# LCSL/nys-koop-lqr

Hardware: AMD Instinct MI355X
Metric: Nyström-Koopman fits/sec (K_nm build + A,B,C solve), N=1e5 m=2000 d=384 (higher is better)
Workload: dtype f64

## Files before the change

nys_koop_lqr_amd/csrc/nk_api.hip:

```cpp
#include "nk_common.h"

#include <cmath>
#include <cstdarg>
#include <cstdio>
#include <cstring>
#include <chrono>
#include <cstdlib>
#include <algorithm>
#include <condition_variable>
#include <mutex>
#include <set>
#include <thread>

namespace nk {

static thread_local std::string g_err;

void set_error(const char* fmt, ...) {
  char buf[1024];
  va_list ap;
  va_start(ap, fmt);
  vsnprintf(buf, sizeof(buf), fmt, ap);
  va_end(ap);
  g_err = buf;
// ... 111 lines not shown
  double* d = nullptr;
  NK_TRY(arena_alloc_t(ctx, (size_t)rows * ldd, &d));
  NK_HIP(hipMemcpy2DAsync(d, (size_t)ldd * 8, p, (size_t)ld * 8, (size_t)cols * 8, (size_t)rows, hipMemcpyHostToDevice,
                          ctx->stream));
  out->ptr = d;
  out->ld = ldd;
  out->staged = true;
  return NK_OK;
}
struct MatOut {
  double* dev = nullptr;
  int64_t ld = 0;
  double* host = nullptr;
  int64_t host_ld = 0;
  int64_t rows = 0, cols = 0;
};
static int stage_out(nk_ctx* ctx, double* p, int64_t ld, int64_t rows, int64_t cols, MatOut* out) {
  out->rows = rows;
  out->cols = cols;
  if (is_device_ptr(p)) {
    out->dev = p;
    out->ld = ld;
    out->host = nullptr;
    return NK_OK;
  }
  const int64_t ldd = cols + (cols & 1);
  NK_TRY(arena_alloc_t(ctx, (size_t)(rows > 0 ? rows : 1) * ldd, &out->dev));
  out->ld = ldd;
  out->host = p;
  out->host_ld = ld;
  return NK_OK;
}
static int finish_out(nk_ctx* ctx, const MatOut& o) {
  if (o.host && o.rows > 0 && o.cols > 0)
    NK_HIP(hipMemcpy2DAsync(o.host, (size_t)o.host_ld * 8, o.dev, (size_t)o.ld * 8, (size_t)o.cols * 8, (size_t)o.rows,
                            hipMemcpyDeviceToHost, ctx->stream));
  return NK_OK;
}

static int check_ctx(nk_ctx* ctx) {
  if (!ctx) {
    set_error("null context");
    return NK_ERR_BAD_ARG;
  }
  tl_ctx = ctx;
  NK_HIP(hipSetDevice(ctx->device));
  return arena_reset(ctx);
}

static int make_winv(nk_ctx* ctx, const nk_kernel_desc* kd, int d, double* dst_dev) {
  NK_REQUIRE(kd != nullptr, "null kernel descriptor");
  NK_REQUIRE(kd->type >= NK_KERNEL_RBF && kd->type <= NK_KERNEL_LINEAR, "unknown kernel type %d", kd->type);
  NK_REQUIRE(kd->d == d, "kernel descriptor is for %d dimensions, data has %d", kd->d, d);
  std::vector<double> w((size_t)d, 1.0);
  if (kd->type != NK_KERNEL_LINEAR) {
    NK_REQUIRE(kd->lengthscale != nullptr, "kernel lengthscale pointer is null");
    NK_REQUIRE(kd->n_lengthscale == 1 || kd->n_lengthscale == d,
               "Anisotropic kernel must have the same number of dimensions as data (%d!=%d)", kd->n_lengthscale, d);
    for (int k = 0; k < d; ++k) {
      const double l = kd->lengthscale[kd->n_lengthscale == 1 ? 0 : k];
      NK_REQUIRE(l > 0.0 && std::isfinite(l), "lengthscale[%d] = %g is not positive", k, l);
      w[k] = 1.0 / l;
    }
  }
  NK_HIP(hipMemcpyAsync(dst_dev, w.data(), sizeof(double) * d, hipMemcpyHostToDevice, ctx->stream));
  NK_HIP(hipStreamSynchronize(ctx->stream));
  return NK_OK;
}

struct ModelBuf {
  int device;
  size_t bytes;
  double* ptr;
};
static std::mutex g_pool_mu;
static std::vector<ModelBuf> g_pool;
static std::mutex g_reg_mu;
static std::set<nk_ctx*> g_ctxs;
static std::set<nk_model*> g_models;
static std::set<void*> g_host_blocks;

static double* pool_take(int device, size_t bytes) {
  std::lock_guard<std::mutex> lk(g_pool_mu);
  for (size_t i = 0; i < g_pool.size(); ++i)
    if (g_pool[i].device == device && g_pool[i].bytes == bytes) {
      double* p = g_pool[i].ptr;
      g_pool.erase(g_pool.begin() + i);
      return p;
    }
  return nullptr;
}
static void pool_give(int device, size_t bytes, double* ptr) {
  {
    std::lock_guard<std::mutex> lk(g_pool_mu);
    if (g_pool.size() < 512) {
      g_pool.push_back(ModelBuf{device, bytes, ptr});
      return;
    }
  }
  (void)hipSetDevice(device);
  (void)hipFree(ptr);
}
static void pool_drain() {
  std::lock_guard<std::mutex> lk(g_pool_mu);
  for (auto& b : g_pool) {
    (void)hipSetDevice(b.device);
    (void)hipFree(b.ptr);
  }
  g_pool.clear();
}

static int model_alloc(nk_ctx* ctx, int m, int d, int p, nk_model** out) {
  nk_model* mdl = new nk_model();
  mdl->device = ctx->device;
  mdl->m = m; mdl->d = d; mdl->p = p;
  const size_t mp = (size_t)m + p;
  const size_t total = (size_t)m * mp  + (size_t)d * m  + (size_t)d * mp  + 2 * (size_t)m * m +
                       (size_t)m * d  + (size_t)d  + 64;
  mdl->bytes = total * sizeof(double);
  mdl->buf = pool_take(ctx->device, mdl->bytes);
  if (!mdl->buf) {
    hipError_t e = hipMalloc(reinterpret_cast<void**>(&mdl->buf), mdl->bytes);
    if (e != hipSuccess) {
      (void)hipGetLastError();
      delete mdl;
      set_error("model allocation of %zu bytes failed: %s", total * sizeof(double), hipGetErrorString(e));
      return NK_ERR_OOM;
    }
  }
  double* q = mdl->buf;
  auto take = [&](size_t cnt) { double* r = q; q += (cnt + 1) & ~(size_t)1; return r; };
  mdl->A = take((size_t)m * mp);
  mdl->B = mdl->A + m;
  mdl->C = take((size_t)d * m);
  mdl->W = take((size_t)d * mp);
  mdl->S = take((size_t)m * m);
  mdl->Sinv = take((size_t)m * m);
  mdl->Z = take((size_t)m * d);
  mdl->winv = take((size_t)d);
  {
    std::lock_guard<std::mutex> lk(g_reg_mu);
    g_models.insert(mdl);
  }
  *out = mdl;
  return NK_OK;
}

static int lift_device(nk_ctx* ctx, const nk_model* mdl, const double* Xq, int64_t ldx, int64_t nq, double* out,
                       int64_t ldo) {
  const int m = mdl->m;
  const int64_t chunk = 32768;
  const ArenaMark mk = arena_mark(ctx);
  double* Kq = nullptr;
  NK_TRY(arena_alloc_t(ctx, (size_t)(nq < chunk ? nq : chunk) * m, &Kq));
  for (int64_t r0 = 0; r0 < nq; r0 += chunk) {
    const int64_t len = nq - r0 < chunk ? nq - r0 : chunk;
    NK_TRY(launch_kmat(ctx, mdl->ktype, Xq + r0 * ldx, ldx, len, mdl->Z, mdl->d, m, mdl->d, mdl->winv, mdl->sigma0, Kq,
                       m));
    NK_TRY(launch_gemm(ctx, false, false, len, m, m, 1.0, Kq, m, mdl->Sinv, m, 0.0, out + r0 * ldo, ldo));
  }
  arena_release(ctx, mk);
  return NK_OK;
}

static int predict_device(nk_ctx* ctx, const nk_model* mdl, const double* Xaug, int64_t ldx, int64_t nq, double* out,
                          int64_t ldo) {
  const int m = mdl->m, d = mdl->d, p = mdl->p;
  const int64_t chunk = 32768;
  const ArenaMark mk = arena_mark(ctx);
  double* phi = nullptr;
  NK_TRY(arena_alloc_t(ctx, (size_t)(nq < chunk ? nq : chunk) * m, &phi));
  for (int64_t r0 = 0; r0 < nq; r0 += chunk) {
    const int64_t len = nq - r0 < chunk ? nq - r0 : chunk;
    NK_TRY(lift_device(ctx, mdl, Xaug + r0 * ldx, ldx, len, phi, m));
    NK_TRY(launch_gemm(ctx, false, true, len, d, m, 1.0, phi, m, mdl->W, m + p, 0.0, out + r0 * ldo, ldo));
    if (p > 0)
      NK_TRY(launch_gemm(ctx, false, true, len, d, p, 1.0, Xaug + r0 * ldx + d, ldx, mdl->W + m, m + p, 1.0,
                         out + r0 * ldo, ldo));
  }
  arena_release(ctx, mk);
  return NK_OK;
}

struct HostTrace {
  bool on;
  std::chrono::steady_clock::time_point t0, last;
  HostTrace() : on(getenv("NYSKOOP_TRACE") != nullptr) { t0 = last = std::chrono::steady_clock::now(); }
  void mark(const char* what) {
    if (!on) return;
    auto now = std::chrono::steady_clock::now();
    fprintf(stderr, "[nk trace] %-28s +%8.3f ms (total %8.3f)\n", what,
            std::chrono::duration<double, std::milli>(now - last).count(),
            std::chrono::duration<double, std::milli>(now - t0).count());
    last = now;
  }
};

static float ev_ms(nk_ctx* ctx, int a, int b) {
  float ms = 0.f;
  (void)hipEventElapsedTime(&ms, ctx->ev[a], ctx->ev[b]);
  return ms;
}

}

using namespace nk;

extern "C" {

int nk_version(void) { return NK_ABI_VERSION; }

const char* nk_last_error(void) { return g_err.c_str(); }

int nk_device_count(void) {
  int n = 0;
  if (hipGetDeviceCount(&n) != hipSuccess) {
    (void)hipGetLastError();
    return 0;
  }
  return n;
}

int nk_create(int device, nk_ctx** out) {
  NK_REQUIRE(out != nullptr, "nk_create: null output pointer");
  *out = nullptr;
  int n = nk_device_count();
  if (n <= 0) {
    set_error("no HIP device visible: libnyskoop has no CPU fallback");
    return NK_ERR_NO_DEVICE;
  }
  NK_REQUIRE(device >= 0 && device < n, "nk_create: device %d out of range (0..%d)", device, n - 1);
  NK_HIP(hipSetDevice(device));
  hipDeviceProp_t prop;
  NK_HIP(hipGetDeviceProperties(&prop, device));
  if (strncmp(prop.gcnArchName, "gfx950", 6) != 0) {
    set_error("device %d is %s; libnyskoop is built for gfx950 (MI355X) only", device, prop.gcnArchName);
    return NK_ERR_NO_DEVICE;
  }
  nk_ctx* ctx = new nk_ctx();
  ctx->device = device;
  ctx->num_cu = prop.multiProcessorCount;
  int prio_lo = 0, prio_hi = 0;
  NK_HIP(hipDeviceGetStreamPriorityRange(&prio_lo, &prio_hi));
  const int prio_mid = (prio_lo - prio_hi >= 2) ? (prio_lo + prio_hi) / 2 : prio_hi;
  NK_HIP(hipStreamCreateWithPriority(&ctx->stream_main, hipStreamNonBlocking, prio_mid));
  NK_HIP(hipStreamCreateWithPriority(&ctx->stream_side, hipStreamNonBlocking, prio_lo));
  NK_HIP(hipStreamCreateWithPriority(&ctx->stream_prep, hipStreamNonBlocking, prio_hi));
  NK_HIP(hipStreamCreateWithFlags(&ctx->stream_copy, hipStreamNonBlocking));
  NK_HIP(hipStreamCreateWithPriority(&ctx->stream_la[0], hipStreamNonBlocking, prio_hi));
  NK_HIP(hipStreamCreateWithPriority(&ctx->stream_la[1], hipStreamNonBlocking, prio_mid));
  for (int q = 0; q < 2; ++q)
    for (int i = 0; i < 4; ++i) NK_HIP(hipEventCreateWithFlags(&ctx->ev_la[q][i], hipEventDisableTiming));
  ctx->stream = ctx->stream_main;
  ctx->cur_arena = &ctx->arena;
  NK_HIP(hipEventCreateWithFlags(&ctx->ev_fork, hipEventDisableTiming));
  NK_HIP(hipEventCreateWithFlags(&ctx->ev_join, hipEventDisableTiming));
  NK_HIP(hipEventCreateWithFlags(&ctx->ev_chain, hipEventDisableTiming));
  NK_HIP(hipMalloc(reinterpret_cast<void**>(&ctx->d_info), 256));
  ctx->d_piv = reinterpret_cast<unsigned long long*>(ctx->d_info + 16);
  NK_HIP(hipMalloc(reinterpret_cast<void**>(&ctx->d_scalars), 64 * sizeof(double)));
  NK_HIP(hipHostMalloc(reinterpret_cast<void**>(&ctx->h_scalars), 64 * sizeof(double), hipHostMallocMapped | hipHostMallocCoherent));
  NK_HIP(hipHostMalloc(reinterpret_cast<void**>(&ctx->h_info), 256, hipHostMallocMapped | hipHostMallocCoherent));
  ctx->h_piv = reinterpret_cast<unsigned long long*>(ctx->h_info + 16);
  for (int i = 0; i < 16; ++i) NK_HIP(hipEventCreate(&ctx->ev[i]));
  NK_HIP(hipEventCreateWithFlags(&ctx->ev_ext, hipEventDisableTiming));
  for (int i = 0; i < 8; ++i) NK_HIP(hipEventCreateWithFlags(&ctx->ev_up[i], hipEventDisableTiming));
  const char* km = getenv("NYSKOOP_KMAT");
  ctx->kmat_mode = (km && strcmp(km, "direct") == 0) ? 1 : 0;
  const char* st = getenv("NYSKOOP_STRICT_SPD");
  ctx->strict_spd = (st && atoi(st) != 0) ? 1 : 0;
  if (const char* rp = getenv("NYSKOOP_REFINE_PIVOT")) ctx->refine_pivot = atof(rp);
  if (const char* rs = getenv("NYSKOOP_REFINE_STEPS")) ctx->refine_steps = std::max(0, atoi(rs));
  {
    std::lock_guard<std::mutex> lk(g_reg_mu);
    g_ctxs.insert(ctx);
  }
  *out = ctx;
  return NK_OK;
}

static void destroy_ctx_unregistered(nk_ctx* ctx) {
  (void)hipSetDevice(ctx->device);
  if (tl_ctx == ctx) tl_ctx = nullptr;
  group_detach(ctx);
  (void)hipStreamSynchronize(ctx->stream_main);
  (void)hipStreamSynchronize(ctx->stream_side);
  (void)hipStreamSynchronize(ctx->stream_prep);
  (void)hipStreamSynchronize(ctx->stream_copy);
  for (int q = 0; q < 2; ++q) {
    if (ctx->stream_la[q]) { (void)hipStreamSynchronize(ctx->stream_la[q]); (void)hipStreamDestroy(ctx->stream_la[q]); }
    for (int i = 0; i < 4; ++i) if (ctx->ev_la[q][i]) (void)hipEventDestroy(ctx->ev_la[q][i]);
  }
  for (auto& c : ctx->arena.chunks) (void)hipFree(c.base);
  for (auto& c : ctx->arena_side.chunks) (void)hipFree(c.base);
  (void)hipEventDestroy(ctx->ev_fork);
  (void)hipEventDestroy(ctx->ev_join);
  if (ctx->ev_chain) (void)hipEventDestroy(ctx->ev_chain);
  if (ctx->ev_ext) (void)hipEventDestroy(ctx->ev_ext);
  for (int i = 0; i < 8; ++i) if (ctx->ev_up[i]) (void)hipEventDestroy(ctx->ev_up[i]);
  (void)hipStreamDestroy(ctx->stream_side);
  (void)hipStreamDestroy(ctx->stream_prep);
  (void)hipStreamDestroy(ctx->stream_copy);
  (void)hipFree(ctx->d_info);
  (void)hipFree(ctx->d_scalars);
  if (ctx->d_zeros) (void)hipFree(ctx->d_zeros);
  if (ctx->h_stage) (void)hipHostFree(ctx->h_stage);
  (void)hipHostFree(ctx->h_scalars);
  (void)hipHostFree(ctx->h_info);
  for (int i = 0; i < 16; ++i) (void)hipEventDestroy(ctx->ev[i]);
  (void)hipStreamDestroy(ctx->stream_main);
  delete ctx;
}

int nk_destroy(nk_ctx* ctx) {
  if (!ctx) return NK_OK;
  {
    std::lock_guard<std::mutex> lk(g_reg_mu);
    if (g_ctxs.erase(ctx) == 0) return NK_OK;
  }
  destroy_ctx_unregistered(ctx);
  return NK_OK;
}

static int model_wait_unchecked(nk_model* mdl);
static void destroy_model_unregistered(nk_model* model, bool to_pool) {
  (void)model_wait_unchecked(model);
  if (to_pool) {
    pool_give(model->device, model->bytes, model->buf);
  } else {
    (void)hipSetDevice(model->device);
    (void)hipFree(model->buf);
  }
  delete model;
}

int nk_shutdown(void) {
  tl_ctx = nullptr;
  std::set<nk_ctx*> ctxs;
  std::set<nk_model*> models;
  std::set<void*> blocks;
  {
    std::lock_guard<std::mutex> lk(g_reg_mu);
    ctxs.swap(g_ctxs);
    models.swap(g_models);
    blocks.swap(g_host_blocks);
  }
  for (nk_ctx* c : ctxs) {
    (void)hipSetDevice(c->device);
    (void)hipStreamSynchronize(c->stream_main);
    (void)hipStreamSynchronize(c->stream_side);
    (void)hipStreamSynchronize(c->stream_prep);
    (void)hipStreamSynchronize(c->stream_copy);
  }
  for (nk_model* m : models) destroy_model_unregistered(m, false);
  for (nk_ctx* c : ctxs) destroy_ctx_unregistered(c);
  pool_drain();
  for (void* b : blocks) (void)hipHostFree(b);
  return NK_OK;
}

int nk_set_compute_dtype(nk_ctx* ctx, int dtype) {
  NK_REQUIRE(ctx != nullptr && (dtype == NK_DTYPE_F64 || dtype == NK_DTYPE_F32), "nk_set_compute_dtype: bad argument");
  ctx->compute_f32 = dtype == NK_DTYPE_F32 ? 1 : 0;
  return NK_OK;
}

int nk_set_strict_spd(nk_ctx* ctx, int strict) {
  NK_REQUIRE(ctx != nullptr && strict >= 0 && strict <= 2, "nk_set_strict_spd: bad argument");
  ctx->strict_spd = strict;
  return NK_OK;
}

int nk_set_refine(nk_ctx* ctx, double pivot_ratio, int32_t steps) {
  NK_REQUIRE(ctx != nullptr && pivot_ratio >= 0.0 && pivot_ratio <= 1.0 && steps >= 0 && steps <= 8, "nk_set_refine: bad argument");
  ctx->refine_pivot = pivot_ratio;
  ctx->refine_steps = steps;
  return NK_OK;
}

int nk_wait_stream(nk_ctx* ctx, void* producer_stream) {
  NK_REQUIRE(ctx != nullptr, "nk_wait_stream: null context");
  NK_HIP(hipSetDevice(ctx->device));
  if (ctx->group) {
    hipError_t e = real_stream_sync(reinterpret_cast<hipStream_t>(producer_stream));
    if (e != hipSuccess) { set_error("synchronising the producer stream failed: %s", hipGetErrorString(e)); return NK_ERR_HIP; }
    return NK_OK;
  }
  NK_HIP(hipEventRecord(ctx->ev_ext, reinterpret_cast<hipStream_t>(producer_stream)));
  NK_HIP(hipStreamWaitEvent(ctx->stream_main, ctx->ev_ext, 0));
  NK_HIP(hipStreamWaitEvent(ctx->stream_side, ctx->ev_ext, 0));
  NK_HIP(hipStreamWaitEvent(ctx->stream_prep, ctx->ev_ext, 0));
  NK_HIP(hipStreamWaitEvent(ctx->stream_copy, ctx->ev_ext, 0));
  return NK_OK;
}

int nk_group_create(int device, int size, nk_ctx** out) {
  NK_REQUIRE(out != nullptr && size >= 1 && size <= 256, "nk_group_create: bad argument");
  for (int i = 0; i < size; ++i) out[i] = nullptr;
  for (int i = 0; i < size; ++i) {
    int rc = nk_create(device, &out[i]);
    if (rc != NK_OK) {
      for (int j = 0; j < i; ++j) { nk_destroy(out[j]); out[j] = nullptr; }
      return rc;
    }
  }
  nk_group* g = group_new(device, size);
  if (!g) {
    for (int i = 0; i < size; ++i) { nk_destroy(out[i]); out[i] = nullptr; }
    set_error("nk_group_create: could not create the shared stream / argument table");
    return NK_ERR_HIP;
  }
  for (int i = 0; i < size; ++i) group_attach(g, i, out[i]);
  return NK_OK;
}

int nk_group_enter(nk_ctx* ctx) {
  NK_REQUIRE(ctx != nullptr, "nk_group_enter: null context");
  return group_enter(ctx);
}

int nk_group_leave(nk_ctx* ctx) {
  NK_REQUIRE(ctx != nullptr, "nk_group_leave: null context");
  tl_ctx = ctx;
  const int rc = group_leave(ctx);
  tl_ctx = nullptr;
  return rc;
}

int nk_runtime_counters(uint64_t* out, int32_t n) {
  NK_REQUIRE(out != nullptr && n >= 0, "nk_runtime_counters: bad argument");
  for (int i = 0; i < n && i < CNT_N; ++i) out[i] = nk::read_counter(i);
  return NK_OK;
}

int nk_group_stats(nk_ctx* ctx, uint64_t* out4) {
  NK_REQUIRE(ctx != nullptr && out4 != nullptr, "nk_group_stats: null argument");
  group_stats(ctx, out4);
  return NK_OK;
}

int nk_cv_grid(nk_ctx* const* members, int32_t n_members, const double* X, int64_t ldx, const double* Y, int64_t ldy,
               int64_t n, int32_t d, int32_t p, const nk_cv_unit* units, int32_t n_units, double* scores, int32_t* status) {
  NK_REQUIRE(members && n_members >= 1 && X && Y && units && scores, "nk_cv_grid: null argument");
  NK_REQUIRE(n > 0 && d > 0 && p >= 0 && n_units >= 0 && ldx >= d + p && ldy >= d, "nk_cv_grid: bad sizes");
  for (int k = 0; k < n_members; ++k) NK_REQUIRE(members[k] != nullptr, "nk_cv_grid: null member context");
  for (int u = 0; u < n_units; ++u) {
    const nk_cv_unit& cu = units[u];
    NK_REQUIRE(cu.kernel && cu.landmark_rows && cu.m > 0, "nk_cv_grid: unit %d: null kernel / landmarks", u);
    NK_REQUIRE(0 <= cu.test_begin && cu.test_begin < cu.test_end && cu.test_end <= n, "nk_cv_grid: unit %d: bad test fold", u);
    for (int j = 0; j < cu.m; ++j)
      NK_REQUIRE(cu.landmark_rows[j] >= 0 && cu.landmark_rows[j] < n, "nk_cv_grid: unit %d: landmark row out of range", u);
  }
  if (n_units == 0) return NK_OK;
  nk_ctx* lead = members[0];
  NK_HIP(hipSetDevice(lead->device));
  const double *Xd = X, *Yd = Y;
  int64_t ldxd = ldx, ldyd = ldy;
  double *Xown = nullptr, *Yown = nullptr;
  struct Free { double*& a; double*& b; ~Free() { if (a) (void)hipFree(a); if (b) (void)hipFree(b); } } freer{Xown, Yown};
  if (!is_device_ptr(X)) {
    ldxd = d + p + ((d + p) & 1);
    NK_HIP(hipMalloc(reinterpret_cast<void**>(&Xown), (size_t)n * ldxd * 8));
    NK_HIP(hipMemcpy2D(Xown, (size_t)ldxd * 8, X, (size_t)ldx * 8, (size_t)(d + p) * 8, (size_t)n, hipMemcpyHostToDevice));
    Xd = Xown;
  }
  if (!is_device_ptr(Y)) {
    ldyd = d + (d & 1);
    NK_HIP(hipMalloc(reinterpret_cast<void**>(&Yown), (size_t)n * ldyd * 8));
    NK_HIP(hipMemcpy2D(Yown, (size_t)ldyd * 8, Y, (size_t)ldy * 8, (size_t)d * 8, (size_t)n, hipMemcpyHostToDevice));
    Yd = Yown;
  }
  std::vector<double> Yhost;
  const double* Yh = Y;
  int64_t ldyh = ldy;
  if (is_device_ptr(Y)) {
    Yhost.resize((size_t)n * d);
    NK_HIP(hipMemcpy2D(Yhost.data(), (size_t)d * 8, Y, (size_t)ldy * 8, (size_t)d * 8, (size_t)n, hipMemcpyDeviceToHost));
    Yh = Yhost.data();
    ldyh = d;
  }
  const int B = n_members;
  struct Round {
    std::mutex mu;
    std::condition_variable cv;
    int arrived = 0;
    uint64_t gen = 0;
    void wait(int parties) {
      std::unique_lock<std::mutex> lk(mu);
      const uint64_t g = gen;
      if (++arrived == parties) { arrived = 0; ++gen; lk.unlock(); cv.notify_all(); return; }
      cv.wait(lk, [&] { return gen != g; });
    }
  };
  std::vector<int> saved_strict((size_t)B);
  for (int k = 0; k < B; ++k) saved_strict[(size_t)k] = members[k]->strict_spd;
  std::mutex deferred_mu;
  std::vector<int> deferred;
  auto run_units = [&](const std::vector<int>& list, bool defer_rank_deficient) {
    Round round;
    const int count = (int)list.size();
    const int n_rounds = (count + B - 1) / B;
    auto worker = [&](int k) {
      nk_ctx* ctx = members[k];
      std::vector<double> Z;
      for (int r = 0; r < n_rounds; ++r) {
        const int slot = r * B + k;
        const bool mine = slot < count;
        if (mine) (void)group_enter(ctx);
        round.wait(B);
        if (mine) {
          const int u = list[(size_t)slot];
          const nk_cv_unit& cu = units[u];
          Z.resize((size_t)cu.m * d);
          for (int j = 0; j < cu.m; ++j) memcpy(&Z[(size_t)j * d], Yh + cu.landmark_rows[j] * ldyh, (size_t)d * 8);
          const int64_t rr[4] = {0, cu.test_begin, cu.test_end, n};
          nk_model* mdl = nullptr;
          int rc = nk_nystrom_fit(ctx, cu.kernel, Xd, ldxd, Yd, ldyd, n, d, p, rr, 2, nullptr, 0, Z.data(), d, cu.m, cu.gamma,
                                  cu.jitter, &mdl, nullptr);
          double sc = std::nan("");
          if (rc == NK_OK)
            rc = nk_score_neg_rmse(ctx, mdl, Xd + cu.test_begin * ldxd, ldxd, Yd + cu.test_begin * ldyd, ldyd,
                                   cu.test_end - cu.test_begin, &sc);
          if (mdl) nk_model_destroy(mdl);
          tl_ctx = ctx;
          const int rc_leave = group_leave(ctx);
          if (rc == NK_OK) rc = rc_leave;
          if (rc == NK_ERR_NOT_SPD && defer_rank_deficient) {
            std::lock_guard<std::mutex> lk(deferred_mu);
            deferred.push_back(u);
          } else {
            scores[u] = rc == NK_OK ? sc : std::nan("");
            if (status) status[u] = rc;
          }
        }
        round.wait(B);
      }
      tl_ctx = nullptr;
    };
    std::vector<std::thread> threads;
    threads.reserve((size_t)B);
    for (int k = 0; k < B; ++k) threads.emplace_back(worker, k);
    for (auto& t : threads) t.join();
  };
  std::vector<int> all((size_t)n_units);
  for (int u = 0; u < n_units; ++u) all[(size_t)u] = u;
  bool all_lenient = true;
  for (int k = 0; k < B; ++k) all_lenient = all_lenient && saved_strict[(size_t)k] == 0;
  if (!all_lenient) {
    run_units(all, false);
    return NK_OK;
  }
  const bool cv_trace = getenv("NYSKOOP_CV_TRACE") != nullptr;
  const auto t_start = std::chrono::steady_clock::now();
  for (int k = 0; k < B; ++k) members[k]->strict_spd = 1;
  run_units(all, true);
  for (int k = 0; k < B; ++k) members[k]->strict_spd = saved_strict[(size_t)k];
  const auto t_mid = std::chrono::steady_clock::now();
  if (!deferred.empty()) {
    std::sort(deferred.begin(), deferred.end());
    for (int k = 0; k < B; ++k) members[k]->strict_spd = 0;
    run_units(deferred, false);
    for (int k = 0; k < B; ++k) members[k]->strict_spd = saved_strict[(size_t)k];
  }
  if (cv_trace)
    fprintf(stderr, "[nyskoop] cv_grid: %d units in %.3f s, %zu rank-deficient units again in %.3f s (%d members)\n", n_units,
            std::chrono::duration<double>(t_mid - t_start).count(), deferred.size(),
            std::chrono::duration<double>(std::chrono::steady_clock::now() - t_mid).count(), B);
  return NK_OK;
}

int nk_synchronize(nk_ctx* ctx) {
  NK_REQUIRE(ctx != nullptr, "null context");
  tl_ctx = ctx;
  NK_HIP(hipStreamSynchronize(ctx->stream));
  return NK_OK;
}

void* nk_stream(nk_ctx* ctx) { return ctx ? reinterpret_cast<void*>(ctx->stream) : nullptr; }

void* nk_host_alloc(uint64_t bytes) {
  void* p = nullptr;
  if (hipHostMalloc(&p, bytes ? bytes : 1, hipHostMallocDefault) != hipSuccess) {
    (void)hipGetLastError();
    set_error("hipHostMalloc of %llu bytes failed", (unsigned long long)bytes);
    return nullptr;
  }
  std::lock_guard<std::mutex> lk(g_reg_mu);
  g_host_blocks.insert(p);
  return p;
}

void nk_host_free(void* ptr) {
  if (!ptr) return;
  {
    std::lock_guard<std::mutex> lk(g_reg_mu);
    if (g_host_blocks.erase(ptr) == 0) return;
  }
  (void)hipHostFree(ptr);
}

int nk_set_kmat_mode(nk_ctx* ctx, int mode) {
  NK_REQUIRE(ctx != nullptr && (mode == 0 || mode == 1), "nk_set_kmat_mode: bad argument");
  ctx->kmat_mode = mode;
  return NK_OK;
}

// ... 208 lines not shown
  };
  auto queue_side = [&]() -> int {
    NK_TRY(alloc_sqrt_bufs());
    SideScope side(ctx);
    NK_HIP(hipStreamWaitEvent(ctx->stream, ctx->ev_fork, 0));
    NK_HIP(hipStreamWaitEvent(ctx->stream, ev[9], 0));
    NK_HIP(hipEventRecord(ev[6], ctx->stream));
    NK_TRY(sqrtm_finish(ctx, &splan, mdl->S, mdl->Sinv));
    NK_HIP(hipEventRecord(ev[7], ctx->stream));
    NK_TRY(sqrt_products());
    NK_HIP(hipEventRecord(ctx->ev_join, ctx->stream));
    return NK_OK;
  };
  if (mode == FIT_SOLVE) {
    NK_HIP(hipMemcpyAsync(G1, gram_io, gram_doubles(m, d, p) * sizeof(double),
                          is_device_ptr(gram_io) ? hipMemcpyDeviceToDevice : hipMemcpyHostToDevice, ctx->stream));
    NK_HIP(hipEventRecord(ev[2], ctx->stream));
  } else {
  const bool f32 = ctx->compute_f32 != 0 && ctx->kmat_mode == 0 && d >= 32 && !ctx_recording(ctx) && m >= 4 && d >= 4;
  const int64_t off_out = f32 ? ((mp + 3) & ~3) : ((mp + 1) & ~1);
  const int64_t ldf = f32 ? ((off_out + m + 3) & ~(int64_t)3) : ((off_out + m + 1) & ~(int64_t)1);
  const double felem = f32 ? 4.0 : 8.0;
  int64_t pass_rows;
  {
    const char* b = getenv("NYSKOOP_F_BUDGET_GB");
    const double budget = (b ? atof(b) : 48.0) * 1073741824.0;
    pass_rows = (int64_t)(budget / ((double)ldf * felem));
    if (pass_rows < 1024) pass_rows = 1024;
    pass_rows &= ~(int64_t)1023;
    if (host_passes > 1) {
      const int64_t per = ((n_eff + host_passes - 1) / host_passes + 1023) & ~(int64_t)1023;
      if (per < pass_rows) pass_rows = per;
    }
  }
  struct Piece { int64_t b, len; };
  std::vector<std::vector<Piece>> passes(1);
  {
    int64_t used = 0;
    for (size_t i = 0; i < rng.size(); i += 2) {
      int64_t b = rng[i];
      const int64_t e = rng[i + 1];
      while (b < e) {
        if (used == pass_rows) { passes.emplace_back(); used = 0; }
        const int64_t len = std::min(e - b, pass_rows - used);
        passes.back().push_back(Piece{b, len});
        used += len;
        b += len;
      }
    }
  }
  const int64_t f_rows = passes.size() > 1 ? pass_rows : n_eff;
  double* F = nullptr;
  NK_TRY(arena_alloc_t(ctx, f32 ? ((size_t)f_rows * ldf + 1) / 2 + 64 : (size_t)f_rows * ldf + 64, &F));
  const bool gram_form = ctx->kmat_mode == 0 && d >= 32;
  int64_t maxlen = 0;
  for (auto& ps : passes) for (auto& pc : ps) maxlen = std::max(maxlen, pc.len);
  const int64_t ldt = (maxlen + 1) & ~(int64_t)1, ldzt = (m + 1) & ~1;
  double *center = nullptr, *Rt = nullptr, *sqr = nullptr, *Zto = nullptr, *sqzo = nullptr, *Zti = nullptr, *sqzi = nullptr;
  double *Rt2 = nullptr, *sqr2 = nullptr;
  const bool overlap_prep = gram_form && passes.size() == 1 && passes[0].size() == 1;
  if (gram_form) {
    NK_TRY(arena_alloc_t(ctx, (size_t)d, &center));
    if (!f32) {
      NK_TRY(arena_alloc_t(ctx, (size_t)d * ldt, &Rt));
      NK_TRY(arena_alloc_t(ctx, (size_t)maxlen, &sqr));
    }
    if (overlap_prep && !f32) {
      NK_TRY(arena_alloc_t(ctx, (size_t)d * ldt, &Rt2));
      NK_TRY(arena_alloc_t(ctx, (size_t)maxlen, &sqr2));
    }
    NK_TRY(arena_alloc_t(ctx, (size_t)d * ldzt, &Zto));
    NK_TRY(arena_alloc_t(ctx, (size_t)m, &sqzo));
    if (kd->type == NK_KERNEL_LINEAR) NK_TRY(launch_fill(ctx, center, d, 1, d, 0.0));
    else NK_TRY(launch_colmean(ctx, zo.ptr, zo.ld, m, d, center));
    NK_TRY(prep_rows(ctx, zo.ptr, zo.ld, m, d, mdl->winv, center, Zto, ldzt, sqzo));
    if (same_centers) {
      Zti = Zto; sqzi = sqzo;
    } else {
      NK_TRY(arena_alloc_t(ctx, (size_t)d * ldzt, &Zti));
      NK_TRY(arena_alloc_t(ctx, (size_t)m, &sqzi));
      NK_TRY(prep_rows(ctx, zi.ptr, zi.ld, m, d, mdl->winv, center, Zti, ldzt, sqzi));
    }
  }
  float *F32 = reinterpret_cast<float*>(F), *Rt32 = nullptr, *sq32 = nullptr, *Zt32 = nullptr, *sqz32 = nullptr, *Y32 = nullptr;
  const int64_t ldt32 = (maxlen + 3) & ~(int64_t)3, ldzt32 = (m + 3) & ~3, ldy32 = (d + 3) & ~3;
  if (f32) {
    NK_REQUIRE(same_centers, "fp32 engine: separate input landmarks are not supported");
    double* tmp = nullptr;
    NK_TRY(arena_alloc_t(ctx, ((size_t)d * ldt32 + 1) / 2 + 2, &tmp)); Rt32 = reinterpret_cast<float*>(tmp);
    NK_TRY(arena_alloc_t(ctx, ((size_t)maxlen + 1) / 2 + 2, &tmp)); sq32 = reinterpret_cast<float*>(tmp);
    NK_TRY(arena_alloc_t(ctx, ((size_t)d * ldzt32 + 1) / 2 + 2, &tmp)); Zt32 = reinterpret_cast<float*>(tmp);
    NK_TRY(arena_alloc_t(ctx, ((size_t)m + 1) / 2 + 2, &tmp)); sqz32 = reinterpret_cast<float*>(tmp);
    NK_TRY(arena_alloc_t(ctx, ((size_t)f_rows * ldy32 + 1) / 2 + 2, &tmp)); Y32 = reinterpret_cast<float*>(tmp);
    NK_TRY(prep_rows_f32(ctx, zo.ptr, zo.ld, m, d, mdl->winv, center, Zt32, ldzt32, sqz32));
  }
  const bool multi_pass = passes.size() > 1;
  const bool pipelined = host_passes > 1;
  auto upload_pass = [&](size_t ip) -> int {
    for (const Piece& pc : passes[ip]) {
      NK_HIP(hipMemcpy2DAsync(const_cast<double*>(x.ptr) + pc.b * x.ld, (size_t)x.ld * 8, X + pc.b * ldx, (size_t)ldx * 8,
                              (size_t)(d + p) * 8, (size_t)pc.len, hipMemcpyHostToDevice, ctx->stream_side));
      NK_HIP(hipMemcpy2DAsync(const_cast<double*>(y.ptr) + pc.b * y.ld, (size_t)y.ld * 8, Y + pc.b * ldy, (size_t)ldy * 8,
                              (size_t)d * 8, (size_t)pc.len, hipMemcpyHostToDevice, ctx->stream_side));
    }
    NK_HIP(hipEventRecord(ctx->ev_up[ip & 7], ctx->stream_side));
    return NK_OK;
  };
  if (pipelined) {
    NK_HIP(hipEventRecord(ev[12], ctx->stream));
    NK_HIP(hipStreamWaitEvent(ctx->stream_side, ev[12], 0));
    NK_TRY(upload_pass(0));
  }
  for (size_t ip = 0; ip < passes.size(); ++ip) {
    const std::vector<Piece>& ps = passes[ip];
    const double beta = ip == 0 ? 0.0 : 1.0;
    if (pipelined) NK_HIP(hipStreamWaitEvent(ctx->stream, ctx->ev_up[ip & 7], 0));
    if (f32) {
      int64_t o32 = 0;
      for (const Piece& pc : ps) {
        const double* xs = x.ptr + pc.b * x.ld;
        const double* ys = y.ptr + pc.b * y.ld;
        NK_TRY(prep_rows_f32(ctx, xs, x.ld, pc.len, d, mdl->winv, center, Rt32, ldt32, sq32));
        NK_TRY(launch_kmat_gram_f32(ctx, kd->type, Rt32, ldt32, sq32, pc.len, Zt32, ldzt32, sqz32, m, d, kd->sigma0,
                                    F32 + o32 * ldf, ldf));
        NK_TRY(prep_rows_f32(ctx, ys, y.ld, pc.len, d, mdl->winv, center, Rt32, ldt32, sq32));
        NK_TRY(launch_kmat_gram_f32(ctx, kd->type, Rt32, ldt32, sq32, pc.len, Zt32, ldzt32, sqz32, m, d, kd->sigma0,
                                    F32 + o32 * ldf + off_out, ldf));
        if (p > 0) NK_TRY(launch_cvt_f64_f32(ctx, xs + d, x.ld, F32 + o32 * ldf + m, ldf, pc.len, p));
        NK_TRY(launch_cvt_f64_f32(ctx, ys, y.ld, Y32 + o32 * ldy32, ldy32, pc.len, d));
        o32 += pc.len;
      }
      if (ip == 0) {
        NK_HIP(hipEventRecord(ev[2], ctx->stream));
        tr.mark("kmat issued");
      }
      TnProblemF pf[4];
      pf[0].A = F32; pf[0].B = F32; pf[0].lda = pf[0].ldb = ldf; pf[0].M = pf[0].N = mp; pf[0].C = G1; pf[0].ldc = mp;
      pf[0].tri = TRI_UPPER_MIRROR;
      pf[1].A = F32 + off_out; pf[1].B = F32; pf[1].lda = pf[1].ldb = ldf; pf[1].M = m; pf[1].N = mp; pf[1].C = G2; pf[1].ldc = mp;
      pf[2].A = F32 + off_out; pf[2].B = F32 + off_out; pf[2].lda = pf[2].ldb = ldf; pf[2].M = pf[2].N = m; pf[2].C = G3;
      pf[2].ldc = m; pf[2].tri = TRI_UPPER_MIRROR;
      pf[3].A = Y32; pf[3].lda = ldy32; pf[3].M = d; pf[3].N = m; pf[3].C = G4; pf[3].ldc = m; pf[3].B = F32 + off_out;
      pf[3].ldb = ldf;
      for (int q = 0; q < 4; ++q) pf[q].beta = beta;
      float ms1 = 0.f;
      NK_TRY(launch_gemm_tn_f32_multi(ctx, pf, 4, o32, 0, timed ? &ms1 : nullptr, multi_pass));
      if (multi_pass) ms_gram_kernel += ms1; else gram_deferred = timed;
      gram_launches += 1;
      if (pipelined && ip + 1 < passes.size()) NK_TRY(upload_pass(ip + 1));
      continue;
    }
    int64_t o = 0;
    for (const Piece& pc : ps) {
      const double* xs = x.ptr + pc.b * x.ld;
      const double* ys = y.ptr + pc.b * y.ld;
      if (gram_form && overlap_prep) {
        NK_HIP(hipEventRecord(ev[12], ctx->stream));
        {
          SideScope side(ctx);
          NK_HIP(hipStreamWaitEvent(ctx->stream, ev[12], 0));
          NK_TRY(prep_rows(ctx, ys, y.ld, pc.len, d, mdl->winv, center, Rt2, ldt, sqr2));
          NK_HIP(hipEventRecord(ev[13], ctx->stream));
        }
        NK_TRY(prep_rows(ctx, xs, x.ld, pc.len, d, mdl->winv, center, Rt, ldt, sqr));
        NK_TRY(launch_kmat_gram(ctx, kd->type, Rt, ldt, sqr, pc.len, Zti, ldzt, sqzi, m, d, kd->sigma0, F + o * ldf, ldf));
        NK_HIP(hipStreamWaitEvent(ctx->stream, ev[13], 0));
        NK_TRY(launch_kmat_gram(ctx, kd->type, Rt2, ldt, sqr2, pc.len, Zto, ldzt, sqzo, m, d, kd->sigma0,
                                F + o * ldf + off_out, ldf));
      } else if (gram_form) {
        NK_TRY(prep_rows(ctx, xs, x.ld, pc.len, d, mdl->winv, center, Rt, ldt, sqr));
        NK_TRY(launch_kmat_gram(ctx, kd->type, Rt, ldt, sqr, pc.len, Zti, ldzt, sqzi, m, d, kd->sigma0, F + o * ldf, ldf));
        NK_TRY(prep_rows(ctx, ys, y.ld, pc.len, d, mdl->winv, center, Rt, ldt, sqr));
        NK_TRY(launch_kmat_gram(ctx, kd->type, Rt, ldt, sqr, pc.len, Zto, ldzt, sqzo, m, d, kd->sigma0,
                                F + o * ldf + off_out, ldf));
      } else {
        NK_TRY(launch_kmat(ctx, kd->type, xs, x.ld, pc.len, zi.ptr, zi.ld, m, d, mdl->winv, kd->sigma0, F + o * ldf, ldf));
        NK_TRY(launch_kmat(ctx, kd->type, ys, y.ld, pc.len, zo.ptr, zo.ld, m, d, mdl->winv, kd->sigma0,
                           F + o * ldf + off_out, ldf));
      }
      if (p > 0) NK_TRY(launch_copy2d(ctx, xs + d, x.ld, F + o * ldf + m, ldf, pc.len, p));
      o += pc.len;
    }
    const int64_t rows = o;
    if (ip == 0) {
      NK_HIP(hipEventRecord(ev[2], ctx->stream));
      tr.mark("kmat issued");
    }
    TnProblem pr[4];
    pr[0].A = F; pr[0].B = F; pr[0].lda = pr[0].ldb = ldf; pr[0].M = pr[0].N = mp; pr[0].C = G1; pr[0].ldc = mp;
    pr[0].tri = TRI_UPPER_MIRROR;
    pr[1].A = F + off_out; pr[1].B = F; pr[1].lda = pr[1].ldb = ldf; pr[1].M = m; pr[1].N = mp; pr[1].C = G2;
    pr[1].ldc = mp;
    pr[2].A = F + off_out; pr[2].B = F + off_out; pr[2].lda = pr[2].ldb = ldf; pr[2].M = pr[2].N = m; pr[2].C = G3;
    pr[2].ldc = m; pr[2].tri = TRI_UPPER_MIRROR;
    pr[3].A = y.ptr + ps[0].b * y.ld; pr[3].lda = y.ld; pr[3].M = d; pr[3].N = m; pr[3].C = G4; pr[3].ldc = m;
    pr[3].B = F + off_out; pr[3].ldb = ldf;
    for (int q = 0; q < 4; ++q) pr[q].beta = beta;
    const bool single = ps.size() == 1;
    const bool fast = tn_fast_ok(pr[0]) && tn_fast_ok(pr[1]) && tn_fast_ok(pr[2]);
    const bool fast_y = fast && tn_fast_ok(pr[3]);
    bool y_done = false;
    if (fast) {
      const int np = (single && fast_y) ? 4 : 3;
      float ms1 = 0.f;
      NK_TRY(launch_gemm_tn_multi(ctx, pr, np, rows, 0, (timed && !pipelined) ? &ms1 : nullptr, multi_pass));
      if (multi_pass) ms_gram_kernel += ms1; else gram_deferred = timed;
      gram_launches += 1;
      y_done = np == 4;
    } else {
      GemmOpts sym;
      sym.tri = TRI_UPPER_MIRROR;
      float t3[3] = {0.f, 0.f, 0.f};
      NK_TRY(launch_gemm(ctx, true, false, mp, mp, rows, 1.0, F, ldf, F, ldf, beta, G1, mp, sym, timed ? &t3[0] : nullptr));
      NK_TRY(launch_gemm(ctx, true, false, m, mp, rows, 1.0, F + off_out, ldf, F, ldf, beta, G2, mp, GemmOpts(),
                         timed ? &t3[1] : nullptr));
      NK_TRY(launch_gemm(ctx, true, false, m, m, rows, 1.0, F + off_out, ldf, F + off_out, ldf, beta, G3, m, sym,
                         timed ? &t3[2] : nullptr));
      ms_gram_kernel += t3[0] + t3[1] + t3[2];
      gram_launches += 3;
    }
    if (!y_done) {
      int64_t oo = 0;
      bool first = true;
      for (const Piece& pc : ps) {
        NK_TRY(launch_gemm(ctx, true, false, d, m, pc.len, 1.0, y.ptr + pc.b * y.ld, y.ld, F + oo * ldf + off_out, ldf,
                           (first && ip == 0) ? 0.0 : 1.0, G4, m));
        oo += pc.len;
        first = false;
      }
    }
    if (pipelined && ip + 1 < passes.size()) NK_TRY(upload_pass(ip + 1));
  }
  }
  NK_HIP(hipEventRecord(ev[3], ctx->stream));
  if (mode == FIT_GRAM) {
    NK_HIP(hipMemcpyAsync(gram_io, G1, gram_doubles(m, d, p) * sizeof(double),
                          is_device_ptr(gram_io) ? hipMemcpyDeviceToDevice : hipMemcpyDeviceToHost, ctx->stream));
    NK_HIP(hipStreamSynchronize(ctx->stream));
    if (stats) {
      memset(stats, 0, sizeof(*stats));
      stats->ms_total = ev_ms(ctx, 0, 3);
      stats->ms_upload = (x.staged || y.staged) ? ev_ms(ctx, 0, 1) : 0.0;
      stats->ms_kmat = ev_ms(ctx, 1, 2);
      stats->ms_gram = ev_ms(ctx, 2, 3);
      if (gram_deferred) ms_gram_kernel = ev_ms(ctx, 14, 15);
      stats->ms_gram_kernel_avg = gram_launches ? ms_gram_kernel / gram_launches : 0.0;
      stats->gram_kernel_launches = gram_launches;
    }
    if (ctx->arena.chunks.size() > 1 || ctx->arena_side.chunks.size() > 1) NK_TRY(arena_reset(ctx));
    return NK_OK;
  }
  NK_HIP(hipEventRecord(ctx->ev_fork, ctx->stream));
  tr.mark("gram issued");

  NK_TRY(queue_prep());

  if (landmarks_aside) NK_HIP(hipStreamWaitEvent(ctx->stream, ev[8], 0));
  NK_TRY(launch_axpby2d(ctx, gamma_n, Kj_in, m, 1.0, G1, mp, m, m));
  if (p > 0) NK_TRY(launch_add_diag(ctx, G1 + (int64_t)m * mp + m, mp, p, gamma_n));
  NK_TRY(launch_axpby2d(ctx, gamma_n, Kj, m, 1.0, G3, m, m, m));
  double* Gsave = nullptr;
  NK_TRY(arena_alloc_t(ctx, gram_doubles(m, d, p), &Gsave));
  NK_HIP(hipMemcpyAsync(Gsave, G1, gram_doubles(m, d, p) * sizeof(double), hipMemcpyDeviceToDevice, ctx->stream));
  double *Linv = nullptr, *Linv2 = nullptr, *V1 = nullptr, *Wc = nullptr, *Ct = nullptr;
  const int nblk = (mp + CHOL_NB - 1) / CHOL_NB;
  NK_TRY(arena_alloc_t(ctx, (size_t)nblk * CHOL_WS, &Linv));
  NK_TRY(arena_alloc_t(ctx, (size_t)nblk * CHOL_WS, &Linv2));
  NK_TRY(arena_alloc_t(ctx, (size_t)m * m, &V1));
  NK_TRY(alloc_sqrt_bufs());
  NK_TRY(arena_alloc_t(ctx, (size_t)m * ldd, &Wc));
  NK_TRY(arena_alloc_t(ctx, (size_t)m * ldd, &Ct));
  CholSys sys[2];
  double* pivlog = nullptr;
  NK_TRY(arena_alloc_t(ctx, (size_t)mp + m + 4, &pivlog));
  sys[0].P = G1; sys[0].ldp = mp; sys[0].m = mp; sys[0].Linv = Linv; sys[0].extra = m;
  sys[1].P = G3; sys[1].ldp = m; sys[1].m = m; sys[1].Linv = Linv2; sys[1].extra = d;
  sys[0].pivlog = pivlog; sys[1].pivlog = pivlog + mp + (mp & 1);
  NK_TRY(cholesky_aug_pair_async(ctx, sys, 2));
  tr.mark("cholesky + solves issued");

  NK_TRY(queue_side());
  NK_HIP(hipStreamWaitEvent(ctx->stream, ctx->ev_join, 0));
  NK_HIP(hipEventRecord(ev[4], ctx->stream));
  tr.mark("side stream joined (queued)");

  auto operator_products = [&]() -> int {
    NK_TRY(launch_transpose(ctx, G2, mp, V1, m, m, m));
    NK_TRY(launch_gemm(ctx, true, false, m, m, m, 1.0, V1, m, T1t, m, 0.0, X1, m));
    NK_TRY(launch_gemm(ctx, true, false, m, m, m, 1.0, Sinvt, m, X1, m, 0.0, mdl->A, mp));
    if (p > 0) NK_TRY(launch_gemm(ctx, true, false, m, p, m, 1.0, Sinvt, m, G2 + m, mp, 0.0, mdl->B, mp));
    NK_TRY(launch_transpose(ctx, G4, m, Wc, ldd, d, m));
    NK_TRY(launch_gemm(ctx, true, false, m, d, m, 1.0, mdl->S, m, Wc, ldd, 0.0, Ct, ldd));
    NK_TRY(launch_transpose(ctx, Ct, ldd, mdl->C, m, m, d));
    NK_TRY(launch_gemm(ctx, true, false, d, mp, m, 1.0, Ct, ldd, mdl->A, mp, 0.0, mdl->W, mp));
    return NK_OK;
  };
  NK_TRY(operator_products());
  NK_HIP(hipEventRecord(ev[5], ctx->stream));
  tr.mark("solve issued");
  int chol_failed[2] = {0, 0};
  double piv_ratio[2] = {1.0, 1.0};
  NK_TRY(cholesky_fail_flags(ctx, sys, 2, chol_failed, piv_ratio));
  tr.mark("final sync");
  int rank_sys[2] = {mp, m};
  bool redo_products = false;
  if (ctx->strict_spd == 2) chol_failed[0] = chol_failed[1] = -1;
  if (chol_failed[0] || chol_failed[1]) {
    if (ctx->strict_spd == 1) {
      set_error("Cholesky: system %d is numerically rank deficient (non-positive or rounding-level pivot; the reference's "
                "lstsq truncates here) and strict mode is on", chol_failed[0] ? 0 : 1);
      return NK_ERR_NOT_SPD;
    }
    const double rcond = 2.220446049250313e-16;
    for (int q = 0; q < 2; ++q) {
      if (!chol_failed[q]) continue;
      PinvInfo pi;
      if (q == 0)
        NK_TRY(pinv_right_divide(ctx, Gsave, mp, mp, Gsave + (size_t)mp * mp, mp, m, G2, mp, rcond, &pi));
      else
        NK_TRY(pinv_right_divide(ctx, Gsave + gram_block1(m, p), m, m, Gsave + gram_block1(m, p) + (size_t)m * m, m, d, G4,
                                 m, rcond, &pi));
      if (!pi.converged) {
        set_error("rank-revealing fallback: Jacobi SVD of system %d did not converge in %d sweeps", q, pi.sweeps);
        return NK_ERR_NO_CONVERGENCE;
      }
      rank_sys[q] = pi.rank;
    }
    count_event(CNT_RANK_TRUNCATED);
    redo_products = true;
  }
  int refined[2] = {0, 0};
  {
    const double refine_below = ctx->refine_pivot;
    const int refine_steps = ctx->refine_steps;
    double* refine_state = nullptr;
    NK_TRY(arena_alloc_t(ctx, (size_t)8, &refine_state));
    for (int q = 0; q < 2 && refine_steps > 0; ++q) {
      if (chol_failed[q] || !(piv_ratio[q] > 0.0) || piv_ratio[q] >= refine_below) continue;
      const int mq = sys[q].m, nr = sys[q].extra;
      const size_t off = q == 0 ? 0 : gram_block1(m, p);
      const double* Pq = Gsave + off;
      const double* Rq = Gsave + off + (size_t)mq * mq;
      double* Xq = G1 + off + (size_t)mq * mq;
      const ArenaMark mk = arena_mark(ctx);
      double *Res = nullptr, *ResT = nullptr, *partial = nullptr;
      const int64_t ldt_ = nr + (nr & 1);
      NK_TRY(arena_alloc_t(ctx, (size_t)nr * mq, &Res));
      NK_TRY(arena_alloc_t(ctx, (size_t)mq * ldt_, &ResT));
      NK_TRY(arena_alloc_t(ctx, (size_t)2 * refine_partial_blocks(), &partial));
      CholSys y = sys[q];
      y.R = ResT; y.ldr = ldt_; y.nrhs = nr;
      for (int step = 0; step < refine_steps; ++step) {
        NK_TRY(launch_resid_dd(ctx, Xq, mq, Pq, mq, Rq, mq, Res, mq, nr, mq));
        NK_TRY(launch_transpose(ctx, Res, mq, ResT, ldt_, nr, mq));
        NK_TRY(cholesky_solve_pair(ctx, &y, 1));
        NK_TRY(launch_transpose(ctx, ResT, ldt_, Res, mq, mq, nr));
        NK_TRY(launch_refine_apply(ctx, Res, mq, Xq, mq, nr, mq, step, refine_state + 4 * q, partial));
      }
      NK_HIP(hipMemcpyAsync(ctx->h_scalars + 16 + 4 * q, refine_state + 4 * q, 4 * sizeof(double), hipMemcpyDeviceToHost,
                            ctx->stream));
      arena_release(ctx, mk);
      refined[q] = -1;
      redo_products = true;
    }
  }
  {
    const int vr = sqrtm_verdict(ctx, &splan, &it, &resid);
    if (vr == NK_SQRT_RETRY) {
      count_event(CNT_SQRT_RETRY);
      NK_TRY(sqrtm_spd_coupled(ctx, Kj, m, m, mdl->S, mdl->Sinv, &it, &resid));
      NK_TRY(sqrt_products());
      redo_products = true;
    } else {
      NK_TRY(vr);
    }
  }
  if (redo_products) {
    NK_TRY(operator_products());
    NK_HIP(hipStreamSynchronize(ctx->stream));
  }
  double refine_ratio[2] = {0.0, 0.0};
  for (int q = 0; q < 2; ++q)
    if (refined[q] < 0) {
      refined[q] = (int)ctx->h_scalars[16 + 4 * q + 2];
      refine_ratio[q] = ctx->h_scalars[16 + 4 * q + 3];
    }
  if (refined[0] > 0 || refined[1] > 0) count_event(CNT_REFINED);
  mdl->has_ops = true;

  if (stats) {
    memset(stats, 0, sizeof(*stats));
    stats->ms_total = ev_ms(ctx, 0, 5);
    stats->ms_upload = (x.staged || y.staged) ? ev_ms(ctx, 0, 1) : 0.0;
    stats->ms_kmat = ev_ms(ctx, 1, 2);
    stats->ms_gram = ev_ms(ctx, 2, 3);
    stats->ms_sqrt = ev_ms(ctx, 6, 7);
    stats->ms_solve = ev_ms(ctx, 4, 5);
    if (gram_deferred) ms_gram_kernel = ev_ms(ctx, 14, 15);
    stats->ms_gram_kernel_avg = gram_launches ? ms_gram_kernel / gram_launches : 0.0;
    stats->gram_kernel_launches = gram_launches;
    stats->sqrt_iters = it;
    stats->sqrt_residual = resid;
    const double ne = (double)n_eff;
    const double t128 = 128.0;
    auto tiles = [&](double v) { return std::ceil(v / t128); };
    const double tmp_ = tiles(mp), tm_ = tiles(m);
    stats->gram_flops = 2.0 * ne * t128 * t128 * (tmp_ * (tmp_ + 1) / 2 + tm_ * tmp_ + tm_ * (tm_ + 1) / 2) +
                        2.0 * ne * (double)d * m;
    stats->kmat_pairs = 2.0 * ne * m * d + (same_centers ? 1.0 : 3.0) * (double)m * m * d;
    stats->rank_inner = rank_sys[0];
    stats->rank_inner_rec = rank_sys[1];
    stats->pivot_ratio_inner = piv_ratio[0];
    stats->pivot_ratio_inner_rec = piv_ratio[1];
    stats->refined = refined[0] + 16 * refined[1];
    stats->refine_ratio_inner = refine_ratio[0];
    stats->refine_ratio_inner_rec = refine_ratio[1];
  }
  tr.mark("stats");
  if (ctx->arena.chunks.size() > 1 || ctx->arena_side.chunks.size() > 1) NK_TRY(arena_reset(ctx));
  guard.m = nullptr;
  *model = mdl;
  return NK_OK;
}

int nk_nystrom_fit(nk_ctx* ctx, const nk_kernel_desc* kd, const double* X, int64_t ldx, const double* Y, int64_t ldy,
                   int64_t n, int32_t d, int32_t p, const int64_t* row_ranges, int32_t n_ranges, const double* Zin,
                   int64_t ldzi, const double* Zout, int64_t ldzo, int32_t m, double gamma, double jitter,
                   nk_model** model, nk_fit_stats* stats) {
  NK_REQUIRE(model != nullptr, "nk_nystrom_fit: null argument");
  return fit_impl(ctx, kd, X, ldx, Y, ldy, n, d, p, row_ranges, n_ranges, Zin, ldzi, Zout, ldzo, m, gamma, jitter, model,
                  stats, FIT_FULL, nullptr);
}

int nk_gram_doubles(int32_t m, int32_t d, int32_t p, int64_t* count) {
  NK_REQUIRE(count && m > 0 && d > 0 && p >= 0, "nk_gram_doubles: bad argument");
  *count = (int64_t)gram_doubles(m, d, p);
  return NK_OK;
}

int nk_nystrom_gram(nk_ctx* ctx, const nk_kernel_desc* kd, const double* X, int64_t ldx, const double* Y, int64_t ldy,
                    int64_t n, int32_t d, int32_t p, const int64_t* row_ranges, int32_t n_ranges, const double* Zin,
                    int64_t ldzi, const double* Zout, int64_t ldzo, int32_t m, double* gram, nk_fit_stats* stats) {
  return fit_impl(ctx, kd, X, ldx, Y, ldy, n, d, p, row_ranges, n_ranges, Zin, ldzi, Zout, ldzo, m, 0.0, 0.0, nullptr,
                  stats, FIT_GRAM, gram);
}

int nk_nystrom_solve(nk_ctx* ctx, const nk_kernel_desc* kd, const double* Zin, int64_t ldzi, const double* Zout,
                     int64_t ldzo, int32_t m, int32_t d, int32_t p, const double* gram, int64_t n_total, double gamma,
                     double jitter, nk_model** model, nk_fit_stats* stats) {
  NK_REQUIRE(model != nullptr, "nk_nystrom_solve: null argument");
  return fit_impl(ctx, kd, nullptr, 0, nullptr, 0, n_total, d, p, nullptr, 0, Zin, ldzi, Zout, ldzo, m, gamma, jitter,
                  model, stats, FIT_SOLVE, const_cast<double*>(gram));
}

int nk_model_create(nk_ctx* ctx, const nk_kernel_desc* kd, const double* Zout, int64_t ldz, int32_t m, int32_t d,
                    int32_t p, double jitter, const double* A, const double* B, const double* C, const double* W,
                    nk_model** model) {
  NK_TRY(check_ctx(ctx));
  NK_REQUIRE(kd && Zout && model, "nk_model_create: null argument");
  NK_REQUIRE(m > 0 && d > 0 && p >= 0 && ldz >= d, "nk_model_create: bad sizes");
  *model = nullptr;
  nk_model* mdl = nullptr;
  NK_TRY(model_alloc(ctx, m, d, p, &mdl));
  struct Guard { nk_model* m; ~Guard() { if (m) nk_model_destroy(m); } } guard{mdl};
  mdl->ktype = kd->type; mdl->sigma0 = kd->sigma0; mdl->jitter = jitter;
  NK_TRY(make_winv(ctx, kd, d, mdl->winv));
  MatIn z;
  NK_TRY(stage_in(ctx, Zout, ldz, m, d, &z));
  NK_TRY(launch_copy2d(ctx, z.ptr, z.ld, mdl->Z, d, m, d));
  double* Kj = nullptr;
  NK_TRY(arena_alloc_t(ctx, (size_t)m * m, &Kj));
  NK_TRY(launch_kmat(ctx, kd->type, mdl->Z, d, m, mdl->Z, d, m, d, mdl->winv, kd->sigma0, Kj, m));
  NK_TRY(launch_add_diag(ctx, Kj, m, m, jitter));
  NK_TRY(sqrtm_spd(ctx, Kj, m, m, mdl->S, mdl->Sinv, nullptr, nullptr));
  const int mp = m + p;
  if (A && C) {
    NK_REQUIRE(p == 0 || B != nullptr, "nk_model_create: B missing");
    MatIn a, b, c, w;
    NK_TRY(stage_in(ctx, A, m, m, m, &a));
    NK_TRY(launch_copy2d(ctx, a.ptr, a.ld, mdl->A, mp, m, m));
    if (p > 0) {
      NK_TRY(stage_in(ctx, B, p, m, p, &b));
      NK_TRY(launch_copy2d(ctx, b.ptr, b.ld, mdl->B, mp, m, p));
    }
    NK_TRY(stage_in(ctx, C, m, d, m, &c));
    NK_TRY(launch_copy2d(ctx, c.ptr, c.ld, mdl->C, m, d, m));
    if (W) {
      NK_TRY(stage_in(ctx, W, mp, d, mp, &w));
      NK_TRY(launch_copy2d(ctx, w.ptr, w.ld, mdl->W, mp, d, mp));
    } else {
      NK_TRY(launch_gemm(ctx, false, false, d, mp, m, 1.0, mdl->C, m, mdl->A, mp, 0.0, mdl->W, mp));
    }
    mdl->has_ops = true;
  }
  NK_HIP(hipStreamSynchronize(ctx->stream));
  guard.m = nullptr;
  *model = mdl;
  return NK_OK;
}

int nk_model_destroy(nk_model* model) {
  if (!model) return NK_OK;
  {
    std::lock_guard<std::mutex> lk(g_reg_mu);
    if (g_models.erase(model) == 0) return NK_OK;
  }
  destroy_model_unregistered(model, true);
  return NK_OK;
}

int nk_model_dims(const nk_model* model, int32_t* m, int32_t* d, int32_t* p) {
  NK_REQUIRE(model != nullptr, "null model");
  if (m) *m = model->m;
  if (d) *d = model->d;
  if (p) *p = model->p;
  return NK_OK;
}

int nk_model_get(nk_ctx* ctx, const nk_model* mdl, char which, double* out, int64_t ldo) {
  NK_TRY(check_ctx(ctx));
  NK_REQUIRE(mdl && out, "nk_model_get: null argument");
  const int m = mdl->m, d = mdl->d, p = mdl->p, mp = m + p;
  const double* src = nullptr;
  int64_t lds = 0, rows = 0, cols = 0;
  switch (which) {
    case 'A': src = mdl->A; lds = mp; rows = m; cols = m; break;
    case 'B': src = mdl->B; lds = mp; rows = m; cols = p; break;
    case 'C': src = mdl->C; lds = m; rows = d; cols = m; break;
    case 'W': src = mdl->W; lds = mp; rows = d; cols = mp; break;
    case 'S': src = mdl->S; lds = m; rows = m; cols = m; break;
    case 'I': src = mdl->Sinv; lds = m; rows = m; cols = m; break;
    case 'Z': src = mdl->Z; lds = d; rows = m; cols = d; break;
    default: set_error("nk_model_get: unknown selector '%c'", which); return NK_ERR_BAD_ARG;
  }
  if ((which == 'A' || which == 'B' || which == 'C' || which == 'W') && !mdl->has_ops) {
    set_error("nk_model_get: model holds no fitted operators");
    return NK_ERR_BAD_ARG;
  }
  if (rows == 0 || cols == 0) return NK_OK;
  NK_REQUIRE(ldo >= cols, "nk_model_get: leading dimension too small");
  NK_HIP(hipMemcpy2DAsync(out, (size_t)ldo * 8, src, (size_t)lds * 8, (size_t)cols * 8, (size_t)rows,
                          is_device_ptr(out) ? hipMemcpyDeviceToDevice : hipMemcpyDeviceToHost, ctx->stream));
  NK_HIP(hipStreamSynchronize(ctx->stream));
  return NK_OK;
}

int nk_model_get_ops(nk_ctx* ctx, const nk_model* mdl, double* G, int64_t ldg, double* Cm, int64_t ldc, double* W,
                     int64_t ldw) {
  NK_TRY(check_ctx(ctx));
  NK_REQUIRE(mdl != nullptr, "nk_model_get_ops: null model");
  if (!mdl->has_ops) {
    set_error("nk_model_get_ops: model holds no fitted operators");
    return NK_ERR_BAD_ARG;
  }
  const int m = mdl->m, d = mdl->d, mp = m + mdl->p;
  NK_REQUIRE((!G || ldg >= mp) && (!Cm || ldc >= m) && (!W || ldw >= mp), "nk_model_get_ops: leading dimension too small");
  auto copy = [&](double* dst, int64_t ldd, const double* src, int64_t lds, int64_t rows, int64_t cols,
                  hipStream_t st) -> hipError_t {
    const hipMemcpyKind kind = is_device_ptr(dst) ? hipMemcpyDeviceToDevice : hipMemcpyDeviceToHost;
    if (ldd == cols && lds == cols) return hipMemcpyAsync(dst, src, (size_t)rows * cols * 8, kind, st);
    return hipMemcpy2DAsync(dst, (size_t)ldd * 8, src, (size_t)lds * 8, (size_t)cols * 8, (size_t)rows, kind, st);
  };
  if (G) NK_HIP(copy(G, ldg, mdl->A, mp, m, mp, ctx->stream_main));
  if (Cm) NK_HIP(copy(Cm, ldc, mdl->C, m, d, m, ctx->stream_side));
  if (W) NK_HIP(copy(W, ldw, mdl->W, mp, d, mp, ctx->stream_side));
  NK_HIP(hipStreamSynchronize(ctx->stream_side));
  NK_HIP(hipStreamSynchronize(ctx->stream_main));
  return NK_OK;
}

int nk_model_get_ops_async(nk_ctx* ctx, nk_model* mdl, double* G, int64_t ldg, double* Cm, int64_t ldc, double* W,
                           int64_t ldw) {
  NK_TRY(check_ctx(ctx));
  NK_REQUIRE(mdl != nullptr, "nk_model_get_ops_async: null model");
  if (!mdl->has_ops) {
    set_error("nk_model_get_ops_async: model holds no fitted operators");
    return NK_ERR_BAD_ARG;
  }
  const int m = mdl->m, d = mdl->d, mp = m + mdl->p;
  NK_REQUIRE((!G || ldg >= mp) && (!Cm || ldc >= m) && (!W || ldw >= mp),
             "nk_model_get_ops_async: leading dimension too small");
  NK_TRY(nk_model_wait(mdl));
  auto copy = [&](double* dst, int64_t ldd, const double* src, int64_t lds, int64_t rows, int64_t cols) -> hipError_t {
    const hipMemcpyKind kind = is_device_ptr(dst) ? hipMemcpyDeviceToDevice : hipMemcpyDeviceToHost;
    if (ldd == cols && lds == cols) return hipMemcpyAsync(dst, src, (size_t)rows * cols * 8, kind, ctx->stream_copy);
    return hipMemcpy2DAsync(dst, (size_t)ldd * 8, src, (size_t)lds * 8, (size_t)cols * 8, (size_t)rows, kind,
                            ctx->stream_copy);
  };
  if (G) NK_HIP(copy(G, ldg, mdl->A, mp, m, mp));
  if (Cm) NK_HIP(copy(Cm, ldc, mdl->C, m, d, m));
  if (W) NK_HIP(copy(W, ldw, mdl->W, mp, d, mp));
  if (ctx_recording(ctx)) {
    NK_HIP(hipStreamSynchronize(ctx->stream));
    return NK_OK;
  }
  hipEvent_t ev = nullptr;
  NK_HIP(hipEventCreateWithFlags(&ev, hipEventDisableTiming));
  hipError_t e = hipEventRecord(ev, ctx->stream_copy);
  if (e != hipSuccess) {
    (void)hipEventDestroy(ev);
    (void)hipStreamSynchronize(ctx->stream_copy);
    set_error("hipEventRecord failed: %s", hipGetErrorString(e));
    return NK_ERR_HIP;
  }
  mdl->ev_fetch = ev;
  return NK_OK;
}

static int model_wait_unchecked(nk_model* mdl);

int nk_model_wait(nk_model* mdl) {
  NK_REQUIRE(mdl != nullptr, "nk_model_wait: null model");
  {
    std::lock_guard<std::mutex> lk(g_reg_mu);
    if (g_models.count(mdl) == 0) return NK_OK;
  }
  return model_wait_unchecked(mdl);
}

static int model_wait_unchecked(nk_model* mdl) {
  if (mdl->ev_fetch) {
    hipError_t e = real_event_sync(mdl->ev_fetch);
    (void)hipEventDestroy(mdl->ev_fetch);
    mdl->ev_fetch = nullptr;
    if (e != hipSuccess) {
      set_error("hipEventSynchronize failed: %s", hipGetErrorString(e));
      return NK_ERR_HIP;
    }
  }
  return NK_OK;
}

struct SmallStage {
  nk_ctx* ctx = nullptr;
  size_t off = 0;
  struct Out { double* stage; double* user; int64_t user_ld; int64_t rows, cols; };
  std::vector<Out> outs;
};
constexpr size_t SMALL_STAGE_LIMIT = (size_t)4 << 20;
static int small_reserve(nk_ctx* ctx, size_t bytes) {
  if (ctx->h_stage_bytes >= bytes) return NK_OK;
  if (ctx->h_stage) (void)hipHostFree(ctx->h_stage);
  ctx->h_stage = nullptr;
  ctx->h_stage_bytes = 0;
  NK_HIP(hipHostMalloc(reinterpret_cast<void**>(&ctx->h_stage), bytes, hipHostMallocDefault));
  ctx->h_stage_bytes = bytes;
  return NK_OK;
}
static const double* small_in(SmallStage& st, const double* host, int64_t ld, int64_t rows, int64_t cols) {
  double* dst = reinterpret_cast<double*>(reinterpret_cast<char*>(st.ctx->h_stage) + st.off);
  for (int64_t r = 0; r < rows; ++r) memcpy(dst + r * cols, host + r * ld, (size_t)cols * 8);
  st.off += (((size_t)rows * cols * 8) + 255) & ~(size_t)255;
  return dst;
}
static double* small_out(SmallStage& st, double* user, int64_t user_ld, int64_t rows, int64_t cols) {
  double* dst = reinterpret_cast<double*>(reinterpret_cast<char*>(st.ctx->h_stage) + st.off);
  st.off += (((size_t)rows * cols * 8) + 255) & ~(size_t)255;
  st.outs.push_back(SmallStage::Out{dst, user, user_ld, rows, cols});
  return dst;
}
static void small_finish(SmallStage& st) {
  for (auto& o : st.outs)
    for (int64_t r = 0; r < o.rows; ++r) memcpy(o.user + r * o.user_ld, o.stage + r * o.cols, (size_t)o.cols * 8);
}
static inline size_t pad256(size_t doubles) { return ((doubles * 8) + 255) & ~(size_t)255; }

int nk_lift(nk_ctx* ctx, const nk_model* mdl, const double* Xq, int64_t ldx, int64_t nq, double* out, int64_t ldo) {
  NK_TRY(check_ctx(ctx));
  NK_REQUIRE(mdl && Xq && out, "nk_lift: null argument");
  NK_REQUIRE(nq >= 0 && ldx >= mdl->d && ldo >= mdl->m, "nk_lift: bad sizes");
  if (nq == 0) return NK_OK;
// ... 518 lines not shown
```

nys_koop_lqr_amd/csrc/nk_common.h:

```cpp
#pragma once
#include <hip/hip_runtime.h>
#include <stdint.h>
#include <stddef.h>
#include <string>
#include <vector>

#include "nyskoop.h"
#include "nk_lockstep.h"

namespace nk {

void set_error(const char* fmt, ...);

#define NK_HIP(call)                                                                         \
  do {                                                                                       \
    hipError_t e_ = (call);                                                                  \
    if (e_ != hipSuccess) {                                                                  \
      nk::set_error("%s failed: %s (%s:%d)", #call, hipGetErrorString(e_), __FILE__, __LINE__); \
      return e_ == hipErrorOutOfMemory ? NK_ERR_OOM : NK_ERR_HIP;                            \
    }                                                                                        \
  } while (0)

#define NK_TRY(call)            \
  do {                          \
    int rc_ = (call);           \
    if (rc_ != NK_OK) return rc_; \
  } while (0)

#define NK_REQUIRE(cond, ...)     \
  do {                            \
    if (!(cond)) {                \
      nk::set_error(__VA_ARGS__); \
      return NK_ERR_BAD_ARG;      \
    }                             \
  } while (0)

struct ArenaChunk {
  char* base = nullptr;
  size_t cap = 0;
  size_t off = 0;
};
struct Arena {
  std::vector<ArenaChunk> chunks;
  int cur = 0;
};
struct ArenaMark {
  int chunk;
  size_t off;
};

}

struct nk_member_state;
struct nk_ctx {
  int device = 0;
  hipStream_t stream = nullptr;
  hipStream_t stream_main = nullptr;
  hipStream_t stream_side = nullptr;
  hipStream_t stream_copy = nullptr;
  hipStream_t stream_prep = nullptr;
  nk::Arena arena;
  nk::Arena arena_side;
  nk::Arena* cur_arena = nullptr;
  hipStream_t stream_la[2] = {nullptr, nullptr};
  hipEvent_t ev_la[2][4] = {};
  int compute_f32 = 0;
  hipEvent_t ev_fork = nullptr, ev_join = nullptr, ev_chain = nullptr;
  int* d_info = nullptr;
  unsigned long long* d_piv = nullptr;
  unsigned long long* h_piv = nullptr;
  double* d_scalars = nullptr;
  double* h_scalars = nullptr;
  int* h_info = nullptr;
  double* d_zeros = nullptr;
  hipEvent_t ev[16];
  int num_cu = 256;
  int kmat_mode = 0;
  double refine_pivot = 0.0;
  int refine_steps = 2;
  int strict_spd = 0;
  hipEvent_t ev_ext = nullptr;
  hipEvent_t ev_up[8] = {};
  nk_group* group = nullptr;
  nk_member_state* gstate = nullptr;
  double* h_stage = nullptr;
  size_t h_stage_bytes = 0;
};

struct nk_model {
  int device = 0;
  int32_t m = 0, d = 0, p = 0;
  int32_t ktype = 0;
  double sigma0 = 0.0;
  double jitter = 0.0;
  double* buf = nullptr;
  size_t bytes = 0;
  double *A = nullptr, *B = nullptr, *C = nullptr, *W = nullptr, *S = nullptr, *Sinv = nullptr, *Z = nullptr,
         *winv = nullptr;
  bool has_ops = false;
  hipEvent_t ev_fetch = nullptr;
};

namespace nk {

struct SideScope {
  nk_ctx* c;
  hipStream_t s0;
  Arena* a0;
  explicit SideScope(nk_ctx* ctx, hipStream_t s = nullptr) : c(ctx), s0(ctx->stream), a0(ctx->cur_arena) {
    c->stream = s ? s : c->stream_side;
    c->cur_arena = &c->arena_side;
  }
  ~SideScope() {
    c->stream = s0;
    c->cur_arena = a0;
  }
};

inline int info_base(const nk_ctx* c) { return c->stream != c->stream_main ? 2 : 0; }

__device__ __forceinline__ double exp_nonpos_ca() {
  double ca = __longlong_as_double(0x3e5ade156a5dcb37LL);
  asm volatile("" : "+v"(ca));
  return ca;
}
__device__ __forceinline__ double exp_nonpos(double x, double ca_v) {
  const double k = __builtin_rint(x * __longlong_as_double(0x3ff71547652b82feLL));
  double r = __builtin_fma(__longlong_as_double((long long)0xbfe62e42fefa39efULL), k, x);
  r = __builtin_fma(__longlong_as_double((long long)0xbc7abc9e3b39803fULL), k, r);
  double p;
#define NK_EXP_STEP(c) asm("v_fma_f64 %0, %1, %2, %3" : "=v"(p) : "v"(r), "v"(p), "s"(c))
  asm("v_fma_f64 %0, %1, %2, %3" : "=v"(p) : "v"(r), "v"(ca_v), "s"(__longlong_as_double(0x3e928af3fca7ab0cLL)));
  NK_EXP_STEP(__longlong_as_double(0x3ec71dee623fde64LL));
  NK_EXP_STEP(__longlong_as_double(0x3efa01997c89e6b0LL));
  NK_EXP_STEP(__longlong_as_double(0x3f2a01a014761f6eLL));
  NK_EXP_STEP(__longlong_as_double(0x3f56c16c1852b7b0LL));
  NK_EXP_STEP(__longlong_as_double(0x3f81111111122322LL));
  NK_EXP_STEP(__longlong_as_double(0x3fa55555555502a1LL));
  NK_EXP_STEP(__longlong_as_double(0x3fc5555555555511LL));
  NK_EXP_STEP(__longlong_as_double(0x3fe000000000000bLL));
#undef NK_EXP_STEP
  p = __builtin_fma(r, p, 1.0);
  p = __builtin_fma(r, p, 1.0);
  return x < -1075.0 ? 0.0 : ldexp(p, (int)k);
}
__device__ __forceinline__ double exp_nonpos(double x) { return exp_nonpos(x, exp_nonpos_ca()); }

nk_group* group_new(int device, int size);
void group_attach(nk_group* g, int slot, nk_ctx* c);
void group_detach(nk_ctx* c);
int group_enter(nk_ctx* c);
int group_leave(nk_ctx* c);
void group_stats(nk_ctx* c, uint64_t out[4]);
enum { CNT_CHAIN_GIVEUP = 0, CNT_JACOBI_GIVEUP = 1, CNT_RANK_TRUNCATED = 2, CNT_SQRT_RETRY = 3, CNT_REFINED = 4, CNT_N = 5 };
void count_event(int which);
uint64_t read_counter(int which);
hipError_t real_stream_sync(hipStream_t s);
hipError_t real_event_sync(hipEvent_t e);

int arena_reset(nk_ctx* ctx);
ArenaMark arena_mark(nk_ctx* ctx);
void arena_release(nk_ctx* ctx, ArenaMark mk);
int arena_alloc(nk_ctx* ctx, size_t bytes, void** out);
template <typename T>
inline int arena_alloc_t(nk_ctx* ctx, size_t count, T** out) {
  return arena_alloc(ctx, count * sizeof(T), reinterpret_cast<void**>(out));
}
bool is_device_ptr(const void* p);

int launch_kmat(nk_ctx* ctx, int ktype, const double* A, int64_t lda, int64_t nA, const double* B, int64_t ldb,
                int64_t nB, int d, const double* winv, double sigma0, double* out, int64_t ldo);

enum { TRI_FULL = 0, TRI_UPPER_MIRROR = 1, TRI_LOWER = 2 };
struct GemmOpts {
  int tri = TRI_FULL;
  int splitk = 0;
};
int launch_gemm(nk_ctx* ctx, bool transA, bool transB, int64_t M, int64_t N, int64_t K, double alpha, const double* A,
                int64_t lda, const double* B, int64_t ldb, double beta, double* C, int64_t ldc,
                const GemmOpts& opts = GemmOpts(), float* ms_kernel = nullptr);

struct GemmCall {
  int64_t M = 0, N = 0, K = 0;
  double alpha = 1.0, beta = 0.0;
  const double* A = nullptr;
  const double* B = nullptr;
  double* C = nullptr;
  int64_t lda = 0, ldb = 0, ldc = 0;
  GemmOpts opts;
};
int launch_gemm_pair(nk_ctx* ctx, bool transA, bool transB, const GemmCall* calls, int ncalls);

struct TnSkip;
int launch_add_diag(nk_ctx* ctx, double* A, int64_t lda, int n, double v);
int launch_copy2d(nk_ctx* ctx, const double* src, int64_t lds, double* dst, int64_t ldd, int64_t rows, int64_t cols);
int launch_axpby2d(nk_ctx* ctx, double a, const double* X, int64_t ldx, double b, double* Y, int64_t ldy,
                   int64_t rows, int64_t cols);
int launch_scale_add_identity(nk_ctx* ctx, double a, const double* X, int64_t ldx, double c, double* Y, int64_t ldy,
                              int n, const TnSkip* skip = nullptr);
int launch_fill(nk_ctx* ctx, double* A, int64_t lda, int64_t rows, int64_t cols, double v);
int launch_frob_minus_identity(nk_ctx* ctx, const double* M, int64_t ldm, int n, double* d_out,
                               const TnSkip* skip = nullptr);
int launch_max_abs_rowsum(nk_ctx* ctx, const double* M, int64_t ldm, int n, double* d_out);
int launch_colsum_sqdiff(nk_ctx* ctx, const double* P, int64_t ldp, const double* Y, int64_t ldy, int64_t rows,
                         int cols, double* d_colsum);

int sqrtm_spd(nk_ctx* ctx, const double* P, int64_t ldp, int m, double* S, double* Sinv, int* iters, double* resid);
struct SqrtPlan {
  const double* P = nullptr;
  int64_t ldp = 0;
  int m = 0;
  double* W = nullptr;
  double* Linv = nullptr;
  double* X0 = nullptr;
  double* X0t = nullptr;
  double* d_sc = nullptr;
  ArenaMark mark{0, 0};
  bool deferred = false;
  int rc = 0, iters = 0, kmax = 0;
  double resid = 0.0;
  double lambda_min_hint = 0.0;
  bool early = false;
  hipEvent_t pause_event = nullptr;
  int pause_step = -1;
};
constexpr int NK_SQRT_RETRY = 1;
int sqrtm_spd_coupled(nk_ctx* ctx, const double* P, int64_t ldp, int m, double* S, double* Sinv, int* iters, double* resid);
int sqrtm_prepare(nk_ctx* ctx, const double* P, int64_t ldp, int m, SqrtPlan* plan);
int sqrtm_finish(nk_ctx* ctx, SqrtPlan* plan, double* S, double* Sinv);
int sqrtm_verdict(nk_ctx* ctx, SqrtPlan* plan, int* iters, double* resid);
int cholesky_lower(nk_ctx* ctx, double* P, int64_t ldp, int m, double* Linv );
int cholesky_solve(nk_ctx* ctx, const double* L, int64_t ldl, int m, const double* Linv, double* R, int64_t ldr,
                   int nrhs);
struct CholSys {
  double* P = nullptr;
  int64_t ldp = 0;
  int m = 0;
  int extra = 0;
  bool backward = true;
  double* Linv = nullptr;
  double* pivlog = nullptr;
  double* R = nullptr;
  int64_t ldr = 0;
  int nrhs = 0;
};
int cholesky_lower_pair(nk_ctx* ctx, const CholSys* sys, int nsys);
int cholesky_lower_pair_async(nk_ctx* ctx, const CholSys* sys, int nsys);
int cholesky_check_pair(nk_ctx* ctx, const CholSys* sys, int nsys);
int cholesky_solve_pair(nk_ctx* ctx, const CholSys* sys, int nsys);
int cholesky_aug_pair_async(nk_ctx* ctx, const CholSys* sys, int nsys, hipEvent_t pause = nullptr, int pause_step = -1);
constexpr int CHOL_NB = 64;
constexpr int CHOL_WS = 2 * CHOL_NB * CHOL_NB + 8;
constexpr double CHOL_FIX_KAPPA = 8.0 * CHOL_NB;
inline int chol_fix_enabled() {
  const char* e = getenv("NYSKOOP_CHOL_FIX");
  return (e && e[0] == '0') ? 0 : ((e && e[0] == '2') ? 2 : 1);
}
bool launch_chol_trail_pair(nk_ctx* ctx, const GemmCall* calls, int ncalls, int* rc);
bool launch_chol_trail_potrf_pair(nk_ctx* ctx, const GemmCall* calls, int ncalls, const int* nb, double* const* Linv, int blk,
                                  double* const* plog, int* rc);
inline bool chol_fuse_enabled() {
  const char* e = getenv("NYSKOOP_CHOL_FUSE");
  return !(e && e[0] == '0');
}
bool launch_chol_panel_pair(nk_ctx* ctx, const GemmCall* calls, int ncalls, int* rc);
int launch_trsm_right_lower_pair(nk_ctx* ctx, const CholSys* sys, int nsys);

struct PinvInfo {
  int rank = 0, sweeps = 0;
  bool converged = false;
  double sigma_max = 0.0, sigma_min_kept = 0.0, sigma_min = 0.0;
};
int pinv_right_divide(nk_ctx* ctx, const double* P, int64_t ldp, int m, const double* E, int64_t lde, int rows,
                      double* E_out, int64_t ldeo, double rcond, PinvInfo* info);
int cholesky_fail_flags(nk_ctx* ctx, const CholSys* sys, int nsys, int* failed , double* piv_ratio = nullptr);

int launch_lifted_step(nk_ctx* ctx, const double* G, int64_t ldg, int m, int mz, int pu, const double* z, int64_t zstride,
                       const double* u, int64_t ustride, const double* bias, double* out, int64_t ostride, int batch);

struct ChainArgs {
  const double* G = nullptr; int64_t ldg = 0; int m = 0, pu = 0;
  const double* z0 = nullptr; int64_t z0_stride = 0;
  bool lift = false;
  const double* x0 = nullptr; int64_t x0_stride = 0;
  const double* Zl = nullptr; int d = 0; const double* winv = nullptr; const double* Sinv = nullptr; int ktype = 0;
  double sigma0 = 0.0;
  const double* U = nullptr; int64_t u_stride = 0;
  const double* bias = nullptr; int64_t bias_stride = 0;
  double* Zall = nullptr; int64_t z_stride = 0;
  int T = 0, batch = 0;
};
int launch_ref_minus_traj(nk_ctx* ctx, const double* ref, int64_t ref_stride, const double* Phi, int64_t phi_stride,
                          double* D, int64_t d_stride, int steps, int m, int batch);
bool lifted_chain_ok(int m, int pu, int d_lift);
int launch_lifted_chain(nk_ctx* ctx, const ChainArgs& a);
bool lifted_chain_mw_ok(const nk_ctx* ctx, int m, int pu);
int chain_mw_workgroups(int m);
int chain_mw_group(int m, int batch);
int launch_lifted_chain_mw(nk_ctx* ctx, const ChainArgs& a);
int lifted_chain_mw_reset(nk_ctx* ctx);
int lifted_chain_mw_fetch_status(nk_ctx* ctx);
bool lifted_chain_mw_timed_out(nk_ctx* ctx, int* row, int* step, int* traj);

}

namespace nk {
enum { KTRIM_NONE = 0, KTRIM_B_UPPER = 1 , KTRIM_A_LOWER = 2  };
struct TnProblem {
  const double* A = nullptr;
  const double* B = nullptr;
  double* C = nullptr;
  int64_t lda = 0, ldb = 0, ldc = 0;
  int M = 0, N = 0;
  int tri = TRI_FULL;
  int ktrim = 0;
  double alpha = 1.0, beta = 0.0;
  double* Ct = nullptr;
  int64_t ldct = 0;
  const double* A_even = nullptr;
  const double* B_even = nullptr;
  double* Caff = nullptr;
  double aff_a = 0.0, aff_c = 0.0;
};
struct TnSkip {
  const double* state = nullptr;
  int step = 0;
  const double* select = nullptr;
  double* resid_partials = nullptr;
  int* resid_count = nullptr;
};
bool tn_fast_ok(const TnProblem& p);
struct TnProblemF {
  const float* A = nullptr;
  const float* B = nullptr;
  double* C = nullptr;
  int64_t lda = 0, ldb = 0, ldc = 0;
  int M = 0, N = 0;
  int tri = TRI_FULL;
  double beta = 0.0;
};
bool tnf_fast_ok(const TnProblemF& p);
int launch_gemm_tn_f32_multi(nk_ctx* ctx, const TnProblemF* probs, int nprob, int64_t K, int splitk ,
                             float* ms_kernel = nullptr, bool sync_timing = true);
int prep_rows_f32(nk_ctx* ctx, const double* X, int64_t ldx, int64_t rows, int d, const double* winv, const double* center,
                  float* Xt, int64_t ldt, float* sq);
int launch_cvt_f64_f32(nk_ctx* ctx, const double* src, int64_t lds_, float* dst, int64_t ldd, int64_t rows, int cols);
int launch_kmat_gram_f32(nk_ctx* ctx, int ktype, const float* At, int64_t ldat, const float* sqa, int64_t nA, const float* Bt,
                         int64_t ldbt, const float* sqb, int64_t nB, int d, double sigma0, float* out, int64_t ldo);
int launch_gemm_tn_multi(nk_ctx* ctx, const TnProblem* probs, int nprob, int64_t K, int splitk ,
                         float* ms_kernel = nullptr, bool sync_timing = true, const TnSkip* skip = nullptr);
int launch_transpose(nk_ctx* ctx, const double* src, int64_t lds, double* dst, int64_t ldd, int rows, int cols);
constexpr int refine_partial_blocks() { return 512; }
int launch_refine_apply(nk_ctx* ctx, const double* dX, int64_t ldd, double* X, int64_t ldx, int64_t rows, int64_t cols, int step,
                        double* state, double* partial);
int launch_resid_dd(nk_ctx* ctx, const double* X, int64_t ldx, const double* P, int64_t ldp, const double* R, int64_t ldr,
                    double* Res, int64_t ldres, int nr, int mq);
int launch_colmean(nk_ctx* ctx, const double* Z, int64_t ldz, int rows, int d, double* mean);
int prep_rows(nk_ctx* ctx, const double* X, int64_t ldx, int64_t rows, int d, const double* winv, const double* center,
              double* Xt, int64_t ldt, double* sq);
int launch_kmat_gram(nk_ctx* ctx, int ktype, const double* At, int64_t ldat, const double* sqa, int64_t nA,
                     const double* Bt, int64_t ldbt, const double* sqb, int64_t nB, int d, double sigma0, double* out,
                     int64_t ldo);
}

#if defined(__HIPCC__)
namespace nk {
typedef unsigned chain_u2 __attribute__((ext_vector_type(2)));
template <int CTRL> __device__ __forceinline__ double dpp_f64(double v) {
  int lo = __double2loint(v), hi = __double2hiint(v);
  lo = __builtin_amdgcn_update_dpp(0, lo, CTRL, 0xf, 0xf, true);
  hi = __builtin_amdgcn_update_dpp(0, hi, CTRL, 0xf, 0xf, true);
  return __hiloint2double(hi, lo);
}
__device__ __forceinline__ void swap16_f64(double& a, double& b) {
  const chain_u2 lo = __builtin_amdgcn_permlane16_swap((unsigned)__double2loint(a), (unsigned)__double2loint(b), false, false);
  const chain_u2 hi = __builtin_amdgcn_permlane16_swap((unsigned)__double2hiint(a), (unsigned)__double2hiint(b), false, false);
  a = __hiloint2double((int)hi.x, (int)lo.x);
  b = __hiloint2double((int)hi.y, (int)lo.y);
}
__device__ __forceinline__ void swap32_f64(double& a, double& b) {
  const chain_u2 lo = __builtin_amdgcn_permlane32_swap((unsigned)__double2loint(a), (unsigned)__double2loint(b), false, false);
  const chain_u2 hi = __builtin_amdgcn_permlane32_swap((unsigned)__double2hiint(a), (unsigned)__double2hiint(b), false, false);
  a = __hiloint2double((int)hi.x, (int)lo.x);
  b = __hiloint2double((int)hi.y, (int)lo.y);
}
__device__ __forceinline__ double wave_sum64_dpp(double c) {
  c += dpp_f64<0xB1>(c);
  c += dpp_f64<0x4E>(c);
  c += dpp_f64<0x141>(c);
  c += dpp_f64<0x140>(c);
  double a = c, b = c;
  swap16_f64(a, b);
  c = a + b;
  a = c; b = c;
  swap32_f64(a, b);
  return a + b;
}

}
#endif
```

nys_koop_lqr_amd/csrc/nk_linalg.hip:

```cpp
#include "nk_common.h"

#include <algorithm>
#include <cmath>
#include <cstring>
#include <vector>

namespace nk {

__device__ __forceinline__ void add_diag_kernel_body(double* A, int64_t lda, int n, double v) {
  int i = blockIdx.x * blockDim.x + threadIdx.x;
  if (i < n) A[(int64_t)i * lda + i] += v;
}
__global__ void __launch_bounds__(256) add_diag_kernel(double* A, int64_t lda, int n, double v) { add_diag_kernel_body(A, lda, n, v); }
NK_BATCHED_TWIN(add_diag_kernel, (256), double*, int64_t, int, double)
__device__ __forceinline__ void copy2d_kernel_body(const double* __restrict__ src, int64_t lds, double* __restrict__ dst, int64_t ldd, int64_t rows, int64_t cols) {
  const int64_t total = rows * cols;
  for (int64_t e = blockIdx.x * (int64_t)blockDim.x + threadIdx.x; e < total; e += (int64_t)gridDim.x * blockDim.x) {
    const int64_t r = e / cols, c = e - r * cols;
    dst[r * ldd + c] = src[r * lds + c];
  }
}
__global__ void __launch_bounds__(256) copy2d_kernel(const double* __restrict__ src, int64_t lds, double* __restrict__ dst, int64_t ldd, int64_t rows, int64_t cols) { copy2d_kernel_body(src, lds, dst, ldd, rows, cols); }
NK_BATCHED_TWIN(copy2d_kernel, (256), const double*, int64_t, double*, int64_t, int64_t, int64_t)
__device__ __forceinline__ void axpby2d_kernel_body(double a, const double* __restrict__ X, int64_t ldx, double b, double* __restrict__ Y, int64_t ldy, int64_t rows, int64_t cols) {
// ... 316 lines not shown
  if (rows <= 0 || cols <= 0) return NK_OK;
  hipLaunchKernelGGL(fill_kernel, dim3(grid_for(rows * cols, ctx->num_cu)), dim3(256), 0, ctx->stream, A, lda, rows,
                     cols, v);
  NK_HIP(hipGetLastError());
  return NK_OK;
}
int launch_frob_minus_identity(nk_ctx* ctx, const double* M, int64_t ldm, int n, double* d_out, const TnSkip* skip) {
  const ArenaMark mk = arena_mark(ctx);
  const int blocks = grid_for((int64_t)n * n, ctx->num_cu);
  double* partial = nullptr;
  NK_TRY(arena_alloc_t(ctx, (size_t)blocks, &partial));
  hipLaunchKernelGGL(frob_mi_partial_kernel, dim3(blocks), dim3(256), 0, ctx->stream, M, ldm, n, partial,
                     skip ? skip->state : nullptr, skip ? skip->step : 0);
  hipLaunchKernelGGL(sum_partials_kernel, dim3(1), dim3(256), 0, ctx->stream, partial, blocks, d_out);
  NK_HIP(hipGetLastError());
  arena_release(ctx, mk);
  return NK_OK;
}
int launch_max_abs_rowsum(nk_ctx* ctx, const double* M, int64_t ldm, int n, double* d_out) {
  const ArenaMark mk = arena_mark(ctx);
  double* rs = nullptr;
  NK_TRY(arena_alloc_t(ctx, (size_t)n, &rs));
  hipLaunchKernelGGL(abs_rowsum_kernel, dim3((n + 3) / 4), dim3(256), 0, ctx->stream, M, ldm, n, rs);
  hipLaunchKernelGGL(max_kernel, dim3(1), dim3(256), 0, ctx->stream, rs, n, d_out);
  NK_HIP(hipGetLastError());
  arena_release(ctx, mk);
  return NK_OK;
}
int launch_colsum_sqdiff(nk_ctx* ctx, const double* P, int64_t ldp, const double* Y, int64_t ldy, int64_t rows,
                         int cols, double* d_colsum) {
  const ArenaMark mk = arena_mark(ctx);
  const int rpb = 256;
  const int nslabs = (int)((rows + rpb - 1) / rpb);
  double* partial = nullptr;
  NK_TRY(arena_alloc_t(ctx, (size_t)nslabs * cols, &partial));
  hipLaunchKernelGGL(colsum_sqdiff_partial_kernel, dim3((cols + 63) / 64, nslabs), dim3(256), 0, ctx->stream, P, ldp, Y,
                     ldy, rows, cols, rpb, partial);
  hipLaunchKernelGGL(colsum_finish_kernel, dim3((cols + 255) / 256), dim3(256), 0, ctx->stream, partial, nslabs, cols,
                     d_colsum);
  NK_HIP(hipGetLastError());
  arena_release(ctx, mk);
  return NK_OK;
}

static int read_scalar(nk_ctx* ctx, const double* d_ptr, double* out) {
  NK_HIP(hipMemcpyAsync(ctx->h_scalars, d_ptr, sizeof(double), hipMemcpyDeviceToHost, ctx->stream));
  NK_HIP(hipStreamSynchronize(ctx->stream));
  *out = ctx->h_scalars[0];
  return NK_OK;
}

int sqrtm_spd_coupled(nk_ctx* ctx, const double* P, int64_t ldp, int m, double* S, double* Sinv, int* iters,
                      double* resid) {
  const ArenaMark mk = arena_mark(ctx);
  const size_t mm = (size_t)m * m;
  double *Y = nullptr, *Z = nullptr, *Yn = nullptr, *Zn = nullptr, *M = nullptr, *T = nullptr;
  double *Yt = nullptr, *Zt = nullptr, *Ytn = nullptr, *Ztn = nullptr;
  NK_TRY(arena_alloc_t(ctx, mm, &Y));
  NK_TRY(arena_alloc_t(ctx, mm, &Z));
  NK_TRY(arena_alloc_t(ctx, mm, &Yn));
  NK_TRY(arena_alloc_t(ctx, mm, &Zn));
  NK_TRY(arena_alloc_t(ctx, mm, &M));
  NK_TRY(arena_alloc_t(ctx, mm, &T));
  NK_TRY(arena_alloc_t(ctx, mm, &Yt));
  NK_TRY(arena_alloc_t(ctx, mm, &Zt));
  NK_TRY(arena_alloc_t(ctx, mm, &Ytn));
  NK_TRY(arena_alloc_t(ctx, mm, &Ztn));
  double c = 0.0;
  NK_TRY(launch_max_abs_rowsum(ctx, P, ldp, m, ctx->d_scalars));
  NK_TRY(read_scalar(ctx, ctx->d_scalars, &c));
  if (!(c > 0.0) || !std::isfinite(c)) {
    set_error("sqrtm: matrix norm is %g", c);
    arena_release(ctx, mk);
    return NK_ERR_NOT_SPD;
  }
  NK_TRY(launch_axpby2d(ctx, 1.0 / c, P, ldp, 0.0, Y, m, m, m));
  NK_TRY(launch_fill(ctx, Z, m, m, m, 0.0));
  NK_TRY(launch_add_diag(ctx, Z, m, m, 1.0));
  NK_TRY(launch_transpose(ctx, Y, m, Yt, m, m, m));
  NK_TRY(launch_copy2d(ctx, Z, m, Zt, m, m, m));
  double a_lo = 1.0, b_hi = 1.0;
  {
    const int blocks = grid_for((int64_t)m * m, ctx->num_cu);
    double* partial = nullptr;
    NK_TRY(arena_alloc_t(ctx, (size_t)2 * blocks, &partial));
    hipLaunchKernelGGL(sumsq_trace_partial_kernel, dim3(blocks), dim3(256), 0, ctx->stream, Y, (int64_t)m, m, partial,
                       blocks);
    hipLaunchKernelGGL(sum_partials_kernel, dim3(1), dim3(256), 0, ctx->stream, partial, blocks, ctx->d_scalars + 1);
    hipLaunchKernelGGL(sum_partials_kernel, dim3(1), dim3(256), 0, ctx->stream, partial + blocks, blocks,
                       ctx->d_scalars + 2);
    NK_HIP(hipGetLastError());
    NK_HIP(hipMemcpyAsync(ctx->h_scalars, ctx->d_scalars, 4 * sizeof(double), hipMemcpyDeviceToHost, ctx->stream));
    NK_HIP(hipStreamSynchronize(ctx->stream));
    const double fro = std::sqrt(ctx->h_scalars[1]), tr = ctx->h_scalars[2];
    const double lam1 = fro < 1.0 ? fro : 1.0;
    if (m > 1 && tr > lam1) a_lo = (tr - lam1) / (m - 1);
    else a_lo = tr / m * 1e-2;
    if (!(a_lo > 0.0) || !std::isfinite(a_lo)) a_lo = 1e-12;
    if (a_lo > 1.0) a_lo = 1.0;
  }
  auto p3 = [](double x) { return x * (3.0 - x) * (3.0 - x) * 0.25; };
  GemmOpts sym;
  sym.tri = TRI_UPPER_MIRROR;
  const int maxit = 100;
  double r = 1e300, r_prev = 1e300;
  int it = 0;
  bool ok = false;
  for (; it < maxit; ++it) {
    if (it == 0) {
      NK_TRY(launch_copy2d(ctx, Y, m, M, m, m, m));
      NK_TRY(launch_axpby2d(ctx, 0.5, Yt, m, 0.5, M, m, m, m));
    } else {
      NK_TRY(launch_gemm(ctx, true, false, m, m, m, 1.0, Zt, m, Y, m, 0.0, M, m, sym));
    }
    if (a_lo >= 0.5 || it + 1 == maxit) {
      NK_TRY(launch_frob_minus_identity(ctx, M, m, m, ctx->d_scalars));
      double r2 = 0.0;
      NK_TRY(read_scalar(ctx, ctx->d_scalars, &r2));
      r_prev = r;
      r = std::sqrt(r2 / m);
      if (!std::isfinite(r)) break;
      if (r < 5e-14 || r_prev < 1e-7) {
        ok = true;
        break;
      }
    }
    const double s2 = 3.0 / (a_lo + std::sqrt(a_lo * b_hi) + b_hi);
    const double sc = std::sqrt(s2);
    {
      const double xa = s2 * a_lo, xb = s2 * b_hi;
      const double lo = p3(xa) < p3(xb) ? p3(xa) : p3(xb);
      b_hi = (xa <= 1.0 && xb >= 1.0) ? 1.0 : (p3(xa) > p3(xb) ? p3(xa) : p3(xb));
      a_lo = lo < b_hi ? lo : b_hi;
    }
    NK_TRY(launch_scale_add_identity(ctx, -0.5 * s2 * sc, M, m, 1.5 * sc, T, m, m));
    {
      TnProblem pr[2];
      pr[0].A = Yt; pr[0].B = T; pr[0].C = Yn; pr[0].lda = pr[0].ldb = pr[0].ldc = m; pr[0].M = pr[0].N = m;
      pr[0].Ct = Ytn; pr[0].ldct = m;
      pr[1].A = T; pr[1].B = Z; pr[1].C = Zn; pr[1].lda = pr[1].ldb = pr[1].ldc = m; pr[1].M = pr[1].N = m;
      pr[1].Ct = Ztn; pr[1].ldct = m;
      if (it == 0) {
        if (tn_fast_ok(pr[0]) && m >= 128) {
          NK_TRY(launch_gemm_tn_multi(ctx, pr, 1, m, 0));
        } else {
          NK_TRY(launch_gemm(ctx, true, false, m, m, m, 1.0, Yt, m, T, m, 0.0, Yn, m));
          NK_TRY(launch_transpose(ctx, Yn, m, Ytn, m, m, m));
        }
        NK_TRY(launch_copy2d(ctx, T, m, Zn, m, m, m));
        NK_TRY(launch_copy2d(ctx, T, m, Ztn, m, m, m));
      } else if (tn_fast_ok(pr[0]) && tn_fast_ok(pr[1]) && m >= 128) {
        NK_TRY(launch_gemm_tn_multi(ctx, pr, 2, m, 0));
      } else {
        NK_TRY(launch_gemm(ctx, true, false, m, m, m, 1.0, Yt, m, T, m, 0.0, Yn, m));
        NK_TRY(launch_gemm(ctx, true, false, m, m, m, 1.0, T, m, Z, m, 0.0, Zn, m));
        NK_TRY(launch_transpose(ctx, Yn, m, Ytn, m, m, m));
        NK_TRY(launch_transpose(ctx, Zn, m, Ztn, m, m, m));
      }
    }
    double* t = Y; Y = Yn; Yn = t;
    t = Z; Z = Zn; Zn = t;
    t = Yt; Yt = Ytn; Ytn = t;
    t = Zt; Zt = Ztn; Ztn = t;
  }
  if (iters) *iters = it;
  if (resid) *resid = r;
  NK_TRY(x_align());
  if (!ok) {
    set_error("sqrtm: Newton-Schulz did not converge (residual %g after %d iterations)", r, it);
    arena_release(ctx, mk);
    return NK_ERR_NO_CONVERGENCE;
  }
  const double sc = std::sqrt(c);
  NK_TRY(launch_axpby2d(ctx, sc, Y, m, 0.0, S, m, m, m));
  NK_TRY(launch_axpby2d(ctx, 1.0 / sc, Z, m, 0.0, Sinv, m, m, m));
  arena_release(ctx, mk);
  return NK_OK;
}

int launch_potrf_diag_pair(nk_ctx* ctx, double* const* Ajj, const int64_t* lda, const int* nb, double* const* Linv,
                           int nsys, int blk, double* const* plog);

__device__ __forceinline__ void reset_pivots_kernel_body(int* info, unsigned long long* piv) {
  if (threadIdx.x < 4) piv[threadIdx.x] = (threadIdx.x & 1) ? 0ull : 0x7FF0000000000000ull;
  if (threadIdx.x < 2) info[threadIdx.x] = 0;
}
__global__ void __launch_bounds__(256) reset_pivots_kernel(int* info, unsigned long long* piv) { reset_pivots_kernel_body(info, piv); }
NK_BATCHED_TWIN(reset_pivots_kernel, (256), int*, unsigned long long*)
static int reset_pivots(nk_ctx* ctx) {
  hipLaunchKernelGGL(reset_pivots_kernel, dim3(1), dim3(64), 0, ctx->stream, ctx->d_info + info_base(ctx),
                     ctx->d_piv + 2 * info_base(ctx));
  NK_HIP(hipGetLastError());
  return NK_OK;
}

static void next_block(const CholSys* sys, int nsys, int jb, int* nbn, double** Lin, double** Pln) {
  constexpr int NB = CHOL_NB;
  const int j1 = (jb + 1) * NB;
  for (int q = 0; q < nsys; ++q) {
    const CholSys& y = sys[q];
    if (j1 >= y.m) continue;
    nbn[q] = y.m - j1 < NB ? y.m - j1 : NB;
    Lin[q] = y.Linv + (size_t)(jb + 1) * CHOL_WS;
    Pln[q] = y.pivlog ? y.pivlog + j1 : nullptr;
  }
}

int cholesky_lower_pair_async(nk_ctx* ctx, const CholSys* sys, int nsys) {
  constexpr int NB = CHOL_NB;
  NK_REQUIRE(nsys >= 1 && nsys <= 2, "cholesky_lower_pair: 1..2 systems");
  NK_TRY(reset_pivots(ctx));
  int nblk = 0;
  for (int q = 0; q < nsys; ++q) nblk = std::max(nblk, (sys[q].m + NB - 1) / NB);
  const bool fuse = chol_fuse_enabled();
  bool diag_done = false;
  for (int jb = 0; jb < nblk; ++jb) {
    const int j0 = jb * NB;
    double* Ajj[2] = {nullptr, nullptr};
    double* Li[2] = {nullptr, nullptr};
    double* Pl[2] = {nullptr, nullptr};
    int64_t lda[2] = {0, 0};
    int nbj[2] = {0, 0};
    GemmCall panel[2], trail[2];
    for (int q = 0; q < nsys; ++q) {
      const CholSys& y = sys[q];
      if (j0 >= y.m) continue;
      nbj[q] = y.m - j0 < NB ? y.m - j0 : NB;
      Ajj[q] = y.P + (int64_t)j0 * y.ldp + j0;
      lda[q] = y.ldp;
      Li[q] = y.Linv + (size_t)jb * CHOL_WS;
      Pl[q] = y.pivlog ? y.pivlog + j0 : nullptr;
      const int rem = y.m - j0 - nbj[q];
      if (rem > 0) {
        double* pnl = y.P + (int64_t)(j0 + nbj[q]) * y.ldp + j0;
        panel[q].M = rem; panel[q].N = nbj[q]; panel[q].K = nbj[q];
        panel[q].A = pnl; panel[q].lda = y.ldp; panel[q].B = Li[q]; panel[q].ldb = NB;
        panel[q].C = pnl; panel[q].ldc = y.ldp;
        trail[q].M = rem; trail[q].N = rem; trail[q].K = nbj[q]; trail[q].alpha = -1.0; trail[q].beta = 1.0;
        trail[q].A = pnl; trail[q].lda = y.ldp; trail[q].B = pnl; trail[q].ldb = y.ldp;
        trail[q].C = y.P + (int64_t)(j0 + nbj[q]) * y.ldp + (j0 + nbj[q]); trail[q].ldc = y.ldp;
        trail[q].opts.tri = TRI_LOWER;
      }
    }
    if (!diag_done) NK_TRY(launch_potrf_diag_pair(ctx, Ajj, lda, nbj, Li, nsys, jb, Pl));
    diag_done = false;
    {
      int rc_panel = NK_OK;
      if (!launch_chol_panel_pair(ctx, panel, nsys, &rc_panel)) NK_TRY(launch_gemm_pair(ctx, false, true, panel, nsys));
      NK_TRY(rc_panel);
    }
    if (fuse && jb + 1 < nblk) {
      int rc_f = NK_OK;
      int nbn[2] = {0, 0};
      double* Lin[2] = {nullptr, nullptr};
      double* Pln[2] = {nullptr, nullptr};
      next_block(sys, nsys, jb, nbn, Lin, Pln);
      if (launch_chol_trail_potrf_pair(ctx, trail, nsys, nbn, Lin, jb + 1, Pln, &rc_f)) {
        NK_TRY(rc_f);
        diag_done = true;
        continue;
      }
    }
    {
      int rc_trail = NK_OK;
      if (!launch_chol_trail_pair(ctx, trail, nsys, &rc_trail)) NK_TRY(launch_gemm_pair(ctx, false, true, trail, nsys));
      NK_TRY(rc_trail);
    }
  }
  return NK_OK;
}

int cholesky_check_pair(nk_ctx* ctx, const CholSys* sys, int nsys) {
  int failed[2] = {0, 0};
  NK_TRY(cholesky_fail_flags(ctx, sys, nsys, failed));
  for (int q = 0; q < nsys; ++q)
    if (failed[q] != 0) {
      if (failed[q] > 0)
        set_error("Cholesky: non-positive pivot at index %d of %d (system %d is numerically rank deficient; the "
                  "reference's lstsq would truncate here)", failed[q] - 1, sys[q].m, q);
      else
        set_error("Cholesky: system %d (order %d) has an isolated cluster of rounding-level pivots: an exact null space (the "
                  "reference's lstsq truncates it)", q, sys[q].m);
      return NK_ERR_NOT_SPD;
    }
  return NK_OK;
}

int cholesky_fail_flags(nk_ctx* ctx, const CholSys* sys, int nsys, int* failed, double* piv_ratio) {
  const int ib = info_base(ctx);
  std::vector<double> plog[2];
  NK_HIP(hipMemcpyAsync(ctx->h_info + ib, ctx->d_info + ib, 2 * sizeof(int), hipMemcpyDeviceToHost, ctx->stream));
  NK_HIP(hipMemcpyAsync(ctx->h_piv + 2 * ib, ctx->d_piv + 2 * ib, 4 * sizeof(unsigned long long), hipMemcpyDeviceToHost,
                        ctx->stream));
  for (int q = 0; q < nsys; ++q)
    if (sys[q].pivlog) {
      plog[q].resize((size_t)sys[q].m);
      NK_HIP(hipMemcpyAsync(plog[q].data(), sys[q].pivlog, sizeof(double) * sys[q].m, hipMemcpyDeviceToHost, ctx->stream));
    }
  NK_HIP(hipStreamSynchronize(ctx->stream));
  const double eps = 2.220446049250313e-16;
  for (int q = 0; q < nsys; ++q) {
    failed[q] = ctx->h_info[ib + q];
    if (piv_ratio) piv_ratio[q] = 0.0;
    if (failed[q] != 0) continue;
    double dmin, dmax;
    memcpy(&dmin, &ctx->h_piv[2 * (ib + q)], 8);
    memcpy(&dmax, &ctx->h_piv[2 * (ib + q) + 1], 8);
    if (!(dmax > 0.0)) continue;
    if (piv_ratio) piv_ratio[q] = dmin / dmax;
    if (dmin <= eps * dmax) { failed[q] = -1; continue; }
    if (plog[q].empty()) continue;
    std::sort(plog[q].begin(), plog[q].end());
    const double window = 8.0 * (double)sys[q].m * eps * dmax;
    size_t k = 0;
    while (k < plog[q].size() && plog[q][k] <= window) ++k;
    if (k > 0 && k < plog[q].size() && plog[q][k] >= 1000.0 * plog[q][k - 1]) failed[q] = -1;
  }
  return NK_OK;
}

int cholesky_lower_pair(nk_ctx* ctx, const CholSys* sys, int nsys) {
  NK_TRY(cholesky_lower_pair_async(ctx, sys, nsys));
  return cholesky_check_pair(ctx, sys, nsys);
}

int cholesky_aug_pair_async(nk_ctx* ctx, const CholSys* sys, int nsys, hipEvent_t pause, int pause_step) {
  constexpr int NB = CHOL_NB;
  NK_REQUIRE(nsys >= 1 && nsys <= 2, "cholesky_aug_pair: 1..2 systems");
  NK_TRY(reset_pivots(ctx));
  int nblk = 0;
  for (int q = 0; q < nsys; ++q) nblk = std::max(nblk, (sys[q].m + NB - 1) / NB);
  static const bool la_env = getenv("NYSKOOP_CHOL_LOOKAHEAD") && getenv("NYSKOOP_CHOL_LOOKAHEAD")[0] == '1';
  const int la = ctx->stream == ctx->stream_main ? 1 : -1;
  const bool lookahead = la_env && la >= 0 && nblk >= 4 && !ctx_recording(ctx);
  hipStream_t s_chain = ctx->stream;
  hipStream_t s_rest = lookahead ? ctx->stream_la[la] : ctx->stream;
  hipEvent_t* ev = lookahead ? ctx->ev_la[la] : nullptr;
  bool rest_pending = false;
  hipEvent_t last_rest = nullptr;
  if (lookahead) {
    NK_HIP(hipEventRecord(ev[1], s_chain));
    NK_HIP(hipStreamWaitEvent(s_rest, ev[1], 0));
  }
  const bool fuse = chol_fuse_enabled();
  bool diag_done = false;
  for (int jb = 0; jb < nblk; ++jb) {
    if (pause != nullptr && jb == pause_step) NK_HIP(hipStreamWaitEvent(ctx->stream, pause, 0));
    const int j0 = jb * NB;
    double* Ajj[2] = {nullptr, nullptr};
    double* Li[2] = {nullptr, nullptr};
    double* Pl[2] = {nullptr, nullptr};
    int64_t lda[2] = {0, 0};
    int nbj[2] = {0, 0};
    GemmCall panel[2], trail[2], next[2], rest[2];
    bool any_rest = false;
    for (int q = 0; q < nsys; ++q) {
      const CholSys& y = sys[q];
      if (j0 >= y.m) continue;
      nbj[q] = y.m - j0 < NB ? y.m - j0 : NB;
      Ajj[q] = y.P + (int64_t)j0 * y.ldp + j0;
      lda[q] = y.ldp;
      Li[q] = y.Linv + (size_t)jb * CHOL_WS;
      Pl[q] = y.pivlog ? y.pivlog + j0 : nullptr;
      const int rem = y.m - j0 - nbj[q];
      const int rows = rem + y.extra;
      if (rows > 0) {
        double* pnl = y.P + (int64_t)(j0 + nbj[q]) * y.ldp + j0;
        panel[q].M = rows; panel[q].N = nbj[q]; panel[q].K = nbj[q];
        panel[q].A = pnl; panel[q].lda = y.ldp; panel[q].B = Li[q]; panel[q].ldb = NB;
        panel[q].C = pnl; panel[q].ldc = y.ldp;
        if (rem > 0) {
          trail[q].M = rows; trail[q].N = rem; trail[q].K = nbj[q]; trail[q].alpha = -1.0; trail[q].beta = 1.0;
          trail[q].A = pnl; trail[q].lda = y.ldp; trail[q].B = pnl; trail[q].ldb = y.ldp;
          trail[q].C = y.P + (int64_t)(j0 + nbj[q]) * y.ldp + (j0 + nbj[q]); trail[q].ldc = y.ldp;
          trail[q].opts.tri = TRI_LOWER;
          const int nbn = rem < NB ? rem : NB;
          next[q] = trail[q];
          next[q].N = nbn;
          if (rem > nbn) {
            rest[q] = trail[q];
            rest[q].M = rows - nbn; rest[q].N = rem - nbn;
            rest[q].A = rest[q].B = pnl + (int64_t)nbn * y.ldp;
            rest[q].C = trail[q].C + (int64_t)nbn * y.ldp + nbn;
            any_rest = true;
          }
        }
      }
    }
    if (!diag_done) NK_TRY(launch_potrf_diag_pair(ctx, Ajj, lda, nbj, Li, nsys, jb, Pl));
    diag_done = false;
    {
      int rc_panel = NK_OK;
      if (!launch_chol_panel_pair(ctx, panel, nsys, &rc_panel)) NK_TRY(launch_gemm_pair(ctx, false, true, panel, nsys));
      NK_TRY(rc_panel);
    }
    if (fuse && !lookahead && jb + 1 < nblk) {
      int rc_f = NK_OK;
      int nbn[2] = {0, 0};
      double* Lin[2] = {nullptr, nullptr};
      double* Pln[2] = {nullptr, nullptr};
      next_block(sys, nsys, jb, nbn, Lin, Pln);
      if (launch_chol_trail_potrf_pair(ctx, trail, nsys, nbn, Lin, jb + 1, Pln, &rc_f)) {
        NK_TRY(rc_f);
        diag_done = true;
        continue;
      }
    }
    auto update = [&](const GemmCall* calls) -> int {
      int rc_trail = NK_OK;
      if (!launch_chol_trail_pair(ctx, calls, nsys, &rc_trail)) NK_TRY(launch_gemm_pair(ctx, false, true, calls, nsys));
      return rc_trail;
    };
    if (!lookahead) {
      NK_TRY(update(trail));
    } else {
      hipEvent_t evP = ev[jb & 1], evR = ev[2 + (jb & 1)], evR_prev = ev[2 + ((jb + 1) & 1)];
      NK_HIP(hipEventRecord(evP, s_chain));
      if (rest_pending) NK_HIP(hipStreamWaitEvent(s_chain, evR_prev, 0));
      NK_TRY(update(next));
      rest_pending = false;
      if (any_rest) {
        ctx->stream = s_rest;
        NK_HIP(hipStreamWaitEvent(s_rest, evP, 0));
        const int rc = update(rest);
        if (rc == NK_OK) NK_HIP(hipEventRecord(evR, s_rest));
        last_rest = evR;
        ctx->stream = s_chain;
        NK_TRY(rc);
        rest_pending = true;
      }
    }
  }
  if (lookahead && last_rest) NK_HIP(hipStreamWaitEvent(s_chain, last_rest, 0));
  NK_TRY(launch_trsm_right_lower_pair(ctx, sys, nsys));
  return NK_OK;
}

int cholesky_solve_pair(nk_ctx* ctx, const CholSys* sys, int nsys) {
  constexpr int NB = CHOL_NB;
  NK_REQUIRE(nsys >= 1 && nsys <= 2, "cholesky_solve_pair: 1..2 systems");
  int nblk = 0;
  for (int q = 0; q < nsys; ++q) nblk = std::max(nblk, (sys[q].m + NB - 1) / NB);
  const ArenaMark mk = arena_mark(ctx);
  double* tmp[2] = {nullptr, nullptr};
  for (int q = 0; q < nsys; ++q) NK_TRY(arena_alloc_t(ctx, (size_t)NB * sys[q].ldr, &tmp[q]));
  auto diag_solve = [&](int jb, bool trans) -> int {
    const int j0 = jb * NB;
    GemmCall g1[2], g2[2], g3[2];
    for (int q = 0; q < nsys; ++q) {
      const CholSys& y = sys[q];
      if (j0 >= y.m) continue;
      const int nbj = y.m - j0 < NB ? y.m - j0 : NB;
      const double* Li = y.Linv + (size_t)jb * CHOL_WS;
      const double* Ld = Li + NB * NB;
      double* Rj = y.R + (int64_t)j0 * y.ldr;
      NK_TRY(launch_copy2d(ctx, Rj, y.ldr, tmp[q], y.ldr, nbj, y.nrhs));
      g1[q].M = nbj; g1[q].N = y.nrhs; g1[q].K = nbj; g1[q].A = Li; g1[q].lda = NB; g1[q].B = tmp[q]; g1[q].ldb = y.ldr;
      g1[q].C = Rj; g1[q].ldc = y.ldr;
      g2[q] = g1[q]; g2[q].A = Ld; g2[q].B = Rj; g2[q].C = tmp[q]; g2[q].alpha = -1.0; g2[q].beta = 1.0;
      g3[q] = g1[q]; g3[q].beta = 1.0;
    }
    NK_TRY(launch_gemm_pair(ctx, trans, false, g1, nsys));
    NK_TRY(launch_gemm_pair(ctx, trans, false, g2, nsys));
    NK_TRY(launch_gemm_pair(ctx, trans, false, g3, nsys));
    return NK_OK;
  };
  for (int jb = 0; jb < nblk; ++jb) {
    const int j0 = jb * NB;
    GemmCall upd[2];
    for (int q = 0; q < nsys; ++q) {
      const CholSys& y = sys[q];
      if (j0 >= y.m) continue;
      const int nbj = y.m - j0 < NB ? y.m - j0 : NB;
      double* Rj = y.R + (int64_t)j0 * y.ldr;
      const int rem = y.m - j0 - nbj;
      if (rem > 0) {
        upd[q].M = rem; upd[q].N = y.nrhs; upd[q].K = nbj; upd[q].alpha = -1.0; upd[q].beta = 1.0;
        upd[q].A = y.P + (int64_t)(j0 + nbj) * y.ldp + j0; upd[q].lda = y.ldp; upd[q].B = Rj; upd[q].ldb = y.ldr;
        upd[q].C = y.R + (int64_t)(j0 + nbj) * y.ldr; upd[q].ldc = y.ldr;
      }
    }
    NK_TRY(diag_solve(jb, false));
    NK_TRY(launch_gemm_pair(ctx, false, false, upd, nsys));
  }
  for (int jb = nblk - 1; jb >= 0; --jb) {
    const int j0 = jb * NB;
    GemmCall upd[2];
    for (int q = 0; q < nsys; ++q) {
      const CholSys& y = sys[q];
      if (j0 >= y.m) continue;
      const int nbj = y.m - j0 < NB ? y.m - j0 : NB;
      double* Rj = y.R + (int64_t)j0 * y.ldr;
      if (j0 > 0) {
        upd[q].M = j0; upd[q].N = y.nrhs; upd[q].K = nbj; upd[q].alpha = -1.0; upd[q].beta = 1.0;
        upd[q].A = y.P + (int64_t)j0 * y.ldp; upd[q].lda = y.ldp; upd[q].B = Rj; upd[q].ldb = y.ldr;
        upd[q].C = y.R; upd[q].ldc = y.ldr;
      }
    }
    NK_TRY(diag_solve(jb, true));
    NK_TRY(launch_gemm_pair(ctx, true, false, upd, nsys));
  }
  arena_release(ctx, mk);
  return NK_OK;
}

int cholesky_lower(nk_ctx* ctx, double* P, int64_t ldp, int m, double* Linv) {
  CholSys y;
  y.P = P; y.ldp = ldp; y.m = m; y.Linv = Linv;
  return cholesky_lower_pair(ctx, &y, 1);
}

int cholesky_solve(nk_ctx* ctx, const double* L, int64_t ldl, int m, const double* Linv, double* R, int64_t ldr,
                   int nrhs) {
  CholSys y;
  y.P = const_cast<double*>(L); y.ldp = ldl; y.m = m; y.Linv = const_cast<double*>(Linv); y.R = R; y.ldr = ldr;
  y.nrhs = nrhs;
  return cholesky_solve_pair(ctx, &y, 1);
}

__device__ __forceinline__ void tri_scale_both_kernel_body(const double* __restrict__ L, int64_t ldl, int m, const double* __restrict__ d_c, double* __restrict__ Xt, double* __restrict__ X) {
  __shared__ double tile[32][33];
  const double s = 1.0 / sqrt(d_c[0]);
  const int bx = blockIdx.x * 32, by = blockIdx.y * 32;
  const int tx = threadIdx.x & 31, ty = threadIdx.x >> 5;
  for (int r = ty; r < 32; r += 8) {
    const int i = by + r, j = bx + tx;
    double v = 0.0;
    if (i < m && j <= i) v = L[(int64_t)i * ldl + j] * s;
    if (i < m && j < m) Xt[(int64_t)i * m + j] = v;
    tile[r][tx] = v;
  }
  __syncthreads();
  for (int r = ty; r < 32; r += 8) {
    const int i = bx + r, j = by + tx;
    if (i < m && j < m) X[(int64_t)i * m + j] = tile[tx][r];
  }
}
__global__ void __launch_bounds__(256) tri_scale_both_kernel(const double* __restrict__ L, int64_t ldl, int m, const double* __restrict__ d_c, double* __restrict__ Xt, double* __restrict__ X) { tri_scale_both_kernel_body(L, ldl, m, d_c, Xt, X); }
NK_BATCHED_TWIN(tri_scale_both_kernel, (256), const double*, int64_t, int, const double*, double*, double*)

int sqrtm_prepare(nk_ctx* ctx, const double* P, int64_t ldp, int m, SqrtPlan* plan) {
  plan->P = P; plan->ldp = ldp; plan->m = m;
  plan->mark = arena_mark(ctx);
  const size_t mm = (size_t)m * m;
  const int nblk = (m + CHOL_NB - 1) / CHOL_NB;
  NK_TRY(arena_alloc_t(ctx, 2 * mm, &plan->W));
  NK_TRY(arena_alloc_t(ctx, (size_t)nblk * CHOL_WS, &plan->Linv));
  NK_TRY(arena_alloc_t(ctx, mm, &plan->X0));
  NK_TRY(arena_alloc_t(ctx, mm, &plan->X0t));
  NK_TRY(arena_alloc_t(ctx, (size_t)8, &plan->d_sc));
  NK_TRY(launch_max_abs_rowsum(ctx, P, ldp, m, plan->d_sc));
  {
    const ArenaMark mk = arena_mark(ctx);
    const int blocks = grid_for((int64_t)m * m, ctx->num_cu);
    double* partial = nullptr;
    NK_TRY(arena_alloc_t(ctx, (size_t)2 * blocks, &partial));
    hipLaunchKernelGGL(sumsq_trace_partial_kernel, dim3(blocks), dim3(256), 0, ctx->stream, P, ldp, m, partial, blocks);
    hipLaunchKernelGGL(sum_partials_kernel, dim3(1), dim3(256), 0, ctx->stream, partial, blocks, plan->d_sc + 1);
    hipLaunchKernelGGL(sum_partials_kernel, dim3(1), dim3(256), 0, ctx->stream, partial + blocks, blocks, plan->d_sc + 2);
    NK_HIP(hipGetLastError());
    arena_release(ctx, mk);
  }
  NK_HIP(hipMemcpyAsync(ctx->h_scalars + 12, plan->d_sc, 3 * sizeof(double), hipMemcpyDeviceToHost, ctx->stream));
  NK_HIP(hipEventRecord(ctx->ev[11], ctx->stream));
  double* E = plan->W + mm;
  NK_TRY(launch_copy2d(ctx, P, ldp, plan->W, m, m, m));
  NK_TRY(launch_fill(ctx, E, m, m, m, 0.0));
  NK_TRY(launch_add_diag(ctx, E, m, m, 1.0));
  CholSys y;
  y.P = plan->W; y.ldp = m; y.m = m; y.extra = m; y.backward = false; y.Linv = plan->Linv;
  NK_TRY(cholesky_aug_pair_async(ctx, &y, 1, plan->pause_event, plan->pause_step));
  {
    const ArenaMark mk = arena_mark(ctx);
    const int blocks = grid_for((int64_t)m * m, ctx->num_cu);
    double* partial = nullptr;
    NK_TRY(arena_alloc_t(ctx, (size_t)2 * blocks, &partial));
    hipLaunchKernelGGL(sumsq_trace_partial_kernel, dim3(blocks), dim3(256), 0, ctx->stream, E, (int64_t)m, m, partial, blocks);
    hipLaunchKernelGGL(sum_partials_kernel, dim3(1), dim3(256), 0, ctx->stream, partial, blocks, plan->d_sc + 3);
    NK_HIP(hipGetLastError());
    arena_release(ctx, mk);
  }
  const int tb = (m + 31) / 32;
  hipLaunchKernelGGL(tri_scale_both_kernel, dim3(tb, tb), dim3(256), 0, ctx->stream, plan->W, (int64_t)m, m, plan->d_sc,
                     plan->X0t, plan->X0);
  NK_HIP(hipGetLastError());
  return NK_OK;
}

__device__ __forceinline__ void ns_flag_kernel_body(const double* __restrict__ partial, int count, int m, int step, double* __restrict__ state) {
  __shared__ double sh[4];
  double s = 0.0;
  for (int i = threadIdx.x; i < count; i += blockDim.x) s += partial[i];
  s = wave_sum(s);
  if ((threadIdx.x & 63) == 0) sh[threadIdx.x >> 6] = s;
  __syncthreads();
  if (threadIdx.x == 0) {
    const double r = sqrt((sh[0] + sh[1] + sh[2] + sh[3]) / m);
    state[2] = r;
    if (state[0] == 0.0 && r < 1e-7) {
      state[0] = (double)(step + 1);
      state[1] = r;
    }
  }
}
__global__ void __launch_bounds__(256) ns_flag_kernel(const double* __restrict__ partial, int count, int m, int step, double* __restrict__ state) { ns_flag_kernel_body(partial, count, m, step, state); }
NK_BATCHED_TWIN(ns_flag_kernel, (256), const double*, int, int, int, double*)

static int sqrtm_polar_products(nk_ctx* ctx, SqrtPlan* plan, const double* Q, double* scratch, double c, double* S,
                                double* Sinv, const double* Q_even = nullptr, const double* select = nullptr) {
  const int m = plan->m;
  const size_t mm = (size_t)m * m;
  double* Linv_full = scratch;
  NK_TRY(launch_transpose(ctx, plan->W + mm, m, Linv_full, m, m, m));
  TnProblem pr[2];
  pr[0].A = Q; pr[0].B = plan->X0; pr[0].C = S; pr[0].lda = pr[0].ldb = pr[0].ldc = m; pr[0].M = pr[0].N = m;
  pr[0].alpha = std::sqrt(c);
  pr[0].ktrim = KTRIM_B_UPPER;
  pr[1].ktrim = KTRIM_A_LOWER;
  pr[1].A = Linv_full; pr[1].B = Q; pr[1].C = Sinv; pr[1].lda = pr[1].ldb = pr[1].ldc = m; pr[1].M = pr[1].N = m;
  pr[0].A_even = Q_even;
  pr[1].B_even = Q_even;
  TnSkip sel;
  sel.select = select;
  if (tn_fast_ok(pr[0]) && tn_fast_ok(pr[1]) && m >= 128) {
    NK_TRY(launch_gemm_tn_multi(ctx, pr, 2, m, 0, nullptr, true, select ? &sel : nullptr));
  } else {
    NK_TRY(launch_gemm(ctx, true, false, m, m, m, pr[0].alpha, Q, m, plan->X0, m, 0.0, S, m));
    NK_TRY(launch_gemm(ctx, true, false, m, m, m, 1.0, Linv_full, m, Q, m, 0.0, Sinv, m));
  }
  return NK_OK;
}

int sqrtm_finish(nk_ctx* ctx, SqrtPlan* plan, double* S, double* Sinv) {
  const int m = plan->m;
  const size_t mm = (size_t)m * m;
  const int ib = info_base(ctx);
  plan->deferred = false;
  plan->rc = NK_OK; plan->iters = 0; plan->resid = 0.0;
  plan->early = plan->lambda_min_hint > 0.0 && m >= 1024 && m % 2 == 0;
  double c, sumsq, trace, linv2 = 0.0;
  if (plan->early) {
    NK_HIP(hipEventSynchronize(ctx->ev[11]));
    c = ctx->h_scalars[12]; sumsq = ctx->h_scalars[13]; trace = ctx->h_scalars[14];
    if (!(c > 0.0) || !std::isfinite(c)) plan->early = false;
  }
  if (!plan->early) {
    NK_HIP(hipMemcpyAsync(ctx->h_scalars, plan->d_sc, 4 * sizeof(double), hipMemcpyDeviceToHost, ctx->stream));
    NK_HIP(hipMemcpyAsync(ctx->h_info + ib, ctx->d_info + ib, sizeof(int), hipMemcpyDeviceToHost, ctx->stream));
    NK_HIP(hipStreamSynchronize(ctx->stream));
    c = ctx->h_scalars[0]; sumsq = ctx->h_scalars[1]; trace = ctx->h_scalars[2]; linv2 = ctx->h_scalars[3];
  }
  if (!plan->early &&
      (ctx->h_info[ib] != 0 || !(c > 0.0) || !std::isfinite(c) || !(linv2 > 0.0) || !std::isfinite(linv2))) {
    arena_release(ctx, plan->mark);
    plan->rc = sqrtm_spd_coupled(ctx, plan->P, plan->ldp, m, S, Sinv, &plan->iters, &plan->resid);
    return plan->rc;
  }
  double *Xa = nullptr, *Xta = nullptr, *Xb = nullptr, *Xtb = nullptr, *M = nullptr, *T = nullptr;
  NK_TRY(arena_alloc_t(ctx, mm, &Xa));
  NK_TRY(arena_alloc_t(ctx, mm, &Xta));
  NK_TRY(arena_alloc_t(ctx, mm, &Xb));
  NK_TRY(arena_alloc_t(ctx, mm, &Xtb));
  NK_TRY(arena_alloc_t(ctx, mm, &M));
  NK_TRY(arena_alloc_t(ctx, mm, &T));
  double a_lo = 1.0, b_hi = 1.0;
  {
    const double fro = std::sqrt(sumsq) / c, tr = trace / c;
    const double lam1 = fro < 1.0 ? fro : 1.0;
    if (m > 1 && tr > lam1) a_lo = (tr - lam1) / (m - 1);
    else a_lo = tr / m * 1e-2;
    if (!(a_lo > 0.0) || !std::isfinite(a_lo)) a_lo = 1e-12;
    if (a_lo > 1.0) a_lo = 1.0;
  }
  auto p3 = [](double x) { return x * (3.0 - x) * (3.0 - x) * 0.25; };
  auto advance = [&](double s2, double& a, double& b) {
    const double xa = s2 * a, xb = s2 * b;
    const double lo = p3(xa) < p3(xb) ? p3(xa) : p3(xb);
    b = (xa <= 1.0 && xb >= 1.0) ? 1.0 : (p3(xa) > p3(xb) ? p3(xa) : p3(xb));
    a = lo < b ? lo : b;
  };
  GemmOpts sym;
  sym.tri = TRI_UPPER_MIRROR;
  const double* X = plan->X0;
  const double* Xt = plan->X0t;
  double *Xn = Xa, *Xtn = Xta;
  TnProblem probe;
  probe.A = Xta; probe.B = T; probe.C = Xa; probe.lda = probe.ldb = probe.ldc = m; probe.M = probe.N = m;
  const bool fast = m >= 128 && tn_fast_ok(probe);
  const bool queued = fast && m >= 1024;
  if (plan->early && !queued) {
    set_error("sqrtm: internal: early queueing needs the LDS-DMA path");
    return NK_ERR_BAD_ARG;
  }

  if (queued) {
    double s2s[128];
    bool checks[128];
    int kmax = 0;
    {
      double ta = plan->early ? 0.9 * plan->lambda_min_hint / c : 0.5 / (c * linv2), tb = 1.0;
      if (ta > a_lo) ta = a_lo;
      const double a_sched = std::pow(a_lo, 0.8) * std::pow(ta, 0.2);
      double a = a_sched, b = b_hi;
      int kconv = -1;
      for (int k = 0; k < 100; ++k) {
        if (kconv < 0 && ta >= 1.0 - 1e-9 && tb <= 1.0 + 1e-9) kconv = k;
        checks[k] = a >= 0.5;
        const double s2 = 3.0 / (a + std::sqrt(a * b) + b);
        s2s[k] = s2;
        advance(s2, a, b);
        advance(s2, ta, tb);
        if (kconv >= 0 && k >= kconv + 1) { kmax = k + 1; break; }
      }
      if (kmax == 0) kmax = 100;
    }
    double* state = plan->d_sc + 5;
    NK_HIP(hipMemsetAsync(state, 0, 3 * sizeof(double), ctx->stream));
    double* rpart = nullptr;
    {
      const size_t mt = (size_t)(m + 127) / 128;
      const size_t need = std::max((size_t)grid_for((int64_t)m * m, ctx->num_cu), mt * (mt + 1) / 2 * 8);
      NK_TRY(arena_alloc_t(ctx, need, &rpart));
    }
    for (int k = 0; k < kmax; ++k) {
      TnSkip skip;
      skip.state = state; skip.step = k;
      int npart = 0;
      if (k == 0) {
        NK_TRY(launch_transpose(ctx, plan->P, plan->ldp, M, m, m, m));
        NK_TRY(launch_axpby2d(ctx, 0.5 / c, plan->P, plan->ldp, 0.5 / c, M, m, m, m));
      } else {
        const double s2k = s2s[k], sck = std::sqrt(s2k);
        TnProblem pm;
        pm.A = X; pm.B = X; pm.C = M; pm.lda = pm.ldb = pm.ldc = m; pm.M = pm.N = m; pm.tri = TRI_UPPER_MIRROR;
        pm.Caff = T; pm.aff_a = -0.5 * s2k * sck; pm.aff_c = 1.5 * sck;
        TnSkip skip_m = skip;
        skip_m.resid_partials = rpart; skip_m.resid_count = &npart;
        NK_TRY(launch_gemm_tn_multi(ctx, &pm, 1, m, 0, nullptr, true, &skip_m));
      }
      if (checks[k]) {
        if (npart == 0) {
          npart = grid_for((int64_t)m * m, ctx->num_cu);
          hipLaunchKernelGGL(frob_mi_partial_kernel, dim3(npart), dim3(256), 0, ctx->stream, M, (int64_t)m, m, rpart,
                             skip.state, skip.step);
        }
        hipLaunchKernelGGL(ns_flag_kernel, dim3(1), dim3(256), 0, ctx->stream, rpart, npart, m, k, state);
        NK_HIP(hipGetLastError());
      }
      if (k == 0) {
        const double s2 = s2s[0], sc = std::sqrt(s2);
        NK_TRY(launch_scale_add_identity(ctx, -0.5 * s2 * sc, M, m, 1.5 * sc, T, m, m, &skip));
      }
      TnProblem pr;
      pr.A = Xt; pr.B = T; pr.C = Xn; pr.lda = pr.ldb = pr.ldc = m; pr.M = pr.N = m; pr.Ct = Xtn; pr.ldct = m;
      NK_TRY(launch_gemm_tn_multi(ctx, &pr, 1, m, 1, nullptr, true, &skip));
      X = Xn; Xt = Xtn;
      Xn = (Xn == Xa) ? Xb : Xa;
      Xtn = (Xtn == Xta) ? Xtb : Xta;
    }
    NK_TRY(sqrtm_polar_products(ctx, plan, Xa, T, c, S, Sinv, Xb, state));
    NK_HIP(hipMemcpyAsync(ctx->h_scalars + 8, state, 3 * sizeof(double), hipMemcpyDeviceToHost, ctx->stream));
    if (plan->early)
      NK_HIP(hipMemcpyAsync(ctx->h_info + ib, ctx->d_info + ib, sizeof(int), hipMemcpyDeviceToHost, ctx->stream));
    plan->deferred = true;
    plan->kmax = kmax;
    arena_release(ctx, plan->mark);
    return NK_OK;
  }

  const int maxit = 100;
  double r = 1e300;
  int it = 0;
  bool ok = false;
  for (; it < maxit; ++it) {
    if (it == 0) {
      NK_TRY(launch_transpose(ctx, plan->P, plan->ldp, M, m, m, m));
      NK_TRY(launch_axpby2d(ctx, 0.5 / c, plan->P, plan->ldp, 0.5 / c, M, m, m, m));
    } else {
      NK_TRY(launch_gemm(ctx, true, false, m, m, m, 1.0, X, m, X, m, 0.0, M, m, sym));
    }
    const bool check = a_lo >= 0.5 || it + 2 >= maxit;
    if (check) {
      NK_TRY(launch_frob_minus_identity(ctx, M, m, m, ctx->d_scalars));
      NK_HIP(hipMemcpyAsync(ctx->h_scalars, ctx->d_scalars, sizeof(double), hipMemcpyDeviceToHost, ctx->stream));
      NK_HIP(hipEventRecord(ctx->ev[10], ctx->stream));
    }
    const double s2 = 3.0 / (a_lo + std::sqrt(a_lo * b_hi) + b_hi);
    const double sc = std::sqrt(s2);
    advance(s2, a_lo, b_hi);
    NK_TRY(launch_scale_add_identity(ctx, -0.5 * s2 * sc, M, m, 1.5 * sc, T, m, m));
    if (fast) {
      TnProblem pr;
      pr.A = Xt; pr.B = T; pr.C = Xn; pr.lda = pr.ldb = pr.ldc = m; pr.M = pr.N = m; pr.Ct = Xtn; pr.ldct = m;
      NK_TRY(launch_gemm_tn_multi(ctx, &pr, 1, m, 0));
    } else {
      NK_TRY(launch_gemm(ctx, true, false, m, m, m, 1.0, Xt, m, T, m, 0.0, Xn, m));
      NK_TRY(launch_transpose(ctx, Xn, m, Xtn, m, m, m));
    }
    X = Xn; Xt = Xtn;
    Xn = (Xn == Xa) ? Xb : Xa;
    Xtn = (Xtn == Xta) ? Xtb : Xta;
    if (check) {
      NK_HIP(hipEventSynchronize(ctx->ev[10]));
      r = std::sqrt(ctx->h_scalars[0] / m);
      if (!std::isfinite(r)) break;
      if (r < 1e-7) {
        ok = true;
        ++it;
        break;
      }
    }
  }
  plan->iters = it;
  plan->resid = r;
  NK_TRY(x_align());
  if (!ok) {
    set_error("sqrtm: Newton-Schulz did not converge (residual %g after %d iterations)", r, it);
    arena_release(ctx, plan->mark);
    plan->rc = NK_ERR_NO_CONVERGENCE;
    return plan->rc;
  }
  NK_TRY(sqrtm_polar_products(ctx, plan, X, T, c, S, Sinv));
  arena_release(ctx, plan->mark);
  return NK_OK;
}

int sqrtm_verdict(nk_ctx* ctx, SqrtPlan* plan, int* iters, double* resid) {
  if (plan->deferred) {
    const double flag = ctx->h_scalars[8];
    plan->deferred = false;
    if (plan->early && (ctx->h_info[2] != 0 || flag == 0.0 || !std::isfinite(ctx->h_scalars[10]))) {
      plan->iters = plan->kmax;
      plan->resid = ctx->h_scalars[10];
      plan->rc = NK_SQRT_RETRY;
    } else if (flag == 0.0 || !std::isfinite(ctx->h_scalars[10])) {
      plan->iters = plan->kmax;
      plan->resid = ctx->h_scalars[10];
      plan->rc = NK_ERR_NO_CONVERGENCE;
      set_error("sqrtm: Newton-Schulz did not converge (residual %g after %d iterations)", plan->resid, plan->kmax);
    } else {
      plan->iters = (int)flag;
      plan->resid = ctx->h_scalars[9];
      plan->rc = NK_OK;
    }
  }
  if (iters) *iters = plan->iters;
  if (resid) *resid = plan->resid;
  return plan->rc;
}

int sqrtm_spd(nk_ctx* ctx, const double* P, int64_t ldp, int m, double* S, double* Sinv, int* iters, double* resid) {
  SqrtPlan plan;
  NK_TRY(sqrtm_prepare(ctx, P, ldp, m, &plan));
  NK_TRY(sqrtm_finish(ctx, &plan, S, Sinv));
  NK_HIP(hipStreamSynchronize(ctx->stream));
  return sqrtm_verdict(ctx, &plan, iters, resid);
}

}
```

nys_koop_lqr_amd/csrc/nk_potrf_body.h:

```cpp
#pragma once
#include "nk_common.h"

namespace nk {

typedef double d4 __attribute__((ext_vector_type(4)));

__device__ __forceinline__ double readlane_f64(double v, int lane) {
  const int lo = __builtin_amdgcn_readlane(__double2loint(v), lane);
  const int hi = __builtin_amdgcn_readlane(__double2hiint(v), lane);
  return __hiloint2double(hi, lo);
}

struct PotrfBatch {
  double* A[2];
  int64_t lda[2];
  int nb[2];
  double* Linv[2];
  int* info[2];
  unsigned long long* piv[2];
  double* plog[2];
};

constexpr int PLD = CHOL_NB + 1;
constexpr int SLD = 17;

template <bool NEG>
__device__ __forceinline__ d4 mm16(const double* P, int ldp, const double* Q, int ldq, d4 acc, int l15, int l4) {
#pragma unroll
  for (int ks = 0; ks < 4; ++ks) {
    double a = P[l15 * ldp + 4 * ks + l4];
    const double b = Q[(4 * ks + l4) * ldq + l15];
    if (NEG) a = -a;
    acc = __builtin_amdgcn_mfma_f64_16x16x4f64(a, b, acc, 0, 0, 0);
  }
  return acc;
}
__device__ __forceinline__ void store_tile(double* T, int ldt, d4 acc, int l15, int l4) {
#pragma unroll
  for (int reg = 0; reg < 4; ++reg) T[(l4 + 4 * reg) * ldt + l15] = acc[reg];
}

__device__ __forceinline__ void potrf_diag_kernel_body(const PotrfBatch& pb, int blk, int which, int lane) {
  constexpr int NB = CHOL_NB;
  static_assert(NB == 64, "one lane per row, four 16-column panels");
  const int nb = pb.nb[which];
  if (nb <= 0) return;
  __builtin_amdgcn_s_setprio(3);
  double* __restrict__ A = pb.A[which];
  const int64_t lda = pb.lda[which];
  double* __restrict__ Linv = pb.Linv[which];
  int* __restrict__ info = pb.info[which];
  double* __restrict__ plog = pb.plog[which];
  double piv_min = 1.0e308, piv_max = 0.0;
  __shared__ double As[NB * PLD];
  __shared__ double Iv[NB * PLD];
  __shared__ double Sc[3 * 16 * SLD];
  __shared__ double dinv[NB];
  const int l15 = lane & 15, l4 = lane >> 4;
#pragma unroll 8
  for (int r = 0; r < NB; ++r) {
    double v = (r == lane) ? 1.0 : 0.0;
    if (r < nb && lane < nb) v = A[(int64_t)r * lda + lane];
    As[r * PLD + lane] = v;
  }
  __syncthreads();

#pragma unroll
  for (int pbk = 0; pbk < 4; ++pbk) {
    const int c0 = 16 * pbk;
    double R[16];
#pragma unroll
    for (int jj = 0; jj < 16; ++jj) R[jj] = As[lane * PLD + c0 + jj];
#pragma unroll
    for (int k = 0; k < 16; ++k) {
      double dkk = readlane_f64(R[k], c0 + k);
      if (lane == 0 && plog != nullptr && c0 + k < nb) plog[c0 + k] = dkk;
      if (!(dkk > 0.0) || !isfinite(dkk)) {
        if (lane == 0 && c0 + k < nb) atomicCAS(info, 0, blk * NB + c0 + k + 1);
        dkk = 1.0;
      } else if (c0 + k < nb) {
        piv_min = fmin(piv_min, dkk);
        piv_max = fmax(piv_max, dkk);
      }
      double inv = __builtin_amdgcn_rsq(dkk);
      inv = inv * fma(-0.5 * dkk * inv, inv, 1.5);
      inv = inv * fma(-0.5 * dkk * inv, inv, 1.5);
      double s = dkk * inv;
      s = fma(0.5 * inv, fma(-s, s, dkk), s);
      inv = fma(inv, fma(-s, inv, 1.0), inv);
      if (lane == c0 + k) dinv[c0 + k] = inv;
      R[k] = (lane == c0 + k) ? s : R[k] * inv;
      {
        const int rk_lo = __double2loint(R[k]), rk_hi = __double2hiint(R[k]);
#pragma unroll
        for (int jj = k + 1; jj < 16; ++jj)
          asm volatile("v_readlane_b32 s96, %1, %3\n\tv_readlane_b32 s97, %2, %3\n\ts_nop 0\n\tv_fma_f64 %0, -%4, s[96:97], %0"
                       : "+v"(R[jj])
                       : "v"(rk_lo), "v"(rk_hi), "i"(c0 + jj), "v"(R[k])
                       : "s96", "s97");
      }
    }
#pragma unroll
    for (int jj = 0; jj < 16; ++jj) As[lane * PLD + c0 + jj] = R[jj];
    __syncthreads();
#pragma unroll
    for (int ti = pbk + 1; ti < 4; ++ti)
#pragma unroll
      for (int tj = pbk + 1; tj <= ti; ++tj) {
        d4 c;
#pragma unroll
        for (int reg = 0; reg < 4; ++reg) c[reg] = As[(16 * ti + l4 + 4 * reg) * PLD + 16 * tj + l15];
#pragma unroll
        for (int ks = 0; ks < 4; ++ks) {
          const double a = -As[(16 * ti + l15) * PLD + c0 + 4 * ks + l4];
          const double b = As[(16 * tj + l15) * PLD + c0 + 4 * ks + l4];
          c = __builtin_amdgcn_mfma_f64_16x16x4f64(a, b, c, 0, 0, 0);
        }
#pragma unroll
        for (int reg = 0; reg < 4; ++reg) As[(16 * ti + l4 + 4 * reg) * PLD + 16 * tj + l15] = c[reg];
      }
    __syncthreads();
  }
#pragma unroll 8
  for (int r = 0; r < NB; ++r)
    if (r < nb && lane < nb) A[(int64_t)r * lda + lane] = As[r * PLD + lane];

  {
    const double* Lb = As + (16 * l4) * PLD + 16 * l4;
    double x[16];
#pragma unroll
    for (int i = 0; i < 16; ++i) {
      double s0 = (i == l15) ? 1.0 : 0.0, s1 = 0.0;
#pragma unroll
      for (int j = 0; j < i; ++j) {
        const double l = Lb[i * PLD + j];
        if ((j & 1) == 0) s0 = fma(-l, x[j], s0);
        else s1 = fma(-l, x[j], s1);
      }
      x[i] = (s0 + s1) * dinv[16 * l4 + i];
    }
    double* Db = Iv + (16 * l4) * PLD + 16 * l4;
#pragma unroll
    for (int i = 0; i < 16; ++i) Db[i * PLD + l15] = x[i];
  }
  __syncthreads();
  auto Lblk = [&](int i, int j) { return As + (16 * i) * PLD + 16 * j; };
  auto Xblk = [&](int i, int j) { return Iv + (16 * i) * PLD + 16 * j; };
  const d4 zero = d4{0.0, 0.0, 0.0, 0.0};
#pragma unroll
  for (int i = 1; i < 4; ++i)
    store_tile(Sc + (i - 1) * 16 * SLD, SLD, mm16<false>(Lblk(i, i - 1), PLD, Xblk(i - 1, i - 1), PLD, zero, l15, l4), l15, l4);
  __syncthreads();
#pragma unroll
  for (int i = 1; i < 4; ++i)
    store_tile(Xblk(i, i - 1), PLD, mm16<true>(Xblk(i, i), PLD, Sc + (i - 1) * 16 * SLD, SLD, zero, l15, l4), l15, l4);
  __syncthreads();
#pragma unroll
  for (int i = 2; i < 4; ++i) {
    d4 t = mm16<false>(Lblk(i, i - 2), PLD, Xblk(i - 2, i - 2), PLD, zero, l15, l4);
    t = mm16<false>(Lblk(i, i - 1), PLD, Xblk(i - 1, i - 2), PLD, t, l15, l4);
    store_tile(Sc + (i - 2) * 16 * SLD, SLD, t, l15, l4);
  }
  __syncthreads();
#pragma unroll
  for (int i = 2; i < 4; ++i)
    store_tile(Xblk(i, i - 2), PLD, mm16<true>(Xblk(i, i), PLD, Sc + (i - 2) * 16 * SLD, SLD, zero, l15, l4), l15, l4);
  __syncthreads();
  {
    d4 t = mm16<false>(Lblk(3, 0), PLD, Xblk(0, 0), PLD, zero, l15, l4);
    t = mm16<false>(Lblk(3, 1), PLD, Xblk(1, 0), PLD, t, l15, l4);
    t = mm16<false>(Lblk(3, 2), PLD, Xblk(2, 0), PLD, t, l15, l4);
    store_tile(Sc, SLD, t, l15, l4);
  }
  __syncthreads();
  store_tile(Xblk(3, 0), PLD, mm16<true>(Xblk(3, 3), PLD, Sc, SLD, zero, l15, l4), l15, l4);
  __syncthreads();
#pragma unroll 8
  for (int i = 0; i < NB; ++i) Linv[i * NB + lane] = (l4 <= (i >> 4)) ? Iv[i * PLD + lane] : 0.0;
  double sl = 0.0, si = 0.0;
#pragma unroll 8
  for (int i = 0; i < NB; ++i) {
    const double vl = (lane <= i) ? As[i * PLD + lane] : 0.0;
    const double vi = (l4 <= (i >> 4)) ? Iv[i * PLD + lane] : 0.0;
    Linv[NB * NB + i * NB + lane] = vl;
    sl = fma(vl, vl, sl);
    si = fma(vi, vi, si);
  }
#pragma unroll
  for (int off = 32; off > 0; off >>= 1) {
    sl += __shfl_xor(sl, off, 64);
    si += __shfl_xor(si, off, 64);
  }
  if (lane == 0) Linv[2 * NB * NB] = (sl * si > CHOL_FIX_KAPPA * CHOL_FIX_KAPPA) ? 1.0 : 0.0;
  if (lane == 0 && piv_max > 0.0) {
    atomicMin(pb.piv[which], (unsigned long long)__double_as_longlong(piv_min));
    atomicMax(pb.piv[which] + 1, (unsigned long long)__double_as_longlong(piv_max));
  }
}
}
```

nys_koop_lqr_amd/csrc/nk_trail.hip:

```cpp
#include "nk_common.h"
#include "nk_potrf_body.h"

namespace nk {


struct TrailSys {
  const double* P;
  int64_t ldp;
  double* C;
  int64_t ldc;
  int rows, rem;
  int tiles_n;
  int nblocks;
};
struct TrailBatch {
  TrailSys s[2];
};

__device__ __forceinline__ void chol_trail_kernel_body(const TrailBatch& tb) {
  const TrailSys s = tb.s[blockIdx.y];
  if ((int)blockIdx.x >= s.nblocks) return;
  __builtin_amdgcn_s_setprio(2);
  int tm = 0, tn = 0;
  {
    int rem = blockIdx.x;
    for (;;) {
      const int cnt = tm + 1 < s.tiles_n ? tm + 1 : s.tiles_n;
      if (rem < cnt) break;
      rem -= cnt;
      ++tm;
    }
    tn = rem;
  }
  const int lane = threadIdx.x & 63;
  const int wave = __builtin_amdgcn_readfirstlane(threadIdx.x >> 6);
  const int wm = wave >> 1, wn = wave & 1;
  const int l15 = lane & 15, l4 = lane >> 4;
  const int m0 = tm * 128 + wm * 64, n0 = tn * 128 + wn * 64;

  d4 acc[4][4];
#pragma unroll
  for (int i = 0; i < 4; ++i)
#pragma unroll
    for (int j = 0; j < 4; ++j) acc[i][j] = d4{0.0, 0.0, 0.0, 0.0};

  const double* pa[4];
  const double* pb[4];
#pragma unroll
  for (int i = 0; i < 4; ++i) {
    pa[i] = s.P + (int64_t)min(m0 + 16 * i + l15, s.rows - 1) * s.ldp + 8 * l4;
    pb[i] = s.P + (int64_t)min(n0 + 16 * i + l15, s.rem - 1) * s.ldp + 8 * l4;
  }
#pragma unroll
  for (int h = 0; h < 2; ++h) {
    double a[4][8], b[4][8];
#pragma unroll
    for (int i = 0; i < 4; ++i)
#pragma unroll
      for (int ks = 0; ks < 8; ++ks) {
        a[i][ks] = pa[i][32 * h + ks];
        b[i][ks] = pb[i][32 * h + ks];
      }
#pragma unroll
    for (int ks = 0; ks < 8; ++ks)
#pragma unroll
      for (int i = 0; i < 4; ++i)
#pragma unroll
        for (int j = 0; j < 4; ++j) acc[i][j] = __builtin_amdgcn_mfma_f64_16x16x4f64(a[i][ks], b[j][ks], acc[i][j], 0, 0, 0);
  }
#pragma unroll
  for (int i = 0; i < 4; ++i)
#pragma unroll
    for (int j = 0; j < 4; ++j)
#pragma unroll
      for (int reg = 0; reg < 4; ++reg) {
        const int row = m0 + 16 * i + l4 + 4 * reg;
        const int col = n0 + 16 * j + l15;
        if (row < s.rows && col < s.rem) {
          double* c = s.C + (int64_t)row * s.ldc + col;
          *c -= acc[i][j][reg];
        }
      }
}
__global__ void __launch_bounds__(256) chol_trail_kernel(TrailBatch tb) { chol_trail_kernel_body(tb); }
__global__ void __launch_bounds__(256) chol_trail_kernel_batched(const nk::ArgPack<TrailBatch>* table) { chol_trail_kernel_body(table[blockIdx.z].v); }
static nk::TwinReg chol_trail_kernel_twin_reg(reinterpret_cast<const void*>(static_cast<void (*)(TrailBatch)>(chol_trail_kernel)),
                                 reinterpret_cast<const void*>(chol_trail_kernel_batched), sizeof(nk::ArgPack<TrailBatch>), "chol_trail_kernel");

bool launch_chol_trail_pair(nk_ctx* ctx, const GemmCall* calls, int ncalls, int* rc);

__device__ __forceinline__ void chol_trail_potrf_kernel_body(const TrailBatch& tb, const PotrfBatch& pb, int blk) {
  chol_trail_kernel_body(tb);
  if (blockIdx.x == 0 && __builtin_amdgcn_readfirstlane(threadIdx.x >> 6) == 0 && pb.nb[blockIdx.y] > 0) {
    __threadfence();
    potrf_diag_kernel_body(pb, blk, blockIdx.y, threadIdx.x & 63);
  }
}
__global__ void __launch_bounds__(256) chol_trail_potrf_kernel(TrailBatch tb, PotrfBatch pb, int blk) { chol_trail_potrf_kernel_body(tb, pb, blk); }
__global__ void __launch_bounds__(256) chol_trail_potrf_kernel_batched(const nk::ArgPack<TrailBatch, PotrfBatch, int>* table) {
  chol_trail_potrf_kernel_body(table[blockIdx.z].v, table[blockIdx.z].rest.v, table[blockIdx.z].rest.rest.v);
}
static nk::TwinReg chol_trail_potrf_twin_reg(reinterpret_cast<const void*>(static_cast<void (*)(TrailBatch, PotrfBatch, int)>(chol_trail_potrf_kernel)),
                                             reinterpret_cast<const void*>(chol_trail_potrf_kernel_batched),
                                             sizeof(nk::ArgPack<TrailBatch, PotrfBatch, int>), "chol_trail_potrf_kernel");

static bool fill_trail_batch(const GemmCall* calls, int ncalls, TrailBatch& tb, int& maxblocks) {
  maxblocks = 0;
  for (int q = 0; q < 2; ++q) {
    TrailSys& t = tb.s[q];
    t = TrailSys{};
    if (q >= ncalls || calls[q].M <= 0 || calls[q].N <= 0) continue;
    const GemmCall& c = calls[q];
    if (c.K != 64 || c.A != c.B || c.lda != c.ldb || c.alpha != -1.0 || c.beta != 1.0 || c.opts.tri != TRI_LOWER ||
        c.M < c.N)
      return false;
    t.P = c.A; t.ldp = c.lda; t.C = c.C; t.ldc = c.ldc; t.rows = (int)c.M; t.rem = (int)c.N;
    t.tiles_n = (t.rem + 127) / 128;
    const int tiles_m = (t.rows + 127) / 128;
    t.nblocks = t.tiles_n * (t.tiles_n + 1) / 2 + (tiles_m - t.tiles_n) * t.tiles_n;
    if (t.nblocks > maxblocks) maxblocks = t.nblocks;
  }
  return true;
}

bool launch_chol_trail_pair(nk_ctx* ctx, const GemmCall* calls, int ncalls, int* rc) {
  *rc = NK_OK;
  TrailBatch tb;
  int maxblocks = 0;
  if (!fill_trail_batch(calls, ncalls, tb, maxblocks)) return false;
  if (maxblocks == 0) return true;
  hipLaunchKernelGGL(chol_trail_kernel, dim3((unsigned)maxblocks, 2), dim3(256), 0, ctx->stream, tb);
  if (hipGetLastError() != hipSuccess) {
    set_error("chol_trail launch failed");
    *rc = NK_ERR_HIP;
  }
  return true;
}

bool launch_chol_trail_potrf_pair(nk_ctx* ctx, const GemmCall* calls, int ncalls, const int* nb, double* const* Linv, int blk,
                                  double* const* plog, int* rc) {
  *rc = NK_OK;
  TrailBatch tb;
  int maxblocks = 0;
  if (!fill_trail_batch(calls, ncalls, tb, maxblocks) || maxblocks == 0) return false;
  PotrfBatch pb;
  for (int q = 0; q < 2; ++q) {
    const bool on = q < ncalls && nb[q] > 0 && tb.s[q].nblocks > 0;
    if (q < ncalls && nb[q] > 0 && tb.s[q].nblocks == 0) return false;
    pb.A[q] = on ? tb.s[q].C : nullptr;
    pb.lda[q] = on ? tb.s[q].ldc : 0;
    pb.nb[q] = on ? nb[q] : 0;
    pb.Linv[q] = on ? Linv[q] : nullptr;
    pb.info[q] = ctx->d_info + info_base(ctx) + q;
    pb.piv[q] = ctx->d_piv + 2 * (info_base(ctx) + q);
    pb.plog[q] = (on && plog) ? plog[q] : nullptr;
  }
  hipLaunchKernelGGL(chol_trail_potrf_kernel, dim3((unsigned)maxblocks, 2), dim3(256), 0, ctx->stream, tb, pb, blk);
  if (hipGetLastError() != hipSuccess) {
    set_error("chol_trail_potrf launch failed");
    *rc = NK_ERR_HIP;
  }
  return true;
}

constexpr int PANEL_ROWS = 64;
struct PanelSys {
  double* P;
  int64_t ldp;
  const double* Linv;
  int rows;
  int nb;
  int fix;
  int nblocks;
};
struct PanelBatch {
  PanelSys s[2];
};

__device__ __forceinline__ void chol_panel_kernel_body(const PanelBatch& pb) {
  const PanelSys s = pb.s[blockIdx.y];
  if ((int)blockIdx.x >= s.nblocks) return;
  __builtin_amdgcn_s_setprio(2);
  const int lane = threadIdx.x & 63;
  const int wave = __builtin_amdgcn_readfirstlane(threadIdx.x >> 6);
  const int l15 = lane & 15, l4 = lane >> 4;
  const int m0 = blockIdx.x * PANEL_ROWS + wave * 16;
  const int nb = s.nb;
  const double* __restrict__ Li = s.Linv;
  const double* __restrict__ Ld = s.Linv + CHOL_NB * CHOL_NB;
  double a[16];
  {
    const double* pr = s.P + (int64_t)min(m0 + l15, s.rows - 1) * s.ldp + l4;
    if (nb == CHOL_NB) {
#pragma unroll
      for (int t = 0; t < 16; ++t) a[t] = pr[4 * t];
    } else {
#pragma unroll
      for (int t = 0; t < 16; ++t) a[t] = (4 * t + l4 < nb) ? pr[4 * t] : 0.0;
    }
  }
  double li[4][16];
#pragma unroll
  for (int j = 0; j < 4; ++j)
#pragma unroll
    for (int t = 0; t < 16; ++t) li[j][t] = Li[(16 * j + l15) * CHOL_NB + 4 * t + l4];
  d4 p1[4];
#pragma unroll
  for (int j = 0; j < 4; ++j) p1[j] = d4{0.0, 0.0, 0.0, 0.0};
#pragma unroll
  for (int t = 0; t < 16; ++t)
#pragma unroll
    for (int j = 0; j < 4; ++j) p1[j] = __builtin_amdgcn_mfma_f64_16x16x4f64(li[j][t], a[t], p1[j], 0, 0, 0);
  if (s.fix == 2 || (s.fix == 1 && s.Linv[2 * CHOL_NB * CHOL_NB] != 0.0)) {
    d4 rs[4];
#pragma unroll
    for (int j = 0; j < 4; ++j) rs[j] = d4{a[4 * j], a[4 * j + 1], a[4 * j + 2], a[4 * j + 3]};
#pragma unroll
    for (int t = 0; t < 16; ++t)
#pragma unroll
      for (int j = 0; j < 4; ++j)
        rs[j] = __builtin_amdgcn_mfma_f64_16x16x4f64(-Ld[(16 * j + l15) * CHOL_NB + 4 * t + l4], p1[t >> 2][t & 3], rs[j], 0, 0, 0);
    d4 p2[4];
#pragma unroll
    for (int j = 0; j < 4; ++j) p2[j] = p1[j];
#pragma unroll
    for (int t = 0; t < 16; ++t)
#pragma unroll
      for (int j = 0; j < 4; ++j) p2[j] = __builtin_amdgcn_mfma_f64_16x16x4f64(li[j][t], rs[t >> 2][t & 3], p2[j], 0, 0, 0);
#pragma unroll
    for (int j = 0; j < 4; ++j) p1[j] = p2[j];
  }
  __syncthreads();
  const int row = m0 + l15;
  if (row < s.rows) {
    double* pw = s.P + (int64_t)row * s.ldp + l4;
#pragma unroll
    for (int j = 0; j < 4; ++j)
#pragma unroll
      for (int reg = 0; reg < 4; ++reg)
        if (nb == CHOL_NB || 16 * j + 4 * reg + l4 < nb) pw[16 * j + 4 * reg] = p1[j][reg];
  }
}
__global__ void __launch_bounds__(256) chol_panel_kernel(PanelBatch pb) { chol_panel_kernel_body(pb); }
__global__ void __launch_bounds__(256) chol_panel_kernel_batched(const nk::ArgPack<PanelBatch>* table) { chol_panel_kernel_body(table[blockIdx.z].v); }
static nk::TwinReg chol_panel_kernel_twin_reg(reinterpret_cast<const void*>(static_cast<void (*)(PanelBatch)>(chol_panel_kernel)),
                                 reinterpret_cast<const void*>(chol_panel_kernel_batched), sizeof(nk::ArgPack<PanelBatch>), "chol_panel_kernel");

bool launch_chol_panel_pair(nk_ctx* ctx, const GemmCall* calls, int ncalls, int* rc) {
  *rc = NK_OK;
  PanelBatch pb;
  int maxblocks = 0;
  for (int q = 0; q < 2; ++q) {
    PanelSys& t = pb.s[q];
    t = PanelSys{};
    if (q >= ncalls || calls[q].M <= 0 || calls[q].N <= 0) continue;
    const GemmCall& c = calls[q];
    if (c.K != c.N || c.N > 64 || c.A != c.C || c.lda != c.ldc || c.ldb != 64 || c.alpha != 1.0 || c.beta != 0.0) return false;
    t.P = c.C; t.ldp = c.ldc; t.Linv = c.B; t.rows = (int)c.M; t.nb = (int)c.N; t.fix = chol_fix_enabled();
    t.nblocks = (t.rows + PANEL_ROWS - 1) / PANEL_ROWS;
    if (t.nblocks > maxblocks) maxblocks = t.nblocks;
  }
  if (maxblocks == 0) return true;
  hipLaunchKernelGGL(chol_panel_kernel, dim3((unsigned)maxblocks, 2), dim3(256), 0, ctx->stream, pb);
  if (hipGetLastError() != hipSuccess) {
    set_error("chol_panel launch failed");
    *rc = NK_ERR_HIP;
  }
  return true;
}

}
```

Measured before the change: 23.63.

## Add persistent dataflow Cholesky kernel with tile flags replacing blocked launch chain

Adds a persistent kernel that factors both Cholesky systems with a single launch. Work items (diagonal potrf, panel solves, trailing updates) are claimed from an atomic counter, and per-tile ready flags in global memory order the dependencies. This replaces the many small per-block kernel launches and their serialization with overlapped tile-level execution. If polling exceeds its limit the kernel gives up and the host reruns the old chain path. The panel body is factored into a shared header, and a wave-level sync variant of potrf is added for single-wave use.

```diff
diff --git a/nys_koop_lqr_amd/csrc/nk_api.hip b/nys_koop_lqr_amd/csrc/nk_api.hip
--- a/nys_koop_lqr_amd/csrc/nk_api.hip
+++ b/nys_koop_lqr_amd/csrc/nk_api.hip
@@ -437,6 +437,7 @@
   (void)hipStreamDestroy(ctx->stream_prep);
   (void)hipStreamDestroy(ctx->stream_copy);
   (void)hipFree(ctx->d_info);
+  for (int i = 0; i < 2; ++i) if (ctx->d_flow[i]) (void)hipFree(ctx->d_flow[i]);
   (void)hipFree(ctx->d_scalars);
   if (ctx->d_zeros) (void)hipFree(ctx->d_zeros);
   if (ctx->h_stage) (void)hipHostFree(ctx->h_stage);
@@ -1251,8 +1252,16 @@
   double piv_ratio[2] = {1.0, 1.0};
   NK_TRY(cholesky_fail_flags(ctx, sys, 2, chol_failed, piv_ratio));
   tr.mark("final sync");
+  bool chol_rerun = false;
+  if (chol_failed[0] == CHOL_FLOW_GIVEUP || chol_failed[1] == CHOL_FLOW_GIVEUP) {
+    ChainOnly chain(ctx);
+    NK_HIP(hipMemcpyAsync(G1, Gsave, gram_doubles(m, d, p) * sizeof(double), hipMemcpyDeviceToDevice, ctx->stream));
+    NK_TRY(cholesky_aug_pair_async(ctx, sys, 2));
+    NK_TRY(cholesky_fail_flags(ctx, sys, 2, chol_failed, piv_ratio));
+    chol_rerun = true;
+  }
   int rank_sys[2] = {mp, m};
-  bool redo_products = false;
+  bool redo_products = chol_rerun;
   if (ctx->strict_spd == 2) chol_failed[0] = chol_failed[1] = -1;
   if (chol_failed[0] || chol_failed[1]) {
     if (ctx->strict_spd == 1) {
@@ -1315,7 +1324,12 @@
   }
   {
     const int vr = sqrtm_verdict(ctx, &splan, &it, &resid);
-    if (vr == NK_SQRT_RETRY) {
+    if (vr == NK_SQRT_RETRY && splan.flow_gave_up) {
+      ChainOnly chain(ctx);
+      NK_TRY(sqrtm_spd(ctx, Kj, m, m, mdl->S, mdl->Sinv, &it, &resid));
+      NK_TRY(sqrt_products());
+      redo_products = true;
+    } else if (vr == NK_SQRT_RETRY) {
       count_event(CNT_SQRT_RETRY);
       NK_TRY(sqrtm_spd_coupled(ctx, Kj, m, m, mdl->S, mdl->Sinv, &it, &resid));
       NK_TRY(sqrt_products());
diff --git a/nys_koop_lqr_amd/csrc/nk_chol_flow.hip b/nys_koop_lqr_amd/csrc/nk_chol_flow.hip
--- /dev/null
+++ b/nys_koop_lqr_amd/csrc/nk_chol_flow.hip
@@ -0,0 +1,329 @@
+#include "nk_common.h"
+#include "nk_panel_body.h"
+#include "nk_potrf_body.h"
+
+namespace nk {
+
+namespace {
+
+constexpr int FLOW_THREADS = 256;
+constexpr int FLOW_HDR = 16;
+constexpr int FLOW_POLL_LIMIT = 1 << 22;
+
+struct FlowSys {
+  double* P;
+  int64_t ldp;
+  int m, extra;
+  double* Linv;
+  double* pivlog;
+  int* info;
+  unsigned long long* piv;
+  int* flags;
+  int nblk;
+  int nex;
+};
+struct FlowArgs {
+  FlowSys s[2];
+  int nsys;
+  int total;
+  int fix;
+  int* hdr;
+};
+
+__device__ __forceinline__ int ld_flag(const int* f) { return __hip_atomic_load(f, __ATOMIC_RELAXED, __HIP_MEMORY_SCOPE_AGENT); }
+
+__device__ __forceinline__ int col_items(const FlowSys& s, int c) {
+  if (c < 0 || c >= s.nblk) return 0;
+  return max(0, s.nblk - c - 2) + s.nex;
+}
+
+__device__ void item_of(const FlowArgs& a, int t, int& q, int& i, int& k) {
+  for (int g = 0;; ++g) {
+    for (int p = 0; p < a.nsys; ++p)
+      if (g < a.s[p].nblk) {
+        if (t == 0) { q = p; i = k = g; return; }
+        --t;
+      }
+    for (int p = 0; p < a.nsys; ++p) {
+      const int n = col_items(a.s[p], g - 1);
+      if (t < n) {
+        q = p; k = g - 1;
+        const int nsq = max(0, a.s[p].nblk - k - 2);
+        i = t < nsq ? k + 2 + t : a.s[p].nblk + (t - nsq);
+        return;
+      }
+      t -= n;
+    }
+  }
+}
+
+__device__ __forceinline__ void tile_rows(const FlowSys& s, int i, int& r0, int& r1) {
+  if (i < s.nblk) { r0 = CHOL_NB * i; r1 = min(r0 + CHOL_NB, s.m); }
+  else { r0 = s.m + CHOL_NB * (i - s.nblk); r1 = min(r0 + CHOL_NB, s.m + s.extra); }
+}
+
+typedef d4 Quarter[2][2];
+
+__device__ __forceinline__ void load_quarter(const FlowSys& s, int r0, int r1, int c0, int c1, int wm, int wn, int l15, int l4,
+                                             Quarter& C) {
+#pragma unroll
+  for (int a = 0; a < 2; ++a)
+#pragma unroll
+    for (int b = 0; b < 2; ++b)
+#pragma unroll
+      for (int reg = 0; reg < 4; ++reg) {
+        const int row = r0 + 32 * wm + 16 * a + l4 + 4 * reg, col = c0 + 32 * wn + 16 * b + l15;
+        C[a][b][reg] = (row < r1 && col < c1) ? s.P[(int64_t)row * s.ldp + col] : 0.0;
+      }
+}
+__device__ __forceinline__ void store_quarter(const FlowSys& s, int r0, int r1, int c0, int c1, int wm, int wn, int l15, int l4,
+                                              const Quarter& C) {
+#pragma unroll
+  for (int a = 0; a < 2; ++a)
+#pragma unroll
+    for (int b = 0; b < 2; ++b)
+#pragma unroll
+      for (int reg = 0; reg < 4; ++reg) {
+        const int row = r0 + 32 * wm + 16 * a + l4 + 4 * reg, col = c0 + 32 * wn + 16 * b + l15;
+        if (row < r1 && col < c1) s.P[(int64_t)row * s.ldp + col] = C[a][b][reg];
+      }
+}
+
+__device__ __forceinline__ void update_quarter(const FlowSys& s, int r0, int r1, int c0, int c1, int j, int wm, int wn, int l15,
+                                               int l4, Quarter& C) {
+  const double* pa[2];
+  const double* pb[2];
+#pragma unroll
+  for (int a = 0; a < 2; ++a) {
+    pa[a] = s.P + (int64_t)min(r0 + 32 * wm + 16 * a + l15, r1 - 1) * s.ldp + CHOL_NB * j + 8 * l4;
+    pb[a] = s.P + (int64_t)min(c0 + 32 * wn + 16 * a + l15, c1 - 1) * s.ldp + CHOL_NB * j + 8 * l4;
+  }
+  d4 acc[2][2];
+#pragma unroll
+  for (int a = 0; a < 2; ++a)
+#pragma unroll
+    for (int b = 0; b < 2; ++b) acc[a][b] = d4{0.0, 0.0, 0.0, 0.0};
+#pragma unroll
+  for (int h = 0; h < 2; ++h) {
+    double x[2][8], y[2][8];
+#pragma unroll
+    for (int a = 0; a < 2; ++a)
+#pragma unroll
+      for (int ks = 0; ks < 8; ++ks) {
+        x[a][ks] = pa[a][32 * h + ks];
+        y[a][ks] = pb[a][32 * h + ks];
+      }
+#pragma unroll
+    for (int ks = 0; ks < 8; ++ks)
+#pragma unroll
+      for (int a = 0; a < 2; ++a)
+#pragma unroll
+        for (int b = 0; b < 2; ++b) acc[a][b] = __builtin_amdgcn_mfma_f64_16x16x4f64(x[a][ks], y[b][ks], acc[a][b], 0, 0, 0);
+  }
+#pragma unroll
+  for (int a = 0; a < 2; ++a)
+#pragma unroll
+    for (int b = 0; b < 2; ++b)
+#pragma unroll
+      for (int reg = 0; reg < 4; ++reg) C[a][b][reg] -= acc[a][b][reg];
+  asm volatile("" ::: "memory");
+}
+
+__device__ __forceinline__ void give_up(const FlowArgs& a) {
+  __hip_atomic_store(a.hdr + 1, 1, __ATOMIC_RELAXED, __HIP_MEMORY_SCOPE_AGENT);
+  for (int q = 0; q < a.nsys; ++q) atomicExch(a.s[q].info, CHOL_FLOW_GIVEUP);
+}
+
+__device__ int wait_tiles(const FlowArgs& a, const FlowSys& s, int ia, int ib, int jlo, int jhi, int* sh) {
+  if (threadIdx.x < 64) {
+    const int lane = threadIdx.x;
+    int res = -1;
+    for (int polls = 0;; ++polls) {
+      const int j = jlo + lane;
+      bool ok = true;
+      if (j < jhi) {
+        ok = ld_flag(s.flags + ia * s.nblk + j) != 0;
+        if (ib >= 0) ok = ok && ld_flag(s.flags + ib * s.nblk + j) != 0;
+      }
+      const unsigned long long ready = __ballot(ok);
+      const int run = ~ready == 0ull ? 64 : __builtin_ctzll(~ready);
+      if (run > 0) { res = min(jlo + run, jhi); break; }
+      if (ld_flag(a.hdr + 1) != 0) break;
+      if (polls >= FLOW_POLL_LIMIT) {
+        if (lane == 0) give_up(a);
+        break;
+      }
+      __builtin_amdgcn_s_sleep(2);
+    }
+    if (lane == 0) {
+      if (res > 0) __builtin_amdgcn_fence(__ATOMIC_ACQUIRE, "agent");
+      asm volatile("s_waitcnt vmcnt(0)" ::: "memory");
+      sh[0] = res;
+    }
+  }
+  __syncthreads();
+  const int r = sh[0];
+  __syncthreads();
+  return r;
+}
+
+__device__ __forceinline__ void publish(const FlowSys& s, int i, int k) {
+  asm volatile("s_waitcnt vmcnt(0)" ::: "memory");
+  __syncthreads();
+  if (threadIdx.x == 0) {
+    __builtin_amdgcn_fence(__ATOMIC_RELEASE, "agent");
+    asm volatile("s_waitcnt vmcnt(0)" ::: "memory");
+    __hip_atomic_store(s.flags + i * s.nblk + k, 1, __ATOMIC_RELAXED, __HIP_MEMORY_SCOPE_AGENT);
+  }
+}
+
+__device__ __forceinline__ void local_sync() {
+  asm volatile("s_waitcnt vmcnt(0)" ::: "memory");
+  __syncthreads();
+}
+
+__device__ __forceinline__ void panel_tile(const FlowArgs& a, const FlowSys& s, int r0, int r1, int k, int wave, int lane) {
+  PanelSys ps;
+  ps.P = s.P + (int64_t)r0 * s.ldp + CHOL_NB * k;
+  ps.ldp = s.ldp;
+  ps.Linv = s.Linv + (size_t)k * CHOL_WS;
+  ps.rows = r1 - r0;
+  ps.nb = min(CHOL_NB, s.m - CHOL_NB * k);
+  ps.fix = a.fix;
+  ps.nblocks = 1;
+  chol_panel_rows(ps, 16 * wave, lane);
+  __builtin_amdgcn_s_setprio(0);
+}
+
+__device__ __noinline__ void flow_potrf(double* A, int64_t lda, int nb, double* Linv, int* info, unsigned long long* piv,
+                                       double* plog, int blk, int lane) {
+  PotrfBatch pb;
+  pb.A[0] = A; pb.lda[0] = lda; pb.nb[0] = nb; pb.Linv[0] = Linv; pb.info[0] = info; pb.piv[0] = piv; pb.plog[0] = plog;
+  pb.A[1] = nullptr; pb.lda[1] = 0; pb.nb[1] = 0; pb.Linv[1] = nullptr; pb.info[1] = nullptr; pb.piv[1] = nullptr;
+  pb.plog[1] = nullptr;
+  potrf_diag_kernel_body<true>(pb, blk, 0, lane);
+  __builtin_amdgcn_s_setprio(0);
+}
+
+__global__ void __launch_bounds__(FLOW_THREADS) chol_flow_kernel(FlowArgs a) {
+  __shared__ int sh[4];
+  const int lane = threadIdx.x & 63;
+  const int wave = __builtin_amdgcn_readfirstlane(threadIdx.x >> 6);
+  const int wm = wave >> 1, wn = wave & 1;
+  const int l15 = lane & 15, l4 = lane >> 4;
+  for (;;) {
+    if (threadIdx.x == 0) sh[1] = atomicAdd(a.hdr, 1);
+    __syncthreads();
+    const int t = sh[1];
+    __syncthreads();
+    if (t >= a.total) return;
+    int q = 0, i = 0, k = 0;
+    item_of(a, t, q, i, k);
+    const FlowSys s = q ? a.s[1] : a.s[0];
+    int r0, r1;
+    tile_rows(s, i, r0, r1);
+    const int c0 = CHOL_NB * k, c1 = min(c0 + CHOL_NB, s.m);
+    if (i == k) {
+      if (k > 0) {
+        const int p0 = c0 - CHOL_NB;
+        Quarter Cp, Cd;
+        load_quarter(s, r0, r1, p0, c0, wm, wn, l15, l4, Cp);
+        load_quarter(s, r0, r1, c0, c1, wm, wn, l15, l4, Cd);
+        bool ok = true;
+        for (int j = 0; j < k - 1 && ok;) {
+          const int J = wait_tiles(a, s, k, k - 1, j, k - 1, sh);
+          if (J < 0) { ok = false; break; }
+          for (; j < J; ++j) {
+            update_quarter(s, r0, r1, p0, c0, j, wm, wn, l15, l4, Cp);
+            update_quarter(s, r0, r1, c0, c1, j, wm, wn, l15, l4, Cd);
+          }
+        }
+        if (!ok) continue;
+        store_quarter(s, r0, r1, p0, c0, wm, wn, l15, l4, Cp);
+        store_quarter(s, r0, r1, c0, c1, wm, wn, l15, l4, Cd);
+        local_sync();
+        if (wait_tiles(a, s, k - 1, -1, k - 1, k, sh) < 0) continue;
+        panel_tile(a, s, r0, r1, k - 1, wave, lane);
+        publish(s, k, k - 1);
+        __syncthreads();
+        load_quarter(s, r0, r1, c0, c1, wm, wn, l15, l4, Cd);
+        update_quarter(s, r0, r1, c0, c1, k - 1, wm, wn, l15, l4, Cd);
+        store_quarter(s, r0, r1, c0, c1, wm, wn, l15, l4, Cd);
+        local_sync();
+      }
+      if (wave == 0)
+        flow_potrf(s.P + (int64_t)c0 * s.ldp + c0, s.ldp, c1 - c0, s.Linv + (size_t)k * CHOL_WS, s.info, s.piv,
+                   s.pivlog ? s.pivlog + c0 : nullptr, k, lane);
+      publish(s, k, k);
+      __syncthreads();
+    } else {
+      if (k > 0) {
+        Quarter C;
+        load_quarter(s, r0, r1, c0, c1, wm, wn, l15, l4, C);
+        bool ok = true;
+        for (int j = 0; j < k && ok;) {
+          const int J = wait_tiles(a, s, i, k, j, k, sh);
+          if (J < 0) { ok = false; break; }
+          for (; j < J; ++j) update_quarter(s, r0, r1, c0, c1, j, wm, wn, l15, l4, C);
+        }
+        if (!ok) continue;
+        store_quarter(s, r0, r1, c0, c1, wm, wn, l15, l4, C);
+        local_sync();
+      }
+      if (wait_tiles(a, s, k, -1, k, k + 1, sh) < 0) continue;
+      panel_tile(a, s, r0, r1, k, wave, lane);
+      publish(s, i, k);
+      __syncthreads();
+    }
+  }
+}
+
+}
+
+bool chol_flow_enabled() {
+  const char* e = getenv("NYSKOOP_CHOL_FLOW");
+  return !(e && e[0] == '0');
+}
+
+int cholesky_flow_pair(nk_ctx* ctx, const CholSys* sys, int nsys) {
+  constexpr int NB = CHOL_NB;
+  NK_REQUIRE(nsys >= 1 && nsys <= 2, "cholesky_flow_pair: 1..2 systems");
+  FlowArgs a;
+  memset(&a, 0, sizeof(a));
+  a.nsys = nsys;
+  a.fix = chol_fix_enabled();
+  size_t words = FLOW_HDR;
+  for (int q = 0; q < nsys; ++q) {
+    const CholSys& y = sys[q];
+    FlowSys& s = a.s[q];
+    s.P = y.P; s.ldp = y.ldp; s.m = y.m; s.extra = y.extra; s.Linv = y.Linv; s.pivlog = y.pivlog;
+    s.info = ctx->d_info + info_base(ctx) + q;
+    s.piv = ctx->d_piv + 2 * (info_base(ctx) + q);
+    s.nblk = (y.m + NB - 1) / NB;
+    s.nex = (y.extra + NB - 1) / NB;
+    words += (size_t)(s.nblk + s.nex) * s.nblk;
+    for (int c = 0; c < s.nblk; ++c) a.total += 1 + std::max(0, s.nblk - c - 2) + s.nex;
+  }
+  const int slot = info_base(ctx) / 2;
+  if (ctx->flow_words[slot] < words) {
+    if (ctx->d_flow[slot]) NK_HIP(hipFree(ctx->d_flow[slot]));
+    ctx->d_flow[slot] = nullptr;
+    ctx->flow_words[slot] = 0;
+    NK_HIP(hipMalloc(reinterpret_cast<void**>(&ctx->d_flow[slot]), words * sizeof(int)));
+    ctx->flow_words[slot] = words;
+  }
+  a.hdr = ctx->d_flow[slot];
+  int* f = a.hdr + FLOW_HDR;
+  for (int q = 0; q < nsys; ++q) {
+    a.s[q].flags = f;
+    f += (size_t)(a.s[q].nblk + a.s[q].nex) * a.s[q].nblk;
+  }
+  NK_HIP(hipMemsetAsync(a.hdr, 0, words * sizeof(int), ctx->stream));
+  const int grid = std::max(1, std::min(a.total, ctx->num_cu / 2));
+  hipLaunchKernelGGL(chol_flow_kernel, dim3((unsigned)grid), dim3(FLOW_THREADS), 0, ctx->stream, a);
+  NK_HIP(hipGetLastError());
+  count_event(CNT_CHOL_FLOW);
+  return NK_OK;
+}
+
+}
diff --git a/nys_koop_lqr_amd/csrc/nk_common.h b/nys_koop_lqr_amd/csrc/nk_common.h
--- a/nys_koop_lqr_amd/csrc/nk_common.h
+++ b/nys_koop_lqr_amd/csrc/nk_common.h
@@ -83,6 +83,9 @@
   hipEvent_t ev_up[8] = {};
   nk_group* group = nullptr;
   nk_member_state* gstate = nullptr;
+  int* d_flow[2] = {nullptr, nullptr};
+  size_t flow_words[2] = {0, 0};
+  bool chol_flow_off = false;
   double* h_stage = nullptr;
   size_t h_stage_bytes = 0;
 };
@@ -115,6 +118,13 @@
     c->stream = s0;
     c->cur_arena = a0;
   }
+};
+
+struct ChainOnly {
+  nk_ctx* c;
+  bool b0;
+  explicit ChainOnly(nk_ctx* ctx) : c(ctx), b0(ctx->chol_flow_off) { c->chol_flow_off = true; }
+  ~ChainOnly() { c->chol_flow_off = b0; }
 };
 
 inline int info_base(const nk_ctx* c) { return c->stream != c->stream_main ? 2 : 0; }
@@ -152,7 +162,8 @@
 int group_enter(nk_ctx* c);
 int group_leave(nk_ctx* c);
 void group_stats(nk_ctx* c, uint64_t out[4]);
-enum { CNT_CHAIN_GIVEUP = 0, CNT_JACOBI_GIVEUP = 1, CNT_RANK_TRUNCATED = 2, CNT_SQRT_RETRY = 3, CNT_REFINED = 4, CNT_N = 5 };
+enum { CNT_CHAIN_GIVEUP = 0, CNT_JACOBI_GIVEUP = 1, CNT_RANK_TRUNCATED = 2, CNT_SQRT_RETRY = 3, CNT_REFINED = 4,
+       CNT_CHOL_FLOW_GIVEUP = 5, CNT_CHOL_FLOW = 6, CNT_N = 7 };
 void count_event(int which);
 uint64_t read_counter(int which);
 hipError_t real_stream_sync(hipStream_t s);
@@ -221,6 +232,7 @@
   double resid = 0.0;
   double lambda_min_hint = 0.0;
   bool early = false;
+  bool flow_gave_up = false;
   hipEvent_t pause_event = nullptr;
   int pause_step = -1;
 };
@@ -263,6 +275,9 @@
   const char* e = getenv("NYSKOOP_CHOL_FUSE");
   return !(e && e[0] == '0');
 }
+bool chol_flow_enabled();
+int cholesky_flow_pair(nk_ctx* ctx, const CholSys* sys, int nsys);
+constexpr int CHOL_FLOW_GIVEUP = -0x40000000;
 bool launch_chol_panel_pair(nk_ctx* ctx, const GemmCall* calls, int ncalls, int* rc);
 int launch_trsm_right_lower_pair(nk_ctx* ctx, const CholSys* sys, int nsys);
 
diff --git a/nys_koop_lqr_amd/csrc/nk_linalg.hip b/nys_koop_lqr_amd/csrc/nk_linalg.hip
--- a/nys_koop_lqr_amd/csrc/nk_linalg.hip
+++ b/nys_koop_lqr_amd/csrc/nk_linalg.hip
@@ -642,6 +642,10 @@
   for (int q = 0; q < nsys; ++q) {
     failed[q] = ctx->h_info[ib + q];
     if (piv_ratio) piv_ratio[q] = 0.0;
+    if (failed[q] == CHOL_FLOW_GIVEUP) {
+      if (q == 0) count_event(CNT_CHOL_FLOW_GIVEUP);
+      continue;
+    }
     if (failed[q] != 0) continue;
     double dmin, dmax;
     memcpy(&dmin, &ctx->h_piv[2 * (ib + q)], 8);
@@ -668,8 +672,17 @@
   constexpr int NB = CHOL_NB;
   NK_REQUIRE(nsys >= 1 && nsys <= 2, "cholesky_aug_pair: 1..2 systems");
   NK_TRY(reset_pivots(ctx));
-  int nblk = 0;
-  for (int q = 0; q < nsys; ++q) nblk = std::max(nblk, (sys[q].m + NB - 1) / NB);
+  int nblk = 0, mmin = sys[0].m;
+  for (int q = 0; q < nsys; ++q) {
+    nblk = std::max(nblk, (sys[q].m + NB - 1) / NB);
+    mmin = std::min(mmin, sys[q].m);
+  }
+  if (!ctx->chol_flow_off && mmin >= 256 && !ctx_recording(ctx) && chol_flow_enabled()) {
+    if (pause != nullptr && pause_step >= 0 && pause_step < nblk) NK_HIP(hipStreamWaitEvent(ctx->stream, pause, 0));
+    NK_TRY(cholesky_flow_pair(ctx, sys, nsys));
+    NK_TRY(launch_trsm_right_lower_pair(ctx, sys, nsys));
+    return NK_OK;
+  }
   static const bool la_env = getenv("NYSKOOP_CHOL_LOOKAHEAD") && getenv("NYSKOOP_CHOL_LOOKAHEAD")[0] == '1';
   const int la = ctx->stream == ctx->stream_main ? 1 : -1;
   const bool lookahead = la_env && la >= 0 && nblk >= 4 && !ctx_recording(ctx);
@@ -990,6 +1003,16 @@
     NK_HIP(hipStreamSynchronize(ctx->stream));
     c = ctx->h_scalars[0]; sumsq = ctx->h_scalars[1]; trace = ctx->h_scalars[2]; linv2 = ctx->h_scalars[3];
   }
+  if (!plan->early && ctx->h_info[ib] == CHOL_FLOW_GIVEUP) {
+    count_event(CNT_CHOL_FLOW_GIVEUP);
+    arena_release(ctx, plan->mark);
+    ChainOnly chain(ctx);
+    SqrtPlan again;
+    NK_TRY(sqrtm_prepare(ctx, plan->P, plan->ldp, m, &again));
+    const int rc = sqrtm_finish(ctx, &again, S, Sinv);
+    *plan = again;
+    return rc;
+  }
   if (!plan->early &&
       (ctx->h_info[ib] != 0 || !(c > 0.0) || !std::isfinite(c) || !(linv2 > 0.0) || !std::isfinite(linv2))) {
     arena_release(ctx, plan->mark);
@@ -1170,6 +1193,8 @@
     const double flag = ctx->h_scalars[8];
     plan->deferred = false;
     if (plan->early && (ctx->h_info[2] != 0 || flag == 0.0 || !std::isfinite(ctx->h_scalars[10]))) {
+      plan->flow_gave_up = ctx->h_info[2] == CHOL_FLOW_GIVEUP;
+      if (plan->flow_gave_up) count_event(CNT_CHOL_FLOW_GIVEUP);
       plan->iters = plan->kmax;
       plan->resid = ctx->h_scalars[10];
       plan->rc = NK_SQRT_RETRY;
diff --git a/nys_koop_lqr_amd/csrc/nk_panel_body.h b/nys_koop_lqr_amd/csrc/nk_panel_body.h
--- /dev/null
+++ b/nys_koop_lqr_amd/csrc/nk_panel_body.h
@@ -0,0 +1,77 @@
+#pragma once
+#include "nk_common.h"
+#include "nk_potrf_body.h"
+
+namespace nk {
+
+constexpr int PANEL_ROWS = 64;
+struct PanelSys {
+  double* P;
+  int64_t ldp;
+  const double* Linv;
+  int rows;
+  int nb;
+  int fix;
+  int nblocks;
+};
+__device__ __forceinline__ void chol_panel_rows(const PanelSys& s, int m0, int lane) {
+  __builtin_amdgcn_s_setprio(2);
+  const int l15 = lane & 15, l4 = lane >> 4;
+  const int nb = s.nb;
+  const double* __restrict__ Li = s.Linv;
+  const double* __restrict__ Ld = s.Linv + CHOL_NB * CHOL_NB;
+  double a[16];
+  {
+    const double* pr = s.P + (int64_t)min(m0 + l15, s.rows - 1) * s.ldp + l4;
+    if (nb == CHOL_NB) {
+#pragma unroll
+      for (int t = 0; t < 16; ++t) a[t] = pr[4 * t];
+    } else {
+#pragma unroll
+      for (int t = 0; t < 16; ++t) a[t] = (4 * t + l4 < nb) ? pr[4 * t] : 0.0;
+    }
+  }
+  double li[4][16];
+#pragma unroll
+  for (int j = 0; j < 4; ++j)
+#pragma unroll
+    for (int t = 0; t < 16; ++t) li[j][t] = Li[(16 * j + l15) * CHOL_NB + 4 * t + l4];
+  d4 p1[4];
+#pragma unroll
+  for (int j = 0; j < 4; ++j) p1[j] = d4{0.0, 0.0, 0.0, 0.0};
+#pragma unroll
+  for (int t = 0; t < 16; ++t)
+#pragma unroll
+    for (int j = 0; j < 4; ++j) p1[j] = __builtin_amdgcn_mfma_f64_16x16x4f64(li[j][t], a[t], p1[j], 0, 0, 0);
+  if (s.fix == 2 || (s.fix == 1 && s.Linv[2 * CHOL_NB * CHOL_NB] != 0.0)) {
+    d4 rs[4];
+#pragma unroll
+    for (int j = 0; j < 4; ++j) rs[j] = d4{a[4 * j], a[4 * j + 1], a[4 * j + 2], a[4 * j + 3]};
+#pragma unroll
+    for (int t = 0; t < 16; ++t)
+#pragma unroll
+      for (int j = 0; j < 4; ++j)
+        rs[j] = __builtin_amdgcn_mfma_f64_16x16x4f64(-Ld[(16 * j + l15) * CHOL_NB + 4 * t + l4], p1[t >> 2][t & 3], rs[j], 0, 0, 0);
+    d4 p2[4];
+#pragma unroll
+    for (int j = 0; j < 4; ++j) p2[j] = p1[j];
+#pragma unroll
+    for (int t = 0; t < 16; ++t)
+#pragma unroll
+      for (int j = 0; j < 4; ++j) p2[j] = __builtin_amdgcn_mfma_f64_16x16x4f64(li[j][t], rs[t >> 2][t & 3], p2[j], 0, 0, 0);
+#pragma unroll
+    for (int j = 0; j < 4; ++j) p1[j] = p2[j];
+  }
+  __syncthreads();
+  const int row = m0 + l15;
+  if (row < s.rows) {
+    double* pw = s.P + (int64_t)row * s.ldp + l4;
+#pragma unroll
+    for (int j = 0; j < 4; ++j)
+#pragma unroll
+      for (int reg = 0; reg < 4; ++reg)
+        if (nb == CHOL_NB || 16 * j + 4 * reg + l4 < nb) pw[16 * j + 4 * reg] = p1[j][reg];
+  }
+}
+
+}
diff --git a/nys_koop_lqr_amd/csrc/nk_potrf_body.h b/nys_koop_lqr_amd/csrc/nk_potrf_body.h
--- a/nys_koop_lqr_amd/csrc/nk_potrf_body.h
+++ b/nys_koop_lqr_amd/csrc/nk_potrf_body.h
@@ -40,6 +40,18 @@
   for (int reg = 0; reg < 4; ++reg) T[(l4 + 4 * reg) * ldt + l15] = acc[reg];
 }
 
+template <bool WAVE_SYNC>
+__device__ __forceinline__ void potrf_sync() {
+  if (WAVE_SYNC) {
+    __builtin_amdgcn_fence(__ATOMIC_RELEASE, "workgroup");
+    __builtin_amdgcn_wave_barrier();
+    __builtin_amdgcn_fence(__ATOMIC_ACQUIRE, "workgroup");
+  } else {
+    __syncthreads();
+  }
+}
+
+template <bool WAVE_SYNC = false>
 __device__ __forceinline__ void potrf_diag_kernel_body(const PotrfBatch& pb, int blk, int which, int lane) {
   constexpr int NB = CHOL_NB;
   static_assert(NB == 64, "one lane per row, four 16-column panels");
@@ -63,7 +75,7 @@
     if (r < nb && lane < nb) v = A[(int64_t)r * lda + lane];
     As[r * PLD + lane] = v;
   }
-  __syncthreads();
+  potrf_sync<WAVE_SYNC>();
 
 #pragma unroll
   for (int pbk = 0; pbk < 4; ++pbk) {
@@ -102,7 +114,7 @@
     }
 #pragma unroll
     for (int jj = 0; jj < 16; ++jj) As[lane * PLD + c0 + jj] = R[jj];
-    __syncthreads();
+    potrf_sync<WAVE_SYNC>();
 #pragma unroll
     for (int ti = pbk + 1; ti < 4; ++ti)
 #pragma unroll
@@ -119,7 +131,7 @@
 #pragma unroll
         for (int reg = 0; reg < 4; ++reg) As[(16 * ti + l4 + 4 * reg) * PLD + 16 * tj + l15] = c[reg];
       }
-    __syncthreads();
+    potrf_sync<WAVE_SYNC>();
   }
 #pragma unroll 8
   for (int r = 0; r < NB; ++r)
@@ -143,38 +155,38 @@
 #pragma unroll
     for (int i = 0; i < 16; ++i) Db[i * PLD + l15] = x[i];
   }
-  __syncthreads();
+  potrf_sync<WAVE_SYNC>();
   auto Lblk = [&](int i, int j) { return As + (16 * i) * PLD + 16 * j; };
   auto Xblk = [&](int i, int j) { return Iv + (16 * i) * PLD + 16 * j; };
   const d4 zero = d4{0.0, 0.0, 0.0, 0.0};
 #pragma unroll
   for (int i = 1; i < 4; ++i)
     store_tile(Sc + (i - 1) * 16 * SLD, SLD, mm16<false>(Lblk(i, i - 1), PLD, Xblk(i - 1, i - 1), PLD, zero, l15, l4), l15, l4);
-  __syncthreads();
+  potrf_sync<WAVE_SYNC>();
 #pragma unroll
   for (int i = 1; i < 4; ++i)
     store_tile(Xblk(i, i - 1), PLD, mm16<true>(Xblk(i, i), PLD, Sc + (i - 1) * 16 * SLD, SLD, zero, l15, l4), l15, l4);
-  __syncthreads();
+  potrf_sync<WAVE_SYNC>();
 #pragma unroll
   for (int i = 2; i < 4; ++i) {
     d4 t = mm16<false>(Lblk(i, i - 2), PLD, Xblk(i - 2, i - 2), PLD, zero, l15, l4);
     t = mm16<false>(Lblk(i, i - 1), PLD, Xblk(i - 1, i - 2), PLD, t, l15, l4);
     store_tile(Sc + (i - 2) * 16 * SLD, SLD, t, l15, l4);
   }
-  __syncthreads();
+  potrf_sync<WAVE_SYNC>();
 #pragma unroll
   for (int i = 2; i < 4; ++i)
     store_tile(Xblk(i, i - 2), PLD, mm16<true>(Xblk(i, i), PLD, Sc + (i - 2) * 16 * SLD, SLD, zero, l15, l4), l15, l4);
-  __syncthreads();
+  potrf_sync<WAVE_SYNC>();
   {
     d4 t = mm16<false>(Lblk(3, 0), PLD, Xblk(0, 0), PLD, zero, l15, l4);
     t = mm16<false>(Lblk(3, 1), PLD, Xblk(1, 0), PLD, t, l15, l4);
     t = mm16<false>(Lblk(3, 2), PLD, Xblk(2, 0), PLD, t, l15, l4);
     store_tile(Sc, SLD, t, l15, l4);
   }
-  __syncthreads();
+  potrf_sync<WAVE_SYNC>();
   store_tile(Xblk(3, 0), PLD, mm16<true>(Xblk(3, 3), PLD, Sc, SLD, zero, l15, l4), l15, l4);
-  __syncthreads();
+  potrf_sync<WAVE_SYNC>();
 #pragma unroll 8
   for (int i = 0; i < NB; ++i) Linv[i * NB + lane] = (l4 <= (i >> 4)) ? Iv[i * PLD + lane] : 0.0;
   double sl = 0.0, si = 0.0;
diff --git a/nys_koop_lqr_amd/csrc/nk_trail.hip b/nys_koop_lqr_amd/csrc/nk_trail.hip
--- a/nys_koop_lqr_amd/csrc/nk_trail.hip
+++ b/nys_koop_lqr_amd/csrc/nk_trail.hip
@@ -1,5 +1,6 @@
 #include "nk_common.h"
 #include "nk_potrf_body.h"
+#include "nk_panel_body.h"
 
 namespace nk {
 
@@ -163,16 +164,6 @@
   return true;
 }
 
-constexpr int PANEL_ROWS = 64;
-struct PanelSys {
-  double* P;
-  int64_t ldp;
-  const double* Linv;
-  int rows;
-  int nb;
-  int fix;
-  int nblocks;
-};
 struct PanelBatch {
   PanelSys s[2];
 };
@@ -180,66 +171,8 @@
 __device__ __forceinline__ void chol_panel_kernel_body(const PanelBatch& pb) {
   const PanelSys s = pb.s[blockIdx.y];
   if ((int)blockIdx.x >= s.nblocks) return;
-  __builtin_amdgcn_s_setprio(2);
-  const int lane = threadIdx.x & 63;
   const int wave = __builtin_amdgcn_readfirstlane(threadIdx.x >> 6);
-  const int l15 = lane & 15, l4 = lane >> 4;
-  const int m0 = blockIdx.x * PANEL_ROWS + wave * 16;
-  const int nb = s.nb;
-  const double* __restrict__ Li = s.Linv;
-  const double* __restrict__ Ld = s.Linv + CHOL_NB * CHOL_NB;
-  double a[16];
-  {
-    const double* pr = s.P + (int64_t)min(m0 + l15, s.rows - 1) * s.ldp + l4;
-    if (nb == CHOL_NB) {
-#pragma unroll
-      for (int t = 0; t < 16; ++t) a[t] = pr[4 * t];
-    } else {
-#pragma unroll
-      for (int t = 0; t < 16; ++t) a[t] = (4 * t + l4 < nb) ? pr[4 * t] : 0.0;
-    }
-  }
-  double li[4][16];
-#pragma unroll
-  for (int j = 0; j < 4; ++j)
-#pragma unroll
-    for (int t = 0; t < 16; ++t) li[j][t] = Li[(16 * j + l15) * CHOL_NB + 4 * t + l4];
-  d4 p1[4];
-#pragma unroll
-  for (int j = 0; j < 4; ++j) p1[j] = d4{0.0, 0.0, 0.0, 0.0};
-#pragma unroll
-  for (int t = 0; t < 16; ++t)
-#pragma unroll
-    for (int j = 0; j < 4; ++j) p1[j] = __builtin_amdgcn_mfma_f64_16x16x4f64(li[j][t], a[t], p1[j], 0, 0, 0);
-  if (s.fix == 2 || (s.fix == 1 && s.Linv[2 * CHOL_NB * CHOL_NB] != 0.0)) {
-    d4 rs[4];
-#pragma unroll
-    for (int j = 0; j < 4; ++j) rs[j] = d4{a[4 * j], a[4 * j + 1], a[4 * j + 2], a[4 * j + 3]};
-#pragma unroll
-    for (int t = 0; t < 16; ++t)
-#pragma unroll
-      for (int j = 0; j < 4; ++j)
-        rs[j] = __builtin_amdgcn_mfma_f64_16x16x4f64(-Ld[(16 * j + l15) * CHOL_NB + 4 * t + l4], p1[t >> 2][t & 3], rs[j], 0, 0, 0);
-    d4 p2[4];
-#pragma unroll
-    for (int j = 0; j < 4; ++j) p2[j] = p1[j];
-#pragma unroll
-    for (int t = 0; t < 16; ++t)
-#pragma unroll
-      for (int j = 0; j < 4; ++j) p2[j] = __builtin_amdgcn_mfma_f64_16x16x4f64(li[j][t], rs[t >> 2][t & 3], p2[j], 0, 0, 0);
-#pragma unroll
-    for (int j = 0; j < 4; ++j) p1[j] = p2[j];
-  }
-  __syncthreads();
-  const int row = m0 + l15;
-  if (row < s.rows) {
-    double* pw = s.P + (int64_t)row * s.ldp + l4;
-#pragma unroll
-    for (int j = 0; j < 4; ++j)
-#pragma unroll
-      for (int reg = 0; reg < 4; ++reg)
-        if (nb == CHOL_NB || 16 * j + 4 * reg + l4 < nb) pw[16 * j + 4 * reg] = p1[j][reg];
-  }
+  chol_panel_rows(s, blockIdx.x * PANEL_ROWS + wave * 16, threadIdx.x & 63);
 }
 __global__ void __launch_bounds__(256) chol_panel_kernel(PanelBatch pb) { chol_panel_kernel_body(pb); }
 __global__ void __launch_bounds__(256) chol_panel_kernel_batched(const nk::ArgPack<PanelBatch>* table) { chol_panel_kernel_body(table[blockIdx.z].v); }
```

After: 24.57 (median of 6 runs). 4.0% higher.
